# AlexiaChen/mpvss-rs

Hardware: NVIDIA B200
Metric: verified DLEQ shares/sec (MODP n=4096 t=2731, verify_distribution_shares) (higher is better)
Workload: dtype u32 limbs (2048-bit integers)

## Files before the change

mpvss_rs_b200/csrc/ctx.h:

```cpp
#pragma once
#include <cuda_runtime.h>
#include <stdint.h>
#include <mutex>
#include <string.h>
#include <algorithm>
#include <string>
#include <vector>
#include "../../include/mpvss_b200.h"
#include "bigint.h"

struct DevBuf {
  void* p = nullptr;
  size_t cap = 0;
  cudaError_t ensure(size_t bytes) {
    if (bytes <= cap) return cudaSuccess;
    if (p) cudaFree(p);
    p = nullptr;
    cap = 0;
    cudaError_t e = cudaMalloc(&p, bytes);
    if (e == cudaSuccess) cap = bytes;
    return e;
  }
  void release() {
    if (p) cudaFree(p);
    p = nullptr;
    cap = 0;
  }
  template <typename T>
  T* as() const { return static_cast<T*>(p); }
};

struct PinBuf {
  void* p = nullptr;
  size_t cap = 0;
  cudaError_t ensure(size_t bytes) {
    if (bytes <= cap) return cudaSuccess;
    if (p) cudaFreeHost(p);
    p = nullptr;
    cap = 0;
    cudaError_t e = cudaMallocHost(&p, bytes);
    if (e == cudaSuccess) cap = bytes;
    return e;
  }
  void release() {
    if (p) cudaFreeHost(p);
    p = nullptr;
    cap = 0;
  }
  template <typename T>
  T* as() const { return static_cast<T*>(p); }
};

struct mpvss_ctx {
  int group = 0;
  int device = 0;
  int sm_count = 148;
  cudaStream_t stream = nullptr;
  cudaStream_t aux[2] = {nullptr, nullptr};
  cudaEvent_t ev0 = nullptr, ev1 = nullptr, ev_mid = nullptr, ev_h0 = nullptr, ev_h1 = nullptr, ev_fork = nullptr, ev_join[2] = {nullptr, nullptr};
  float phase_ms[4] = {0, 0, 0, 0};
  std::recursive_mutex mu;
  std::string err;
  float last_ms = 0.f;
  int last_launches = 0;
  bool timing_open = false;

  int modp_tpi = 8;
  bool modp_tpi_auto = true;
  int v_tpi = 8;
  int v_wpc = 1;
  std::vector<int64_t> v_plan_pos;
  int v_plan_tpi = 0, v_plan_wpc = 0;
  size_t v_plan_t = 0;
  uint32_t v_plan_kreq = 0, v_k = 1;
  DevBuf v_first, v_steps, v_e, v_h, v_t2;
  int modp_chunks = 0;
  uint64_t v_plan_sqr = 0, v_plan_mul = 0;
  int modp_wpc = 0;
  size_t exp2_filler_ctas = 0;
  int modp_overlap = 3;
  big::Int q, qm1, g;
  DevBuf consts_q, consts_g;
  DevBuf gens;
  DevBuf comb[2];
  int modp_comb = 1;
  int modp_msm = 2;
  int msm_threshold = 512;
  static constexpr size_t msm_batch_threshold = 4096;
  bool device_hash = false;
  bool validate = false;
  bool modp_np1 = false;
  size_t ec_threads = 0;
  DevBuf ec_comb;
  DevBuf ec_consts;
  big::Int ec_order;
  std::vector<uint8_t> ec_gen;
  std::vector<DevBuf> scratch;
  std::vector<PinBuf> pinned;
  size_t v_n = 0, v_t = 0;
  uint32_t v_rwin = 0, v_cwin = 0;
  size_t v_np = 0;
  uint32_t v_nops_max = 1;
  std::vector<uint8_t> v_challenge;
  std::vector<uint32_t> v_hpos;
  size_t ec_chunks = 1;
  const uint32_t* v_comb = nullptr;
  DevBuf v_slot, v_nd, v_ops, v_comm, v_cm, v_pos, v_pk, v_y, v_r, v_c, v_x, v_a1, v_a2;
  DevBuf v_st, v_cst;
  DevBuf v_frames, v_gather, v_ordered;
  PinBuf h_frames;
  size_t v_n_total = 0;
  uint64_t horner_sqr = 0, horner_mul = 0;
  void* comm = nullptr;
  int nranks = 1, rank = 0;
  cudaEvent_t ev_chunk[16] = {};

  mpvss_ctx() : scratch(24), pinned(8) {}
  DevBuf& buf(size_t i) { return scratch.at(i); }
  PinBuf& pin(size_t i) { return pinned.at(i); }
};

int mpvss_fail(mpvss_ctx* ctx, int status, const std::string& msg);
int mpvss_cuda_fail(mpvss_ctx* ctx, cudaError_t e, const char* what);

#define MPVSS_CUDA(ctx, expr)                                        \
  do {                                                               \
    cudaError_t _e = (expr);                                         \
    if (_e != cudaSuccess) return mpvss_cuda_fail(ctx, _e, #expr);   \
  } while (0)
#define MPVSS_TRY(expr)            \
  do {                             \
    int _s = (expr);               \
    if (_s != MPVSS_OK) return _s; \
  } while (0)

void timing_begin(mpvss_ctx* ctx);
void timing_launch(mpvss_ctx* ctx, int n = 1);
int timing_end(mpvss_ctx* ctx);

namespace modp_api {
int init(mpvss_ctx* ctx);
void destroy(mpvss_ctx* ctx);
int batch_exp(mpvss_ctx*, const uint8_t*, size_t, const uint8_t*, size_t, uint8_t*);
int fixed_base_exp(mpvss_ctx*, int, const uint8_t*, size_t, uint8_t*);
int batch_mul(mpvss_ctx*, const uint8_t*, const uint8_t*, size_t, uint8_t*);
int poly_eval_exp(mpvss_ctx*, const uint8_t*, size_t, const int64_t*, size_t, uint8_t*);
int dleq_verify_commit(mpvss_ctx*, const uint8_t*, const uint8_t*, const uint8_t*, const uint8_t*, const uint8_t*,
                       const uint8_t*, size_t, size_t, uint8_t*, uint8_t*);
int dleq_prove_commit(mpvss_ctx*, const uint8_t*, const uint8_t*, const uint8_t*, size_t, uint8_t*, uint8_t*);
int multi_exp(mpvss_ctx*, const uint8_t*, const uint8_t*, size_t, uint8_t*);
int verify_stage(mpvss_ctx*, size_t, size_t, const uint8_t*, const int64_t*, const uint8_t*, const uint8_t*,
                 const uint8_t*, const uint8_t*);
int verify_run(mpvss_ctx*, int*, uint8_t*, uint8_t*, uint8_t*, uint8_t*);
int verify_batch(mpvss_ctx*, size_t, const size_t*, const size_t*, const uint8_t*, const int64_t*, const uint8_t*,
                 const uint8_t*, const uint8_t*, const uint8_t*, int*, uint8_t*);
int scalar_poly_eval(mpvss_ctx*, const uint8_t*, size_t, const int64_t*, size_t, uint8_t*);
int distribute(mpvss_ctx*, size_t, size_t, const uint8_t*, size_t, const uint8_t*, const uint8_t*, const uint8_t*,
               uint8_t*, uint8_t*, uint8_t*, uint8_t*, uint8_t*, uint8_t*);
int extract_shares(mpvss_ctx*, size_t, const uint8_t*, const uint8_t*, const uint8_t*, uint8_t*, uint8_t*, uint8_t*,
                   uint8_t*, int*);
int verify_shares(mpvss_ctx*, size_t, const uint8_t*, const uint8_t*, const uint8_t*, const uint8_t*, const uint8_t*,
                  int*);
int reconstruct(mpvss_ctx*, size_t, const int64_t*, const uint8_t*, const uint8_t*, uint8_t*, uint8_t*);
int reconstruct_batch(mpvss_ctx*, size_t, const size_t*, const int64_t*, const uint8_t*, const uint8_t*, uint8_t*,
                      uint8_t*, int*);
}
namespace secp_api {
int init(mpvss_ctx* ctx);
int batch_exp(mpvss_ctx*, const uint8_t*, size_t, const uint8_t*, size_t, uint8_t*);
int fixed_base_exp(mpvss_ctx*, int, const uint8_t*, size_t, uint8_t*);
int batch_mul(mpvss_ctx*, const uint8_t*, const uint8_t*, size_t, uint8_t*);
int poly_eval_exp(mpvss_ctx*, const uint8_t*, size_t, const int64_t*, size_t, uint8_t*);
int dleq_verify_commit(mpvss_ctx*, const uint8_t*, const uint8_t*, const uint8_t*, const uint8_t*, const uint8_t*,
                       const uint8_t*, size_t, size_t, uint8_t*, uint8_t*);
int dleq_prove_commit(mpvss_ctx*, const uint8_t*, const uint8_t*, const uint8_t*, size_t, uint8_t*, uint8_t*);
int multi_exp(mpvss_ctx*, const uint8_t*, const uint8_t*, size_t, uint8_t*);
int verify_stage(mpvss_ctx*, size_t, size_t, const uint8_t*, const int64_t*, const uint8_t*, const uint8_t*,
                 const uint8_t*, const uint8_t*);
int verify_run(mpvss_ctx*, int*, uint8_t*, uint8_t*, uint8_t*, uint8_t*);
int verify_batch(mpvss_ctx*, size_t, const size_t*, const size_t*, const uint8_t*, const int64_t*, const uint8_t*,
                 const uint8_t*, const uint8_t*, const uint8_t*, int*, uint8_t*);
int scalar_poly_eval(mpvss_ctx*, const uint8_t*, size_t, const int64_t*, size_t, uint8_t*);
int distribute(mpvss_ctx*, size_t, size_t, const uint8_t*, size_t, const uint8_t*, const uint8_t*, const uint8_t*,
               uint8_t*, uint8_t*, uint8_t*, uint8_t*, uint8_t*, uint8_t*);
int extract_shares(mpvss_ctx*, size_t, const uint8_t*, const uint8_t*, const uint8_t*, uint8_t*, uint8_t*, uint8_t*,
                   uint8_t*, int*);
int verify_shares(mpvss_ctx*, size_t, const uint8_t*, const uint8_t*, const uint8_t*, const uint8_t*, const uint8_t*,
                  int*);
int reconstruct(mpvss_ctx*, size_t, const int64_t*, const uint8_t*, const uint8_t*, uint8_t*, uint8_t*);
int reconstruct_batch(mpvss_ctx*, size_t, const size_t*, const int64_t*, const uint8_t*, const uint8_t*, uint8_t*,
                      uint8_t*, int*);
}
namespace rist_api {
int init(mpvss_ctx* ctx);
int batch_exp(mpvss_ctx*, const uint8_t*, size_t, const uint8_t*, size_t, uint8_t*);
int fixed_base_exp(mpvss_ctx*, int, const uint8_t*, size_t, uint8_t*);
int batch_mul(mpvss_ctx*, const uint8_t*, const uint8_t*, size_t, uint8_t*);
int poly_eval_exp(mpvss_ctx*, const uint8_t*, size_t, const int64_t*, size_t, uint8_t*);
int dleq_verify_commit(mpvss_ctx*, const uint8_t*, const uint8_t*, const uint8_t*, const uint8_t*, const uint8_t*,
                       const uint8_t*, size_t, size_t, uint8_t*, uint8_t*);
int dleq_prove_commit(mpvss_ctx*, const uint8_t*, const uint8_t*, const uint8_t*, size_t, uint8_t*, uint8_t*);
int multi_exp(mpvss_ctx*, const uint8_t*, const uint8_t*, size_t, uint8_t*);
int verify_stage(mpvss_ctx*, size_t, size_t, const uint8_t*, const int64_t*, const uint8_t*, const uint8_t*,
                 const uint8_t*, const uint8_t*);
int verify_run(mpvss_ctx*, int*, uint8_t*, uint8_t*, uint8_t*, uint8_t*);
int verify_batch(mpvss_ctx*, size_t, const size_t*, const size_t*, const uint8_t*, const int64_t*, const uint8_t*,
                 const uint8_t*, const uint8_t*, const uint8_t*, int*, uint8_t*);
int scalar_poly_eval(mpvss_ctx*, const uint8_t*, size_t, const int64_t*, size_t, uint8_t*);
int distribute(mpvss_ctx*, size_t, size_t, const uint8_t*, size_t, const uint8_t*, const uint8_t*, const uint8_t*,
               uint8_t*, uint8_t*, uint8_t*, uint8_t*, uint8_t*, uint8_t*);
int extract_shares(mpvss_ctx*, size_t, const uint8_t*, const uint8_t*, const uint8_t*, uint8_t*, uint8_t*, uint8_t*,
                   uint8_t*, int*);
int verify_shares(mpvss_ctx*, size_t, const uint8_t*, const uint8_t*, const uint8_t*, const uint8_t*, const uint8_t*,
                  int*);
int reconstruct(mpvss_ctx*, size_t, const int64_t*, const uint8_t*, const uint8_t*, uint8_t*, uint8_t*);
int reconstruct_batch(mpvss_ctx*, size_t, const size_t*, const int64_t*, const uint8_t*, const uint8_t*, uint8_t*,
                      uint8_t*, int*);
}
```

mpvss_rs_b200/csrc/modp.cu:

```cuda
#include <cuda_runtime.h>
#include "modp_kernels.cuh"
#include "modp_launch.h"

namespace modp {


template <int TPI, bool NP1, bool CHUNKED>
__global__ void __launch_bounds__(HORNER_MAX_WARPS_PER_CTA * 32) horner_kernel(HornerArgs A) {
  extern __shared__ __align__(16) uint32_t smem[];
  uint32_t w = threadIdx.x >> 5;
  horner_body<TPI, NP1, CHUNKED>(A, blockIdx.x * (blockDim.x >> 5) + w, smem + w * horner_smem_words<TPI>,
                                 A.nops ? A.nops[blockIdx.x] : A.nops_all, blockIdx.x);
}

template <int TPI>
__global__ void __launch_bounds__(WARPS_PER_CTA * 32) exp2_kernel(Exp2Args A) {
  extern __shared__ __align__(16) uint32_t smem[];
  uint32_t w = threadIdx.x >> 5;
  exp2_body<TPI>(A, blockIdx.x * WARPS_PER_CTA + w, smem + w * exp2_smem_words<TPI>);
}

template <int TPI>
__global__ void __launch_bounds__(32) exp2_filler_kernel(Exp2Args A, uint32_t nwarps) {
  extern __shared__ __align__(16) uint32_t smem[];
  for (uint32_t w = blockIdx.x; w < nwarps; w += gridDim.x) {
    exp2_body<TPI>(A, w, smem);
    __syncwarp();
  }
}

template <int TPI>
__global__ void __launch_bounds__(32) comb1_kernel(CombArgs A) {
  extern __shared__ __align__(16) uint32_t smem[];
  comb1_body<TPI>(A, blockIdx.x, smem);
}
template <int TPI>
__global__ void __launch_bounds__(32) comb2_kernel(CombArgs A) {
  extern __shared__ __align__(16) uint32_t smem[];
  comb2_body<TPI>(A, blockIdx.x, smem);
}

template <int TPI>
__global__ void __launch_bounds__(WARPS_PER_CTA * 32) mul_kernel(MulArgs A) {
  extern __shared__ __align__(16) uint32_t smem[];
  uint32_t w = threadIdx.x >> 5;
  mul_body<TPI>(A, blockIdx.x * WARPS_PER_CTA + w, smem + w * mul_smem_words<TPI>);
}

__global__ void __launch_bounds__(128) frame_kernel(FrameArgs A) { frame_body(A, blockIdx.x * 128 + threadIdx.x); }
__global__ void __launch_bounds__(64) resp_kernel(RespArgs A) { resp_body(A, blockIdx.x * 64 + threadIdx.x); }
__global__ void __launch_bounds__(64) poly_kernel(PolyArgs A) { poly_body(A, blockIdx.x * 64 + threadIdx.x); }
__global__ void __launch_bounds__(64) lagrange_kernel(LagrangeArgs A) { lagrange_body(A, blockIdx.x * 64 + threadIdx.x); }
__global__ void __launch_bounds__(64) lagrange_boxes_kernel(LagrangeBoxesArgs A) {
  lagrange_boxes_body(A, blockIdx.x * 64 + threadIdx.x);
}

template <int TPI>
__global__ void __launch_bounds__(WARPS_PER_CTA * 32) mul_rows_kernel(MulRowsArgs A) {
  extern __shared__ __align__(16) uint32_t smem[];
  uint32_t w = threadIdx.x >> 5;
  mul_rows_body<TPI>(A, blockIdx.x * WARPS_PER_CTA + w, smem + w * mul_smem_words<TPI>);
}

__global__ void __launch_bounds__(256) msm_sort_kernel(const uint8_t* scalars, uint32_t k, uint32_t* idx, uint32_t* start) {
  __shared__ uint32_t cnt[257], cur[256];
  const uint32_t w = blockIdx.x;
  for (uint32_t d = threadIdx.x; d < 257; d += blockDim.x) cnt[d] = 0;
  __syncthreads();
  for (uint32_t i = threadIdx.x; i < k; i += blockDim.x) atomicAdd(&cnt[scalars[(size_t)i * 256 + w] + 1u], 1u);
  __syncthreads();
  if (threadIdx.x == 0)
    for (int d = 0; d < 256; ++d) cnt[d + 1] += cnt[d];
  __syncthreads();
  for (uint32_t d = threadIdx.x; d < 257; d += blockDim.x) {
    start[w * 257u + d] = cnt[d];
    if (d < 256) cur[d] = cnt[d];
  }
  __syncthreads();
  for (uint32_t i = threadIdx.x; i < k; i += blockDim.x)
    idx[(size_t)w * k + atomicAdd(&cur[scalars[(size_t)i * 256 + w]], 1u)] = i;
}

template <int TPI>
__global__ void __launch_bounds__(WARPS_PER_CTA * 32) msm_bucket_kernel(MsmBucketArgs A) {
  extern __shared__ __align__(16) uint32_t smem[];
  uint32_t w = threadIdx.x >> 5;
  msm_bucket_body<TPI>(A, blockIdx.x * WARPS_PER_CTA + w, smem + w * msm_smem_words<TPI>);
}
template <int TPI>
__global__ void __launch_bounds__(32) msm_window_kernel(MsmWindowArgs A) {
  extern __shared__ __align__(16) uint32_t smem[];
  msm_window_body<TPI>(A, blockIdx.x, smem);
}
template <int TPI>
__global__ void __launch_bounds__(32) msm_fold_kernel(MsmFoldArgs A) {
  extern __shared__ __align__(16) uint32_t smem[];
  msm_fold_body<TPI>(A, smem);
}

template <int TPI>
static uint32_t ctas_for(uint32_t n) {
  uint32_t per_cta = WARPS_PER_CTA * (32 / TPI);
  return (n + per_cta - 1) / per_cta;
}

template <typename K>
static cudaError_t set_smem(K kernel, size_t bytes) {
  cudaError_t e = cudaFuncSetAttribute(kernel, cudaFuncAttributePreferredSharedMemoryCarveout,
                                       (int)cudaSharedmemCarveoutMaxShared);
  if (e != cudaSuccess) return e;
  return cudaFuncSetAttribute(kernel, cudaFuncAttributeMaxDynamicSharedMemorySize, (int)bytes);
}

#define MODP_DISPATCH(tpi, ...)                            \
  switch (tpi) {                                           \
    case 4: { constexpr int T = 4; __VA_ARGS__; break; }   \
    case 8: { constexpr int T = 8; __VA_ARGS__; break; }   \
    case 16: { constexpr int T = 16; __VA_ARGS__; break; } \
    default: return cudaErrorInvalidValue;                 \
  }

template <int TPI, bool NP1, bool CHUNKED>
static cudaError_t horner_go(const HornerArgs& A, uint32_t grid, uint32_t wpc, size_t sm, cudaStream_t s) {
  cudaError_t e = set_smem(horner_kernel<TPI, NP1, CHUNKED>, sm);
  if (e != cudaSuccess) return e;
  horner_kernel<TPI, NP1, CHUNKED><<<grid, wpc * 32, sm, s>>>(A);
  return cudaSuccess;
}
cudaError_t launch_horner(int tpi, const HornerArgs& A, bool np_is_one, cudaStream_t s) {
  if (A.n == 0 || A.t == 0 || A.warps_per_cta > (uint32_t)HORNER_MAX_WARPS_PER_CTA) return cudaErrorInvalidValue;
  MODP_DISPATCH(tpi, {
    const uint32_t wpc = A.warps_per_cta ? A.warps_per_cta : 1u;
    size_t sm = wpc * horner_smem_words<T> * 4;
    uint32_t per_cta = wpc * (32 / T);
    uint32_t grid = (A.n + per_cta - 1) / per_cta;
    const bool chunked = A.cfirst && A.csteps;
    cudaError_t e = np_is_one ? (chunked ? horner_go<T, true, true>(A, grid, wpc, sm, s) : horner_go<T, true, false>(A, grid, wpc, sm, s))
                              : (chunked ? horner_go<T, false, true>(A, grid, wpc, sm, s) : horner_go<T, false, false>(A, grid, wpc, sm, s));
    if (e != cudaSuccess) return e;
  });
  return cudaGetLastError();
}

cudaError_t launch_exp2(int tpi, const Exp2Args& A, cudaStream_t s) {
  if (A.n == 0 || A.e1_windows == 0 || (A.b2 && A.e2_windows == 0)) return cudaErrorInvalidValue;
  MODP_DISPATCH(tpi, {
    size_t sm = WARPS_PER_CTA * exp2_smem_words<T> * 4;
    cudaError_t e = set_smem(exp2_kernel<T>, sm);
    if (e != cudaSuccess) return e;
    exp2_kernel<T><<<ctas_for<T>(A.n), WARPS_PER_CTA * 32, sm, s>>>(A);
  });
  return cudaGetLastError();
}

cudaError_t launch_exp2_filler(int tpi, const Exp2Args& A, size_t ctas, cudaStream_t s) {
  if (A.n == 0 || A.e1_windows == 0 || (A.b2 && A.e2_windows == 0)) return cudaErrorInvalidValue;
  MODP_DISPATCH(tpi, {
    size_t sm = exp2_smem_words<T> * 4;
    cudaError_t e = set_smem(exp2_filler_kernel<T>, sm);
    if (e != cudaSuccess) return e;
    uint32_t per_cta = 32 / T, nwarps = (A.n + per_cta - 1) / per_cta;
    uint32_t grid = (uint32_t)ctas;
    exp2_filler_kernel<T><<<grid < nwarps ? grid : nwarps, 32, sm, s>>>(A, nwarps);
  });
  return cudaGetLastError();
}

cudaError_t launch_frames(const FrameArgs& A, cudaStream_t s) {
  if (A.n == 0) return cudaErrorInvalidValue;
  frame_kernel<<<(A.n * 4 + 127) / 128, 128, 0, s>>>(A);
  return cudaGetLastError();
}

cudaError_t launch_resp(const RespArgs& A, cudaStream_t s) {
  if (A.n == 0) return cudaErrorInvalidValue;
  resp_kernel<<<(A.n + 63) / 64, 64, 0, s>>>(A);
  return cudaGetLastError();
}

cudaError_t launch_poly(const PolyArgs& A, cudaStream_t s) {
  if (A.n == 0 || A.t == 0) return cudaErrorInvalidValue;
  poly_kernel<<<(A.n + 63) / 64, 64, 0, s>>>(A);
  return cudaGetLastError();
}

cudaError_t launch_lagrange(const LagrangeArgs& A, cudaStream_t s) {
  if (A.k == 0) return cudaErrorInvalidValue;
  const uint32_t threads = 2u * (A.parts ? A.parts : 1u) * A.k;
  lagrange_kernel<<<(threads + 63) / 64, 64, 0, s>>>(A);
  return cudaGetLastError();
}

cudaError_t launch_lagrange_boxes(const LagrangeBoxesArgs& A, cudaStream_t s) {
  if (A.n == 0) return cudaErrorInvalidValue;
  const uint32_t threads = 2u * (A.parts ? A.parts : 1u) * A.n;
  lagrange_boxes_kernel<<<(threads + 63) / 64, 64, 0, s>>>(A);
  return cudaGetLastError();
}

cudaError_t launch_comb_build(int tpi, const CombArgs& A, cudaStream_t s) {
  MODP_DISPATCH(tpi, {
    size_t sm = comb_smem_words<T> * 4;
    comb1_kernel<T><<<1, 32, sm, s>>>(A);
    comb2_kernel<T><<<(A.rows + 32 / T - 1) / (32 / T), 32, sm, s>>>(A);
  });
  return cudaGetLastError();
}

cudaError_t launch_msm(const MsmBucketArgs& B, const uint32_t* scalars, uint32_t* idx, uint32_t* start,
                       uint32_t* wprod, uint32_t* out, cudaStream_t s) {
  if (B.windows == 0 || B.windows > 256 || B.k == 0) return cudaErrorInvalidValue;
  constexpr int T = 8;
  msm_sort_kernel<<<B.windows, 256, 0, s>>>(reinterpret_cast<const uint8_t*>(scalars), B.k, idx, start);
  const uint32_t groups = B.windows * 255u, per_cta = WARPS_PER_CTA * (32 / T);
  size_t sm = WARPS_PER_CTA * msm_smem_words<T> * 4;
  msm_bucket_kernel<T><<<(groups + per_cta - 1) / per_cta, WARPS_PER_CTA * 32, sm, s>>>(B);
  MsmWindowArgs W{B.consts, B.buckets, wprod, B.windows};
  msm_window_kernel<T><<<B.windows, 32, msm_window_smem_words<T> * 4, s>>>(W);
  MsmFoldArgs F{B.consts, wprod, out, B.windows};
  msm_fold_kernel<T><<<1, 32, msm_smem_words<T> * 4, s>>>(F);
  return cudaGetLastError();
}

cudaError_t launch_mul(int tpi, const MulArgs& A, cudaStream_t s) {
  if (A.n == 0) return cudaErrorInvalidValue;
  MODP_DISPATCH(tpi, {
    size_t sm = WARPS_PER_CTA * mul_smem_words<T> * 4;
    cudaError_t e = set_smem(mul_kernel<T>, sm);
    if (e != cudaSuccess) return e;
    mul_kernel<T><<<ctas_for<T>(A.n), WARPS_PER_CTA * 32, sm, s>>>(A);
  });
  return cudaGetLastError();
}

cudaError_t launch_mul_rows(int tpi, const MulRowsArgs& A, cudaStream_t s) {
  if (A.n == 0) return cudaErrorInvalidValue;
  MODP_DISPATCH(tpi, {
    size_t sm = WARPS_PER_CTA * mul_smem_words<T> * 4;
    cudaError_t e = set_smem(mul_rows_kernel<T>, sm);
    if (e != cudaSuccess) return e;
    mul_rows_kernel<T><<<ctas_for<T>(A.n), WARPS_PER_CTA * 32, sm, s>>>(A);
  });
  return cudaGetLastError();
}

}
```

mpvss_rs_b200/csrc/modp_api.cu:

```cuda
#include <algorithm>
#include <cstdlib>
#include "ctx.h"
#include "modp_chain.h"
#include "modp_launch.h"
#include "sha2.h"
#include "hash_launch.h"
#include "transcript.h"

namespace {

constexpr size_t EB = 256;
constexpr size_t EW = 64;

const char* RFC3526_2048 =
    "ffffffffffffffffc90fdaa22168c234c4c6628b80dc1cd129024e088a67cc74"
    "020bbea63b139b22514a08798e3404ddef9519b3cd3a431b302b0a6df25f1437"
    "4fe1356d6d51c245e485b576625e7ec6f44c42e9a637ed6b0bff5cb6f406b7ed"
    "ee386bfb5a899fa5ae9f24117c4b1fe649286651ece45b3dc2007cb8a163bf05"
    "98da48361c55d39a69163fa8fd24cf5f83655d23dca3ad961c62f356208552bb"
    "9ed529077096966d670c354e4abc9804f1746c08ca18217c32905e462e36ce3b"
    "e39e772c180e86039b2783a2ec07a28fb5c55df06f4c52c9de2bcbf695581718"
    "3995497cea956ae515d2261898fa051015728e5a8aacaa68ffffffffffffffff";

big::Int from_hex(const char* s) {
  size_t n = strlen(s);
  std::vector<uint8_t> be((n + 1) / 2, 0);
  for (size_t i = 0; i < n; ++i) {
    char c = s[n - 1 - i];
    uint8_t v = c <= '9' ? c - '0' : (c | 32) - 'a' + 10;
    be[be.size() - 1 - i / 2] |= v << (4 * (i % 2));
  }
  return big::from_be(be.data(), be.size());
}

void fill_consts(const big::Int& m, uint32_t* blk) {
  memset(blk, 0, modp::C_WORDS * 4);
  big::Int R(65, 0);
  R[64] = 1;
  big::Int nq = big::sub(R, m), one = big::mod(R, m), r2 = big::mulmod(one, one, m);
  auto put = [&](const big::Int& v, int off) {
    for (size_t i = 0; i < v.size() && i < 64; ++i) blk[off + i] = v[i];
  };
  put(m, modp::C_Q);
  put(nq, modp::C_NQ);
  put(one, modp::C_ONE);
  put(r2, modp::C_R2);
  big::Int one1(1, 1);
  put(big::shr1(big::add(m, one1)), modp::C_QH);
  uint32_t inv = 1, m0 = m[0];
  for (int i = 0; i < 5; ++i) inv *= 2u - m0 * inv;
  blk[modp::C_NP] = 0u - inv;
}

size_t min_be(const uint8_t* le, uint8_t* out) {
  size_t len = EB;
  while (len > 1 && le[len - 1] == 0) --len;
  for (size_t i = 0; i < len; ++i) out[i] = le[len - 1 - i];
  return len;
}
void framed_update(sha2::Sha256& h, const uint8_t* le) {
  uint8_t tmp[EB], len8[8] = {0};
  size_t len = min_be(le, tmp);
  len8[6] = (uint8_t)(len >> 8);
  len8[7] = (uint8_t)len;
  h.update(len8, 8);
  h.update(tmp, len);
}
void challenge_from_digest(const mpvss_ctx* ctx, const uint8_t digest[32], uint8_t out[EB]) {
  uint8_t h2[32];
  sha2::sha256(digest, 32, h2);
  big::Int c = big::mod(big::from_be(h2, 32), ctx->g);
  big::to_le(c, out, EB);
}
uint32_t windows_for(const uint8_t* scalars, size_t stride, size_t n) {
  size_t top = 0;
  for (size_t i = 0; i < n; ++i) {
    const uint8_t* s = scalars + i * stride;
    size_t len = EB;
    while (len > top && s[len - 1] == 0) --len;
    if (len > top) top = len;
    if (top == EB) break;
  }
  uint32_t w = (uint32_t)(top * 2);
  return w ? w : 1;
}

int h2d(mpvss_ctx* ctx, DevBuf& b, const void* src, size_t bytes) {
  MPVSS_CUDA(ctx, b.ensure(bytes));
  MPVSS_CUDA(ctx, cudaMemcpyAsync(b.p, src, bytes, cudaMemcpyHostToDevice, ctx->stream));
  return MPVSS_OK;
}
int d2h(mpvss_ctx* ctx, void* dst, const DevBuf& b, size_t bytes) {
  MPVSS_CUDA(ctx, cudaMemcpyAsync(dst, b.p, bytes, cudaMemcpyDeviceToHost, ctx->stream));
  return MPVSS_OK;
}
int sync(mpvss_ctx* ctx) {
  MPVSS_CUDA(ctx, cudaStreamSynchronize(ctx->stream));
  return MPVSS_OK;
}

int dev_exp2(mpvss_ctx* ctx, const uint32_t* consts, const uint32_t* b1, uint32_t b1s, const uint32_t* e1,
             uint32_t e1s, uint32_t e1w, const uint32_t* b2, uint32_t b2s, const uint32_t* e2, uint32_t e2s,
             uint32_t e2w, size_t n, uint32_t* out, cudaStream_t stream = nullptr, const uint32_t* comb1 = nullptr) {
  modp::Exp2Args A{consts, b1, e1, b2, e2, out, (uint32_t)n, b1s, e1s, e1w, b2s, e2s, e2w, comb1};
  if (ctx->exp2_filler_ctas)
    MPVSS_CUDA(ctx, modp::launch_exp2_filler(ctx->modp_tpi, A, ctx->exp2_filler_ctas, stream ? stream : ctx->stream));
  else
    MPVSS_CUDA(ctx, modp::launch_exp2(ctx->modp_tpi, A, stream ? stream : ctx->stream));
  timing_launch(ctx);
  return MPVSS_OK;
}
int dev_mul(mpvss_ctx* ctx, const uint32_t* consts, const uint32_t* a, uint32_t as, const uint32_t* b, uint32_t bs,
            uint32_t mode, size_t n, uint32_t* out) {
  modp::MulArgs A{consts, a, b, out, (uint32_t)n, mode, as, bs};
  MPVSS_CUDA(ctx, modp::launch_mul(ctx->modp_tpi, A, ctx->stream));
  timing_launch(ctx);
  return MPVSS_OK;
}

int comb_table(mpvss_ctx* ctx, int which, const uint32_t** out) {
  *out = nullptr;
  if (!ctx->modp_comb) return MPVSS_OK;
  DevBuf& t = ctx->comb[which];
  if (!t.p) {
    MPVSS_CUDA(ctx, t.ensure((size_t)256 * 256 * EB));
    modp::CombArgs A{ctx->consts_q.as<uint32_t>(), ctx->gens.as<uint32_t>() + which * 64, t.as<uint32_t>(), 256};
    MPVSS_CUDA(ctx, modp::launch_comb_build(ctx->modp_tpi, A, ctx->stream));
    MPVSS_CUDA(ctx, cudaStreamSynchronize(ctx->stream));
  }
  *out = t.as<uint32_t>();
  return MPVSS_OK;
}

int check_args(mpvss_ctx* ctx, bool ok, const char* what) {
  if (!ok) return mpvss_fail(ctx, MPVSS_ERR_ARG, what);
  return MPVSS_OK;
}

}

namespace modp_api {

int init(mpvss_ctx* ctx) {
  ctx->q = from_hex(RFC3526_2048);
  ctx->qm1 = big::sub(ctx->q, big::from_u64(1));
  ctx->g = big::shr1(ctx->qm1);
  std::vector<uint32_t> blk(modp::C_WORDS);
  fill_consts(ctx->q, blk.data());
  ctx->modp_np1 = blk[modp::C_NP] == 1u;
  MPVSS_TRY(h2d(ctx, ctx->consts_q, blk.data(), blk.size() * 4));
  fill_consts(ctx->g, blk.data());
  MPVSS_TRY(h2d(ctx, ctx->consts_g, blk.data(), blk.size() * 4));
  std::vector<uint32_t> gens(192, 0);
  gens[0] = 2;
  gens[64] = 4;
  gens[128] = 1;
  MPVSS_TRY(h2d(ctx, ctx->gens, gens.data(), gens.size() * 4));
  return sync(ctx);
}

void destroy(mpvss_ctx* ctx) {
  for (DevBuf* b : {&ctx->consts_q, &ctx->consts_g, &ctx->gens, &ctx->comb[0], &ctx->comb[1], &ctx->v_comm, &ctx->v_cm, &ctx->v_pos, &ctx->v_pk,
                    &ctx->v_y, &ctx->v_r, &ctx->v_c, &ctx->v_x, &ctx->v_a1, &ctx->v_a2, &ctx->v_slot, &ctx->v_nd, &ctx->v_ops, &ctx->v_frames, &ctx->v_gather, &ctx->v_ordered, &ctx->v_st, &ctx->v_cst, &ctx->v_first, &ctx->v_steps,
                    &ctx->v_e, &ctx->v_h, &ctx->v_t2})
    b->release();
}

int batch_exp(mpvss_ctx* ctx, const uint8_t* bases, size_t base_stride, const uint8_t* scalars, size_t n,
              uint8_t* out) {
  MPVSS_TRY(check_args(ctx, bases && scalars && out && n > 0 && (base_stride == 0 || base_stride == EB),
                       "batch_exp: bad arguments"));
  DevBuf &db = ctx->buf(0), &de = ctx->buf(1), &dout = ctx->buf(2);
  MPVSS_TRY(h2d(ctx, db, bases, base_stride ? n * EB : EB));
  MPVSS_TRY(h2d(ctx, de, scalars, n * EB));
  MPVSS_CUDA(ctx, dout.ensure(n * EB));
  timing_begin(ctx);
  MPVSS_TRY(dev_exp2(ctx, ctx->consts_q.as<uint32_t>(), db.as<uint32_t>(), base_stride ? EW : 0, de.as<uint32_t>(), EW,
                     windows_for(scalars, EB, n), nullptr, 0, nullptr, 0, 0, n, dout.as<uint32_t>()));
  MPVSS_TRY(timing_end(ctx));
  MPVSS_TRY(d2h(ctx, out, dout, n * EB));
  return sync(ctx);
}

int fixed_base_exp(mpvss_ctx* ctx, int generator, const uint8_t* scalars, size_t n, uint8_t* out) {
  MPVSS_TRY(check_args(ctx, scalars && out && n > 0 && (generator == MPVSS_GEN_MAIN || generator == MPVSS_GEN_SUBGROUP),
                       "fixed_base_exp: bad arguments"));
  DevBuf &de = ctx->buf(1), &dout = ctx->buf(2);
  MPVSS_TRY(h2d(ctx, de, scalars, n * EB));
  MPVSS_CUDA(ctx, dout.ensure(n * EB));
  const uint32_t* comb;
  MPVSS_TRY(comb_table(ctx, generator ? 1 : 0, &comb));
  timing_begin(ctx);
  MPVSS_TRY(dev_exp2(ctx, ctx->consts_q.as<uint32_t>(), ctx->gens.as<uint32_t>() + (generator ? 64 : 0), 0,
                     de.as<uint32_t>(), EW, windows_for(scalars, EB, n), nullptr, 0, nullptr, 0, 0, n,
                     dout.as<uint32_t>(), nullptr, comb));
  MPVSS_TRY(timing_end(ctx));
  MPVSS_TRY(d2h(ctx, out, dout, n * EB));
  return sync(ctx);
}

int batch_mul(mpvss_ctx* ctx, const uint8_t* a, const uint8_t* b, size_t n, uint8_t* out) {
  MPVSS_TRY(check_args(ctx, a && b && out && n > 0, "batch_mul: bad arguments"));
  DevBuf &da = ctx->buf(0), &db = ctx->buf(1), &dout = ctx->buf(2);
  MPVSS_TRY(h2d(ctx, da, a, n * EB));
  MPVSS_TRY(h2d(ctx, db, b, n * EB));
  MPVSS_CUDA(ctx, dout.ensure(n * EB));
  timing_begin(ctx);
  MPVSS_TRY(dev_mul(ctx, ctx->consts_q.as<uint32_t>(), da.as<uint32_t>(), EW, db.as<uint32_t>(), EW, 0, n,
                    dout.as<uint32_t>()));
  MPVSS_TRY(timing_end(ctx));
  MPVSS_TRY(d2h(ctx, out, dout, n * EB));
  return sync(ctx);
}

static int horner_tpi(const mpvss_ctx* ctx, size_t n) {
  if (!ctx->modp_tpi_auto) return ctx->modp_tpi;
  if (n >= 32768) return 4;
  if (n * 8 / 32 < (size_t)4 * (size_t)ctx->sm_count) return 16;
  return ctx->modp_tpi;
}

static int horner_wpc(const mpvss_ctx* ctx, size_t n, int tpi) {
  if (ctx->modp_wpc) return ctx->modp_wpc;
  (void)n;
  (void)tpi;
  return 1;
}

static uint32_t horner_chunks(const mpvss_ctx* ctx, size_t n, size_t t) {
  uint32_t K = 1;
  if (ctx->modp_chunks > 0) {
    K = (uint32_t)ctx->modp_chunks;
  } else {
    const size_t warps = (n + 3) / 4, full = (size_t)8 * (size_t)ctx->sm_count;
    while (K < 8 && warps * (K * 2) <= full) K *= 2;
  }
  if (ctx->modp_chunks <= 0 && t < 1366) K = 1;
  while (K > 1 && t / K < (ctx->modp_chunks > 0 ? 32u : 340u)) K /= 2;
  return K;
}

struct PosPlan {
  int tpi = 8;
  int wpc = 1;
  uint32_t K = 1, B = 0;
  std::vector<uint32_t> first, steps;
  std::vector<uint32_t> slot;
  std::vector<uint16_t> ops;
  std::vector<uint32_t> nops;
  uint64_t sqr = 0, mul = 0;
  uint32_t nops_max = 1;
};
static modp_chain::PowerTree g_tree;
static std::mutex g_tree_mu;

struct PlanBox {
  const int64_t* positions;
  size_t n, t;
  uint32_t cm_off, row_off;
};

static int prep_boxes(mpvss_ctx* ctx, const PlanBox* boxes, size_t nb, bool chunked, PosPlan& plan) {
  static_assert(modp_chain::SLOTS == modp::HC_SLOTS && modp_chain::OPS_MAX == modp::HC_OPS, "kernel / host op format");
  auto position = [&](const PlanBox& bx, size_t i) { return bx.positions ? bx.positions[i] : (int64_t)i + 1; };
  uint32_t maxp = 1;
  size_t n_all = 0;
  for (size_t b = 0; b < nb; ++b) {
    for (size_t i = 0; i < boxes[b].n; ++i) {
      int64_t p = position(boxes[b], i);
      if (p < 1 || p > 0x7fffffff) return mpvss_fail(ctx, MPVSS_ERR_ARG, "position out of range [1, 2^31)");
      maxp = std::max<uint32_t>(maxp, (uint32_t)p);
    }
    n_all += boxes[b].n;
  }
  std::lock_guard<std::mutex> lk(g_tree_mu);
  g_tree.build(std::min<uint32_t>(maxp, modp_chain::TREE_LIMIT));
  std::vector<std::vector<uint16_t>> ops(n_all);
  std::vector<std::vector<std::vector<uint32_t>>> by(nb, std::vector<std::vector<uint32_t>>(modp_chain::OPS_MAX + 1));
  std::vector<uint32_t> sq(n_all), ml(n_all);
  for (size_t b = 0, g = 0; b < nb; ++b)
    for (size_t i = 0; i < boxes[b].n; ++i, ++g) {
      if (!modp_chain::step_ops((uint32_t)position(boxes[b], i), g_tree, ops[g], &sq[g], &ml[g]))
        return mpvss_fail(ctx, MPVSS_ERR_UNSUPPORTED, "no addition chain within the kernel's slot budget");
      by[b][ops[g].size()].push_back((uint32_t)g);
    }
  const size_t t0 = boxes[0].t;
  if (chunked && nb != 1) return mpvss_fail(ctx, MPVSS_ERR_ARG, "a chunked plan covers one box");
  plan.K = chunked ? horner_chunks(ctx, n_all, t0) : 1;
  plan.B = (uint32_t)((t0 + plan.K - 1) / plan.K);
  plan.K = (uint32_t)((t0 + plan.B - 1) / plan.B);
  plan.tpi = plan.K > 1 ? ctx->modp_tpi : horner_tpi(ctx, n_all);
  plan.wpc = horner_wpc(ctx, n_all, plan.tpi);
  const size_t per_cta = (size_t)plan.wpc * (32 / plan.tpi);
  plan.slot.clear(); plan.ops.clear(); plan.nops.clear(); plan.first.clear(); plan.steps.clear();
  plan.nops_max = 1;
  plan.sqr = plan.mul = 0;
  std::vector<uint32_t> base(nb, 0);
  for (size_t b = 1; b < nb; ++b) base[b] = base[b - 1] + (uint32_t)boxes[b - 1].n;
  for (uint32_t k = 0; k < plan.K; ++k) {
    for (uint32_t len = modp_chain::OPS_MAX; len >= 1; --len) {
      for (size_t b = 0; b < nb; ++b) {
        const std::vector<uint32_t>& cls = by[b][len];
        if (cls.empty()) continue;
        const PlanBox& bx = boxes[b];
        const uint32_t lo = plan.K > 1 ? k * plan.B : 0, hi = (uint32_t)std::min<size_t>(bx.t, (size_t)lo + (plan.K > 1 ? plan.B : bx.t));
        plan.nops_max = std::max(plan.nops_max, len);
        auto emit = [&](uint32_t g, uint32_t slot) {
          plan.slot.push_back(slot);
          size_t at = plan.ops.size();
          plan.ops.resize(at + modp_chain::OPS_MAX, (uint16_t)modp_chain::B_ONE);
          std::copy(ops[g].begin(), ops[g].end(), plan.ops.begin() + at);
        };
        for (uint32_t g : cls) {
          emit(g, bx.row_off + k * (uint32_t)bx.n + (g - base[b]));
          plan.sqr += (uint64_t)sq[g] * (hi - lo - 1);
          plan.mul += (uint64_t)ml[g] * (hi - lo - 1);
        }
        while (plan.slot.size() % per_cta) emit(cls.back(), 0xffffffffu);
        const size_t ctas = plan.slot.size() / per_cta;
        plan.nops.resize(ctas, len);
        plan.first.resize(ctas, bx.cm_off + hi - 1);
        plan.steps.resize(ctas, hi - lo - 1);
      }
    }
  }
  return MPVSS_OK;
}
static int prep_positions(mpvss_ctx* ctx, const int64_t* positions, size_t n, size_t t, PosPlan& plan) {
  const PlanBox box{positions, n, t, 0, 0};
  return prep_boxes(ctx, &box, 1, true, plan);
}

static int dev_chunk_exponents(mpvss_ctx* ctx, const int64_t* positions, size_t n, uint32_t E, uint32_t* e_out_dev) {
  std::vector<uint8_t> base(n * EB, 0), bexp(EB, 0), e(n * EB);
  for (size_t i = 0; i < n; ++i) {
    uint32_t p = (uint32_t)(positions ? positions[i] : (int64_t)i + 1);
    memcpy(base.data() + i * EB, &p, 4);
  }
  memcpy(bexp.data(), &E, 4);
  DevBuf &db = ctx->buf(20), &dx = ctx->buf(21);
  MPVSS_TRY(h2d(ctx, db, base.data(), n * EB));
  MPVSS_TRY(h2d(ctx, dx, bexp.data(), EB));
  MPVSS_TRY(dev_exp2(ctx, ctx->consts_g.as<uint32_t>(), db.as<uint32_t>(), EW, dx.as<uint32_t>(), 0,
                     windows_for(bexp.data(), EB, 1), nullptr, 0, nullptr, 0, 0, n, e_out_dev));
  MPVSS_CUDA(ctx, cudaMemcpyAsync(e.data(), e_out_dev, n * EB, cudaMemcpyDeviceToHost, ctx->stream));
  MPVSS_TRY(sync(ctx));
  for (size_t i = 0; i < n; ++i) {
    if ((e[i * EB] & 1u) != (base[i * EB] & 1u)) {
      big::Int v = big::add(big::from_le(e.data() + i * EB, EB), ctx->g);
      big::to_le(v, e.data() + i * EB, EB);
    }
  }
  MPVSS_CUDA(ctx, cudaMemcpyAsync(e_out_dev, e.data(), n * EB, cudaMemcpyHostToDevice, ctx->stream));
  return sync(ctx);
}
static int plan_chunk_exponents(mpvss_ctx* ctx, const int64_t* positions, size_t n, const PosPlan& plan, DevBuf& e) {
  if (plan.K <= 1) return MPVSS_OK;
  MPVSS_CUDA(ctx, e.ensure((size_t)(plan.K - 1) * n * EB));
  for (uint32_t k = 1; k < plan.K; ++k)
    MPVSS_TRY(dev_chunk_exponents(ctx, positions, n, k * plan.B, e.as<uint32_t>() + (size_t)(k - 1) * n * EW));
  return MPVSS_OK;
}

struct PlanDev {
  const uint16_t* ops;
  const uint32_t *slot, *nops, *first, *steps;
  const uint32_t* e;
  size_t n_padded;
  uint32_t K;
  int tpi, wpc;
  bool boxes = false;
};
static int dev_horner(mpvss_ctx* ctx, const PlanDev& P, const uint32_t* comm, DevBuf& cm, size_t t, size_t n, DevBuf& hbuf,
                      DevBuf& tbuf, uint32_t* x) {
  const uint32_t* Kq = ctx->consts_q.as<uint32_t>();
  MPVSS_CUDA(ctx, cm.ensure(t * EB));
  MPVSS_TRY(dev_mul(ctx, Kq, comm, EW, nullptr, 0, 1, t, cm.as<uint32_t>()));
  uint32_t* h = x;
  if (P.K > 1) {
    MPVSS_CUDA(ctx, hbuf.ensure((size_t)P.K * n * EB));
    MPVSS_CUDA(ctx, tbuf.ensure((size_t)(P.K - 1) * n * EB));
    h = hbuf.as<uint32_t>();
  }
  static const bool uniform = getenv("MPVSS_HORNER_UNIFORM") != nullptr;
  const bool arrays = P.K > 1 || P.boxes || !uniform;
  modp::HornerArgs A{Kq, cm.as<uint32_t>(), P.ops, P.slot, P.nops, h, (uint32_t)t, (uint32_t)P.n_padded, 0,
                     (uint32_t)P.wpc, arrays ? P.first : nullptr, arrays ? P.steps : nullptr};
  MPVSS_CUDA(ctx, cudaEventRecord(ctx->ev_h0, ctx->stream));
  MPVSS_CUDA(ctx, modp::launch_horner(P.tpi, A, ctx->modp_np1, ctx->stream));
  MPVSS_CUDA(ctx, cudaEventRecord(ctx->ev_h1, ctx->stream));
  timing_launch(ctx);
  if (P.K > 1) {
    uint32_t* T = tbuf.as<uint32_t>();
    MPVSS_TRY(dev_exp2(ctx, Kq, h + n * EW, EW, P.e, EW, 512, nullptr, 0, nullptr, 0, 0, (size_t)(P.K - 1) * n, T));
    MPVSS_TRY(dev_mul(ctx, Kq, h, EW, T, EW, 0, n, x));
    for (uint32_t k = 2; k < P.K; ++k) MPVSS_TRY(dev_mul(ctx, Kq, x, EW, T + (size_t)(k - 1) * n * EW, EW, 0, n, x));
  }
  return MPVSS_OK;
}

int poly_eval_exp(mpvss_ctx* ctx, const uint8_t* commitments, size_t t, const int64_t* positions, size_t n,
                  uint8_t* out) {
  MPVSS_TRY(check_args(ctx, commitments && out && n > 0 && t > 0, "poly_eval_exp: bad arguments"));
  PosPlan plan;
  MPVSS_TRY(prep_positions(ctx, positions, n, t, plan));
  DevBuf &dc = ctx->buf(0), &dops = ctx->buf(1), &dout = ctx->buf(2), &dcm = ctx->buf(3), &dsl = ctx->buf(4),
         &dno = ctx->buf(5), &dfi = ctx->buf(6), &dstp = ctx->buf(7), &de = ctx->buf(8);
  const size_t np = plan.slot.size();
  MPVSS_TRY(h2d(ctx, dc, commitments, t * EB));
  MPVSS_TRY(h2d(ctx, dops, plan.ops.data(), plan.ops.size() * 2));
  MPVSS_TRY(h2d(ctx, dsl, plan.slot.data(), np * 4));
  MPVSS_TRY(h2d(ctx, dno, plan.nops.data(), plan.nops.size() * 4));
  MPVSS_TRY(h2d(ctx, dfi, plan.first.data(), plan.first.size() * 4));
  MPVSS_TRY(h2d(ctx, dstp, plan.steps.data(), plan.steps.size() * 4));
  MPVSS_CUDA(ctx, dout.ensure(n * EB));
  MPVSS_TRY(plan_chunk_exponents(ctx, positions, n, plan, de));
  PlanDev P{dops.as<uint16_t>(), dsl.as<uint32_t>(), dno.as<uint32_t>(), dfi.as<uint32_t>(), dstp.as<uint32_t>(),
            de.as<uint32_t>(), np, plan.K, plan.tpi, plan.wpc};
  timing_begin(ctx);
  MPVSS_TRY(dev_horner(ctx, P, dc.as<uint32_t>(), dcm, t, n, ctx->buf(9), ctx->buf(10), dout.as<uint32_t>()));
  MPVSS_TRY(timing_end(ctx));
  ctx->horner_sqr = plan.sqr;
  ctx->horner_mul = plan.mul;
  MPVSS_TRY(d2h(ctx, out, dout, n * EB));
  return sync(ctx);
}

int dleq_verify_commit(mpvss_ctx* ctx, const uint8_t* g1, const uint8_t* h1, const uint8_t* g2, const uint8_t* h2,
                       const uint8_t* r, const uint8_t* c, size_t c_stride, size_t n, uint8_t* a1, uint8_t* a2) {
  MPVSS_TRY(check_args(ctx, g1 && h1 && g2 && h2 && r && c && (!a1 == !a2) && n > 0 && (c_stride == 0 || c_stride == EB),
                       "dleq_verify_commit: bad arguments"));
  DevBuf &dg1 = ctx->buf(0), &dh1 = ctx->buf(1), &dg2 = ctx->buf(2), &dh2 = ctx->buf(3), &dr = ctx->buf(4),
         &dc = ctx->buf(5), &da1 = ctx->buf(6), &da2 = ctx->buf(7);
  MPVSS_TRY(h2d(ctx, dg1, g1, EB));
  MPVSS_TRY(h2d(ctx, dh1, h1, n * EB));
  MPVSS_TRY(h2d(ctx, dg2, g2, n * EB));
  MPVSS_TRY(h2d(ctx, dh2, h2, n * EB));
  MPVSS_TRY(h2d(ctx, dr, r, n * EB));
  MPVSS_TRY(h2d(ctx, dc, c, c_stride ? n * EB : EB));
  MPVSS_CUDA(ctx, da1.ensure(n * EB));
  MPVSS_CUDA(ctx, da2.ensure(n * EB));
  uint32_t rw = windows_for(r, EB, n), cw = windows_for(c, EB, c_stride ? n : 1), cs = c_stride ? EW : 0;
  const uint32_t* K = ctx->consts_q.as<uint32_t>();
  const uint32_t* comb = nullptr;
  {
    bool rest_zero = true;
    for (size_t i = 1; i < EB; ++i) rest_zero = rest_zero && g1[i] == 0;
    if (rest_zero && (g1[0] == 2 || g1[0] == 4)) MPVSS_TRY(comb_table(ctx, g1[0] == 4 ? 1 : 0, &comb));
  }
  timing_begin(ctx);
  MPVSS_TRY(dev_exp2(ctx, K, dg1.as<uint32_t>(), 0, dr.as<uint32_t>(), EW, rw, dh1.as<uint32_t>(), EW,
                     dc.as<uint32_t>(), cs, cw, n, da1.as<uint32_t>(), nullptr, comb));
  MPVSS_TRY(dev_exp2(ctx, K, dg2.as<uint32_t>(), EW, dr.as<uint32_t>(), EW, rw, dh2.as<uint32_t>(), EW,
                     dc.as<uint32_t>(), cs, cw, n, da2.as<uint32_t>()));
  MPVSS_TRY(timing_end(ctx));
  if (a1) MPVSS_TRY(d2h(ctx, a1, da1, n * EB));
  if (a2) MPVSS_TRY(d2h(ctx, a2, da2, n * EB));
  return sync(ctx);
}

int dleq_prove_commit(mpvss_ctx* ctx, const uint8_t* g1, const uint8_t* g2, const uint8_t* w, size_t n, uint8_t* a1,
                      uint8_t* a2) {
  MPVSS_TRY(check_args(ctx, g1 && g2 && w && a1 && a2 && n > 0, "dleq_prove_commit: bad arguments"));
  DevBuf &dg1 = ctx->buf(0), &dg2 = ctx->buf(2), &dw = ctx->buf(4), &da1 = ctx->buf(6), &da2 = ctx->buf(7);
  MPVSS_TRY(h2d(ctx, dg1, g1, EB));
  MPVSS_TRY(h2d(ctx, dg2, g2, n * EB));
  MPVSS_TRY(h2d(ctx, dw, w, n * EB));
  MPVSS_CUDA(ctx, da1.ensure(n * EB));
  MPVSS_CUDA(ctx, da2.ensure(n * EB));
  uint32_t ww = windows_for(w, EB, n);
  const uint32_t* K = ctx->consts_q.as<uint32_t>();
  timing_begin(ctx);
  MPVSS_TRY(dev_exp2(ctx, K, dg1.as<uint32_t>(), 0, dw.as<uint32_t>(), EW, ww, nullptr, 0, nullptr, 0, 0, n,
                     da1.as<uint32_t>()));
  MPVSS_TRY(dev_exp2(ctx, K, dg2.as<uint32_t>(), EW, dw.as<uint32_t>(), EW, ww, nullptr, 0, nullptr, 0, 0, n,
                     da2.as<uint32_t>()));
  MPVSS_TRY(timing_end(ctx));
  MPVSS_TRY(d2h(ctx, a1, da1, n * EB));
  MPVSS_TRY(d2h(ctx, a2, da2, n * EB));
  return sync(ctx);
}

static int dev_product_tree(mpvss_ctx* ctx, uint32_t* v, DevBuf& tmp, size_t n) {
  const uint32_t* K = ctx->consts_q.as<uint32_t>();
  MPVSS_CUDA(ctx, tmp.ensure(((n + 1) / 2) * EB));
  while (n > 1) {
    size_t half = n / 2;
    MPVSS_TRY(dev_mul(ctx, K, v, EW, v + half * EW, EW, 0, half, tmp.as<uint32_t>()));
    if (n & 1)
      MPVSS_CUDA(ctx, cudaMemcpyAsync(tmp.as<uint32_t>() + half * EW, v + 2 * half * EW, EB, cudaMemcpyDeviceToDevice,
                                      ctx->stream));
    n = half + (n & 1);
    MPVSS_CUDA(ctx, cudaMemcpyAsync(v, tmp.p, n * EB, cudaMemcpyDeviceToDevice, ctx->stream));
  }
  return MPVSS_OK;
}

static int multi_exp_buckets(mpvss_ctx* ctx, DevBuf& db, DevBuf& de, uint32_t windows, size_t n, DevBuf& dout) {
  DevBuf &dm = ctx->buf(15), &didx = ctx->buf(16), &dst = ctx->buf(17), &dbk = ctx->buf(18), &dwp = ctx->buf(19);
  MPVSS_CUDA(ctx, didx.ensure((size_t)windows * n * 4));
  MPVSS_CUDA(ctx, dst.ensure((size_t)windows * 257 * 4));
  MPVSS_CUDA(ctx, dm.ensure(n * EB));
  MPVSS_CUDA(ctx, dbk.ensure((size_t)windows * 256 * EB));
  MPVSS_CUDA(ctx, dwp.ensure((size_t)windows * EB));
  const uint32_t* K = ctx->consts_q.as<uint32_t>();
  MPVSS_TRY(dev_mul(ctx, K, db.as<uint32_t>(), EW, nullptr, 0, 1, n, dm.as<uint32_t>()));
  modp::MsmBucketArgs B{K, dm.as<uint32_t>(), didx.as<uint32_t>(), dst.as<uint32_t>(), dbk.as<uint32_t>(), windows,
                        (uint32_t)n};
  MPVSS_CUDA(ctx, modp::launch_msm(B, de.as<uint32_t>(), didx.as<uint32_t>(), dst.as<uint32_t>(), dwp.as<uint32_t>(),
                                   dout.as<uint32_t>(), ctx->stream));
  timing_launch(ctx, 4);
  return MPVSS_OK;
}

int multi_exp(mpvss_ctx* ctx, const uint8_t* bases, const uint8_t* scalars, size_t n, uint8_t* out) {
  MPVSS_TRY(check_args(ctx, bases && scalars && out && n > 0, "multi_exp: bad arguments"));
  DevBuf &db = ctx->buf(0), &de = ctx->buf(1), &dout = ctx->buf(2), &tmp = ctx->buf(3);
  MPVSS_TRY(h2d(ctx, db, bases, n * EB));
  MPVSS_CUDA(ctx, dout.ensure(n * EB));
  const bool buckets = ctx->modp_msm == 1 || (ctx->modp_msm == 2 && n >= (size_t)ctx->msm_threshold);
  MPVSS_TRY(h2d(ctx, de, scalars, n * EB));
  timing_begin(ctx);
  if (buckets) {
    MPVSS_TRY(multi_exp_buckets(ctx, db, de, (windows_for(scalars, EB, n) + 1) / 2, n, dout));
  } else {
    MPVSS_TRY(dev_exp2(ctx, ctx->consts_q.as<uint32_t>(), db.as<uint32_t>(), EW, de.as<uint32_t>(), EW,
                       windows_for(scalars, EB, n), nullptr, 0, nullptr, 0, 0, n, dout.as<uint32_t>()));
    MPVSS_TRY(dev_product_tree(ctx, dout.as<uint32_t>(), tmp, n));
  }
  MPVSS_TRY(timing_end(ctx));
  MPVSS_TRY(d2h(ctx, out, dout, EB));
  return sync(ctx);
}

int scalar_poly_eval(mpvss_ctx* ctx, const uint8_t* coeffs, size_t t, const int64_t* positions, size_t n, uint8_t* out) {
  MPVSS_TRY(check_args(ctx, coeffs && out && n > 0 && t > 0, "scalar_poly_eval: bad arguments"));
  std::vector<uint32_t> order(EW, 0), pos(n);
  for (size_t i = 0; i < ctx->qm1.size(); ++i) order[i] = ctx->qm1[i];
  for (size_t i = 0; i < n; ++i) {
    int64_t p = positions ? positions[i] : (int64_t)i + 1;
    if (p < 1 || p > 0x7fffffff) return mpvss_fail(ctx, MPVSS_ERR_ARG, "position out of range [1, 2^31)");
    pos[i] = (uint32_t)p;
  }
  std::vector<uint8_t> co(t * EB);
  for (size_t j = 0; j < t; ++j) big::to_le(big::mod(big::from_le(coeffs + j * EB, EB), ctx->qm1), co.data() + j * EB, EB);
  DevBuf &dco = ctx->buf(0), &dp = ctx->buf(1), &dord = ctx->buf(11), &dpos = ctx->buf(12);
  MPVSS_TRY(h2d(ctx, dco, co.data(), t * EB));
  MPVSS_TRY(h2d(ctx, dord, order.data(), EB));
  MPVSS_TRY(h2d(ctx, dpos, pos.data(), n * 4));
  MPVSS_CUDA(ctx, dp.ensure(n * EB));
  timing_begin(ctx);
  modp::PolyArgs PA{dco.as<uint32_t>(), dord.as<uint32_t>(), dpos.as<uint32_t>(), dp.as<uint32_t>(), (uint32_t)t,
                    (uint32_t)n};
  MPVSS_CUDA(ctx, modp::launch_poly(PA, ctx->stream));
  timing_launch(ctx);
  MPVSS_TRY(timing_end(ctx));
  MPVSS_TRY(d2h(ctx, out, dp, n * EB));
  MPVSS_CUDA(ctx, cudaMemsetAsync(dco.p, 0, dco.cap, ctx->stream));
  return sync(ctx);
}

static int validate_elements(mpvss_ctx* ctx, const uint32_t* dev, size_t count, uint8_t* bad) {
  std::vector<uint8_t> gexp(EB), res(count * EB), in(count * EB);
  big::to_le(ctx->g, gexp.data(), EB);
  DevBuf &de = ctx->buf(20), &dout = ctx->buf(21);
  MPVSS_TRY(h2d(ctx, de, gexp.data(), EB));
  MPVSS_CUDA(ctx, dout.ensure(count * EB));
  MPVSS_TRY(dev_exp2(ctx, ctx->consts_q.as<uint32_t>(), dev, EW, de.as<uint32_t>(), 0, 512, nullptr, 0, nullptr, 0, 0,
                     count, dout.as<uint32_t>()));
  MPVSS_TRY(d2h(ctx, res.data(), dout, count * EB));
  MPVSS_CUDA(ctx, cudaMemcpyAsync(in.data(), dev, count * EB, cudaMemcpyDeviceToHost, ctx->stream));
  MPVSS_TRY(sync(ctx));
  for (size_t i = 0; i < count; ++i) {
    big::Int x = big::from_le(in.data() + i * EB, EB);
    bool one = res[i * EB] == 1;
    for (size_t k = 1; k < EB && one; ++k) one = res[i * EB + k] == 0;
    if (big::is_zero(x) || big::cmp(x, ctx->q) >= 0 || !one) bad[i] = 1;
  }
  return MPVSS_OK;
}

static const transcript::Geom GEOM{EB, true};

static const uint8_t* slice_rows(const mpvss_ctx* ctx, const uint8_t* all, size_t n_total, size_t width,
                                 std::vector<uint8_t>& tmp) {
  if (ctx->nranks <= 1) return all;
  tmp.clear();
  for (size_t i = (size_t)ctx->rank; i < n_total; i += (size_t)ctx->nranks)
    tmp.insert(tmp.end(), all + i * width, all + (i + 1) * width);
  return tmp.data();
}

int verify_stage(mpvss_ctx* ctx, size_t n_total, size_t t, const uint8_t* commitments, const int64_t* positions,
                 const uint8_t* publickeys, const uint8_t* shares, const uint8_t* responses, const uint8_t* challenge) {
  ctx->v_n_total = 0;
  MPVSS_TRY(check_args(ctx, n_total > 0 && t > 0 && commitments && publickeys && shares && responses && challenge,
                       "verify_distribution: bad arguments"));
  const size_t n = transcript::local_count(n_total, ctx->nranks, ctx->rank);
  std::vector<int64_t> pos(n);
  for (size_t j = 0; j < n; ++j) {
    const size_t i = (size_t)ctx->rank + j * (size_t)ctx->nranks;
    pos[j] = positions ? positions[i] : (int64_t)i + 1;
  }
  for (size_t i = 0; i < n_total; ++i)
    if (positions && (positions[i] < 1 || positions[i] > 0x7fffffff))
      return mpvss_fail(ctx, MPVSS_ERR_ENCODING, "verify_distribution: position out of range [1, 2^31)");
  PosPlan plan;
  const uint32_t want_k = n ? horner_chunks(ctx, n, t) : 1;
  const bool replan = n && !(ctx->v_plan_pos == pos && ctx->v_plan_t == t && ctx->v_plan_kreq == want_k &&
                             ctx->v_plan_tpi == (want_k > 1 ? ctx->modp_tpi : horner_tpi(ctx, n)) &&
                             ctx->v_plan_wpc == horner_wpc(ctx, n, ctx->v_plan_tpi));
  if (replan) {
    ctx->v_plan_pos.clear();
    MPVSS_TRY(prep_positions(ctx, pos.data(), n, t, plan));
    ctx->v_np = plan.slot.size();
    ctx->v_nops_max = plan.nops_max;
    ctx->v_tpi = plan.tpi;
    ctx->v_wpc = plan.wpc;
    ctx->v_k = plan.K;
    ctx->v_plan_sqr = plan.sqr;
    ctx->v_plan_mul = plan.mul;
  }
  ctx->horner_sqr = ctx->v_plan_sqr;
  ctx->horner_mul = ctx->v_plan_mul;
  std::vector<uint8_t> tpk, ty, tr;
  const uint8_t* pk = slice_rows(ctx, publickeys, n_total, EB, tpk);
  const uint8_t* y = slice_rows(ctx, shares, n_total, EB, ty);
  const uint8_t* r = slice_rows(ctx, responses, n_total, EB, tr);
  MPVSS_TRY(h2d(ctx, ctx->v_comm, commitments, t * EB));
  MPVSS_TRY(h2d(ctx, ctx->v_c, challenge, EB));
  if (replan) {
    MPVSS_TRY(h2d(ctx, ctx->v_ops, plan.ops.data(), plan.ops.size() * 2));
    MPVSS_TRY(h2d(ctx, ctx->v_slot, plan.slot.data(), ctx->v_np * 4));
    MPVSS_TRY(h2d(ctx, ctx->v_nd, plan.nops.data(), plan.nops.size() * 4));
    MPVSS_TRY(h2d(ctx, ctx->v_first, plan.first.data(), plan.first.size() * 4));
    MPVSS_TRY(h2d(ctx, ctx->v_steps, plan.steps.data(), plan.steps.size() * 4));
    MPVSS_TRY(plan_chunk_exponents(ctx, pos.data(), n, plan, ctx->v_e));
    MPVSS_TRY(sync(ctx));
    ctx->v_plan_pos = pos;
    ctx->v_plan_t = t;
    ctx->v_plan_kreq = want_k;
    ctx->v_plan_tpi = plan.tpi;
    ctx->v_plan_wpc = plan.wpc;
  }
  if (n) {
    MPVSS_TRY(h2d(ctx, ctx->v_pk, pk, n * EB));
    MPVSS_TRY(h2d(ctx, ctx->v_y, y, n * EB));
    MPVSS_TRY(h2d(ctx, ctx->v_r, r, n * EB));
    MPVSS_CUDA(ctx, ctx->v_x.ensure(n * EB));
    MPVSS_CUDA(ctx, ctx->v_a1.ensure(n * EB));
    MPVSS_CUDA(ctx, ctx->v_a2.ensure(n * EB));
  }
  const size_t rpr = transcript::rows_per_rank(n_total, ctx->nranks);
  MPVSS_CUDA(ctx, ctx->v_frames.ensure(rpr * GEOM.row()));
  MPVSS_CUDA(ctx, cudaMemsetAsync(ctx->v_frames.p, 0, rpr * GEOM.row(), ctx->stream));
  if (ctx->nranks > 1) MPVSS_CUDA(ctx, ctx->v_gather.ensure((size_t)ctx->nranks * rpr * GEOM.row()));
  MPVSS_TRY(comb_table(ctx, 1, &ctx->v_comb));
  ctx->v_rwin = n ? windows_for(r, EB, n) : 1;
  ctx->v_cwin = windows_for(challenge, EB, 1);
  ctx->v_challenge.assign(challenge, challenge + EB);
  ctx->v_n = n;
  ctx->v_t = t;
  MPVSS_TRY(sync(ctx));
  ctx->v_n_total = n_total;
  return MPVSS_OK;
}

static int a2_placement(const mpvss_ctx* ctx, size_t n, double horner, size_t np, int tpi, uint32_t rwin, uint32_t cwin) {
  int overlap = ctx->modp_overlap;
  if (overlap == 3) {
    const size_t groups_per_warp = 32 / (size_t)ctx->modp_tpi;
    const size_t nwarps = (n + groups_per_warp - 1) / groups_per_warp;
    const size_t rounds = (nwarps + (size_t)ctx->sm_count - 1) / (size_t)ctx->sm_count;
    const double filler = (double)rounds * (5.0 * (rwin + cwin) + 30.0);
    if (filler > 0.6 * horner) overlap = 0;
    const size_t slots = (size_t)4 * (size_t)ctx->sm_count;
    const size_t hw = np / (32 / (size_t)tpi);
    const size_t holes = (slots - hw % slots) % slots;
    if (holes < (size_t)ctx->sm_count) overlap = 0;
    if (overlap == 0 && hw + nwarps <= (size_t)12 * (size_t)ctx->sm_count) overlap = 2;
  }
  return overlap;
}

static int verify_kernels(mpvss_ctx* ctx) {
  const size_t n = ctx->v_n, t = ctx->v_t;
  const uint32_t* K = ctx->consts_q.as<uint32_t>();
  uint32_t* X = ctx->v_x.as<uint32_t>();
  timing_begin(ctx);
  if (n == 0) {
    MPVSS_TRY(timing_end(ctx));
    ctx->phase_ms[0] = ctx->phase_ms[1] = ctx->phase_ms[2] = 0.f;
    return MPVSS_OK;
  }
  MPVSS_CUDA(ctx, cudaEventRecord(ctx->ev_fork, ctx->stream));
  auto launch_a2 = [&](cudaStream_t s) {
    return dev_exp2(ctx, K, ctx->v_pk.as<uint32_t>(), EW, ctx->v_r.as<uint32_t>(), EW, ctx->v_rwin,
                    ctx->v_y.as<uint32_t>(), EW, ctx->v_c.as<uint32_t>(), 0, ctx->v_cwin, n,
                    ctx->v_a2.as<uint32_t>(), s);
  };
  const int overlap = a2_placement(ctx, n, (double)(t > 1 ? t - 1 : 0) / (double)ctx->v_k * (double)ctx->v_nops_max,
                                   ctx->v_np, ctx->v_tpi, ctx->v_rwin, ctx->v_cwin);
  const bool side = overlap == 2 || overlap == 3;
  if (!side) MPVSS_TRY(launch_a2(ctx->stream));
  PlanDev P{ctx->v_ops.as<uint16_t>(), ctx->v_slot.as<uint32_t>(), ctx->v_nd.as<uint32_t>(), ctx->v_first.as<uint32_t>(),
            ctx->v_steps.as<uint32_t>(), ctx->v_e.as<uint32_t>(), ctx->v_np, ctx->v_k, ctx->v_tpi, ctx->v_wpc};
  MPVSS_TRY(dev_horner(ctx, P, ctx->v_comm.as<uint32_t>(), ctx->v_cm, t, n, ctx->v_h, ctx->v_t2, X));
  if (side) {
    MPVSS_CUDA(ctx, cudaStreamWaitEvent(ctx->aux[0], ctx->ev_fork, 0));
    if (overlap == 3) ctx->exp2_filler_ctas = (size_t)ctx->sm_count;
    int rc = launch_a2(ctx->aux[0]);
    ctx->exp2_filler_ctas = 0;
    MPVSS_TRY(rc);
    MPVSS_CUDA(ctx, cudaEventRecord(ctx->ev_join[0], ctx->aux[0]));
  }
  MPVSS_CUDA(ctx, cudaEventRecord(ctx->ev_mid, ctx->stream));
  MPVSS_TRY(dev_exp2(ctx, K, ctx->gens.as<uint32_t>() + 64, 0, ctx->v_r.as<uint32_t>(), EW, ctx->v_rwin, X, EW,
                     ctx->v_c.as<uint32_t>(), 0, ctx->v_cwin, n, ctx->v_a1.as<uint32_t>(), nullptr, ctx->v_comb));
  if (side) MPVSS_CUDA(ctx, cudaStreamWaitEvent(ctx->stream, ctx->ev_join[0], 0));
  modp::FrameArgs FA{X, ctx->v_y.as<uint32_t>(), ctx->v_a1.as<uint32_t>(), ctx->v_a2.as<uint32_t>(),
                     ctx->v_frames.as<uint8_t>(), (uint32_t)n};
  MPVSS_CUDA(ctx, modp::launch_frames(FA, ctx->stream));
  timing_launch(ctx);
  if (ctx->validate) {
    std::vector<uint8_t> bad(t + 2 * n, 0);
    MPVSS_TRY(validate_elements(ctx, ctx->v_comm.as<uint32_t>(), t, bad.data()));
    MPVSS_TRY(validate_elements(ctx, ctx->v_pk.as<uint32_t>(), n, bad.data() + t));
    MPVSS_TRY(validate_elements(ctx, ctx->v_y.as<uint32_t>(), n, bad.data() + t + n));
    if (std::find(bad.begin(), bad.end(), 1) != bad.end()) {
      const uint8_t mark = 0xff;
      MPVSS_CUDA(ctx, cudaMemcpyAsync(ctx->v_frames.p, &mark, 1, cudaMemcpyHostToDevice, ctx->stream));
    }
  }
  MPVSS_TRY(timing_end(ctx));
  MPVSS_CUDA(ctx, cudaEventElapsedTime(&ctx->phase_ms[0], ctx->ev0, ctx->ev_mid));
  MPVSS_CUDA(ctx, cudaEventElapsedTime(&ctx->phase_ms[1], ctx->ev_mid, ctx->ev1));
  MPVSS_CUDA(ctx, cudaEventElapsedTime(&ctx->phase_ms[2], ctx->ev_h0, ctx->ev_h1));
  return MPVSS_OK;
}

int verify_run(mpvss_ctx* ctx, int* ok, uint8_t* x_out, uint8_t* a1_out, uint8_t* a2_out, uint8_t* digest_out) {
  MPVSS_TRY(check_args(ctx, ok && ctx->v_n_total > 0, "verify_distribution_run: nothing staged"));
  MPVSS_TRY(check_args(ctx, ctx->nranks <= 1 || (!x_out && !a1_out && !a2_out),
                       "verify_distribution: x/a1/a2 outputs are not available with a communicator"));
  const size_t n = ctx->v_n, n_total = ctx->v_n_total;
  MPVSS_TRY(verify_kernels(ctx));
  const uint8_t* rows = ctx->v_frames.as<uint8_t>();
  if (ctx->nranks > 1) {
    MPVSS_TRY(comm_allgather(ctx, ctx->v_frames.p, ctx->v_gather.p,
                             transcript::rows_per_rank(n_total, ctx->nranks) * GEOM.row()));
    MPVSS_CUDA(ctx, ctx->v_ordered.ensure(n_total * GEOM.row()));
    MPVSS_TRY(comm_reorder_rows(ctx, ctx->v_gather.p, ctx->v_ordered.p, n_total, GEOM.row()));
    rows = ctx->v_ordered.as<uint8_t>();
  }
  uint8_t digest[32], c[EB];
  if (ctx->device_hash) {
    MPVSS_TRY(transcript::device_digest(ctx, rows, n_total, ctx->nranks, GEOM, digest));
  } else {
    sha2::Sha256 h;
    MPVSS_TRY(transcript::fetch_and_hash(ctx, rows, n_total, ctx->nranks, GEOM, h, true));
    h.finalize(digest);
  }
  challenge_from_digest(ctx, digest, c);
  *ok = memcmp(c, ctx->v_challenge.data(), EB) == 0;
  for (size_t r = 0; r < std::min<size_t>((size_t)ctx->nranks, n_total); ++r)
    if (ctx->h_frames.as<uint8_t>()[r * GEOM.row()] == 0xff) *ok = 0;
  if (digest_out) memcpy(digest_out, digest, 32);
  if (x_out) MPVSS_TRY(d2h(ctx, x_out, ctx->v_x, n * EB));
  if (a1_out) MPVSS_TRY(d2h(ctx, a1_out, ctx->v_a1, n * EB));
  if (a2_out) MPVSS_TRY(d2h(ctx, a2_out, ctx->v_a2, n * EB));
  return sync(ctx);
}

int verify_batch(mpvss_ctx* ctx, size_t nb, const size_t* nv, const size_t* tv, const uint8_t* commitments,
                 const int64_t* positions, const uint8_t* publickeys, const uint8_t* shares, const uint8_t* responses,
                 const uint8_t* challenges, int* ok_out, uint8_t* digests_out) {
  std::vector<size_t> noff(nb + 1, 0), toff(nb + 1, 0);
  for (size_t b = 0; b < nb; ++b) {
    noff[b + 1] = noff[b] + nv[b];
    toff[b + 1] = toff[b] + tv[b];
  }
  const size_t N = noff[nb], Tt = toff[nb];
  std::vector<uint8_t> live(nb, 1);
  std::vector<PlanBox> boxes;
  for (size_t b = 0; b < nb; ++b) {
    const int64_t* p = positions ? positions + noff[b] : nullptr;
    for (size_t i = 0; p && i < nv[b] && live[b]; ++i) live[b] = p[i] >= 1 && p[i] <= 0x7fffffff;
    if (live[b]) boxes.push_back(PlanBox{p, nv[b], tv[b], (uint32_t)toff[b], (uint32_t)noff[b]});
  }
  std::vector<uint8_t> cexp(N * EB);
  for (size_t b = 0; b < nb; ++b)
    for (size_t i = noff[b]; i < noff[b + 1]; ++i) memcpy(cexp.data() + i * EB, challenges + b * EB, EB);
  const uint32_t rwin = windows_for(responses, EB, N), cwin = windows_for(challenges, EB, nb);
  DevBuf &dcomm = ctx->buf(0), &dcm = ctx->buf(1), &dpk = ctx->buf(2), &dy = ctx->buf(3), &dr = ctx->buf(4),
         &dc = ctx->buf(5), &dx = ctx->buf(6), &da1 = ctx->buf(7), &da2 = ctx->buf(8), &dfr = ctx->buf(9),
         &dops = ctx->buf(10), &dsl = ctx->buf(11), &dno = ctx->buf(12), &dfi = ctx->buf(13), &dstp = ctx->buf(14);
  MPVSS_TRY(h2d(ctx, dcomm, commitments, Tt * EB));
  MPVSS_TRY(h2d(ctx, dpk, publickeys, N * EB));
  MPVSS_TRY(h2d(ctx, dy, shares, N * EB));
  MPVSS_TRY(h2d(ctx, dr, responses, N * EB));
  MPVSS_TRY(h2d(ctx, dc, cexp.data(), N * EB));
  for (DevBuf* b : {&dx, &da1, &da2}) MPVSS_CUDA(ctx, b->ensure(N * EB));
  MPVSS_CUDA(ctx, dfr.ensure(N * GEOM.row()));
  if (boxes.size() < nb) MPVSS_CUDA(ctx, cudaMemsetAsync(dx.p, 0, N * EB, ctx->stream));
  PosPlan plan;
  if (!boxes.empty()) {
    MPVSS_TRY(prep_boxes(ctx, boxes.data(), boxes.size(), false, plan));
    MPVSS_TRY(h2d(ctx, dops, plan.ops.data(), plan.ops.size() * 2));
    MPVSS_TRY(h2d(ctx, dsl, plan.slot.data(), plan.slot.size() * 4));
    MPVSS_TRY(h2d(ctx, dno, plan.nops.data(), plan.nops.size() * 4));
    MPVSS_TRY(h2d(ctx, dfi, plan.first.data(), plan.first.size() * 4));
    MPVSS_TRY(h2d(ctx, dstp, plan.steps.data(), plan.steps.size() * 4));
  }
// ... 197 lines not shown
  big::Int inv;
  if (!big::modinv_odd(big::from_le(root, EB), ctx->g, &inv))
    return mpvss_fail(ctx, MPVSS_ERR_ARG, "batch inversion: an element is 0 modulo the subgroup order");
  big::to_le(inv, root, EB);
  uint32_t *cur = ia.as<uint32_t>(), *nxt = ib.as<uint32_t>();
  MPVSS_CUDA(ctx, cudaMemcpyAsync(cur, root, EB, cudaMemcpyHostToDevice, ctx->stream));
  MPVSS_CUDA(ctx, cudaStreamSynchronize(ctx->stream));
  memset(root, 0, EB);
  std::fill(inv.begin(), inv.end(), 0u);
  for (size_t l = L; l >= 1; --l) {
    const size_t h = N >> l;
    MPVSS_TRY(dev_mul(ctx, Kg, cur, EW, T + (off[l - 1] + h) * EW, EW, 0, h, nxt));
    MPVSS_TRY(dev_mul(ctx, Kg, cur, EW, T + off[l - 1] * EW, EW, 0, h, nxt + h * EW));
    std::swap(cur, nxt);
  }
  MPVSS_CUDA(ctx, cudaMemcpyAsync(out, cur, n * EB, cudaMemcpyDeviceToDevice, ctx->stream));
  return MPVSS_OK;
}

static int share_challenges(mpvss_ctx* ctx, const uint32_t* h1, const uint32_t* h2, const uint32_t* a1, const uint32_t* a2,
                            size_t n, uint32_t* c_out, uint32_t stride) {
  DevBuf& drows = ctx->buf(14);
  MPVSS_CUDA(ctx, drows.ensure(n * 4 * modp::FRAME_BYTES));
  const float ms0 = ctx->last_ms;
  const int l0 = ctx->last_launches;
  timing_begin(ctx);
  modp::FrameArgs FA{h1, h2, a1, a2, drows.as<uint8_t>(), (uint32_t)n};
  MPVSS_CUDA(ctx, modp::launch_frames(FA, ctx->stream));
  shadev::RowHashArgs HA{drows.as<uint8_t>(), 4u * modp::FRAME_BYTES, (uint32_t)modp::FRAME_BYTES, c_out, stride, nullptr,
                         (uint32_t)n, 0u};
  MPVSS_CUDA(ctx, shadev::launch_row_hash(HA, ctx->stream));
  timing_launch(ctx, 2);
  MPVSS_TRY(timing_end(ctx));
  ctx->last_ms += ms0;
  ctx->last_launches += l0;
  return MPVSS_OK;
}

int extract_shares(mpvss_ctx* ctx, size_t n, const uint8_t* private_keys, const uint8_t* witnesses,
                   const uint8_t* enc_shares, uint8_t* publickeys_out, uint8_t* shares_out, uint8_t* challenges_out,
                   uint8_t* responses_out, int* status_out) {
  MPVSS_TRY(check_args(ctx, n > 0 && private_keys && witnesses && enc_shares && publickeys_out && shares_out &&
                                challenges_out && responses_out,
                       "extract_shares: bad arguments"));
  const uint32_t* K = ctx->consts_q.as<uint32_t>();
  const uint32_t* Kg = ctx->consts_g.as<uint32_t>();
  const uint32_t* G = ctx->gens.as<uint32_t>();
  std::vector<uint8_t> skg(n * EB);
  std::vector<int> st(n, MPVSS_OK);
  for (size_t i = 0; i < n; ++i) {
    big::Int sk = big::mod(big::from_le(private_keys + i * EB, EB), ctx->qm1);
    big::Int r = big::mod(sk, ctx->g);
    if (!big::is_odd(sk) || big::is_zero(r)) {
      st[i] = MPVSS_ERR_NOT_INVERTIBLE;
      r = big::from_u64(1);
    }
    big::to_le(r, skg.data() + i * EB, EB);
  }
  DevBuf &dsk = ctx->buf(0), &dskg = ctx->buf(1), &dinv = ctx->buf(3), &dw = ctx->buf(4),
         &dY = ctx->buf(5), &dpk = ctx->buf(6), &dS = ctx->buf(7), &dA1 = ctx->buf(8), &dA2 = ctx->buf(9);
  MPVSS_TRY(h2d(ctx, dsk, private_keys, n * EB));
  MPVSS_TRY(h2d(ctx, dskg, skg.data(), n * EB));
  MPVSS_TRY(h2d(ctx, dw, witnesses, n * EB));
  MPVSS_TRY(h2d(ctx, dY, enc_shares, n * EB));
  for (DevBuf* b : {&dinv, &dpk, &dS, &dA1, &dA2}) MPVSS_CUDA(ctx, b->ensure(n * EB));
  timing_begin(ctx);
  MPVSS_TRY(dev_batch_inverse_g(ctx, dskg.as<uint32_t>(), n, dinv.as<uint32_t>()));
  MPVSS_TRY(timing_end(ctx));
  std::vector<uint8_t> inv(n * EB);
  MPVSS_TRY(d2h(ctx, inv.data(), dinv, n * EB));
  MPVSS_TRY(sync(ctx));
  for (size_t i = 0; i < n; ++i) {
    big::Int x = big::from_le(inv.data() + i * EB, EB);
    if (!big::is_odd(x)) x = big::add(x, ctx->g);
    big::to_le(x, inv.data() + i * EB, EB);
  }
  MPVSS_TRY(h2d(ctx, dinv, inv.data(), n * EB));
  const uint32_t skw = 512, ww = 512;
  const uint32_t* combG;
  MPVSS_TRY(comb_table(ctx, 0, &combG));
  float ms0 = ctx->last_ms;
  int l0 = ctx->last_launches;
  timing_begin(ctx);
  MPVSS_TRY(dev_exp2(ctx, K, G, 0, dsk.as<uint32_t>(), EW, skw, nullptr, 0, nullptr, 0, 0, n, dpk.as<uint32_t>(),
                     nullptr, combG));
  MPVSS_TRY(dev_exp2(ctx, K, dY.as<uint32_t>(), EW, dinv.as<uint32_t>(), EW, 512, nullptr, 0, nullptr, 0, 0, n,
                     dS.as<uint32_t>()));
  MPVSS_TRY(dev_exp2(ctx, K, G, 0, dw.as<uint32_t>(), EW, ww, nullptr, 0, nullptr, 0, 0, n, dA1.as<uint32_t>(),
                     nullptr, combG));
  MPVSS_TRY(dev_exp2(ctx, K, dS.as<uint32_t>(), EW, dw.as<uint32_t>(), EW, ww, nullptr, 0, nullptr, 0, 0, n,
                     dA2.as<uint32_t>()));
  MPVSS_TRY(timing_end(ctx));
  ctx->last_ms += ms0;
  ctx->last_launches += l0;
  {
    std::vector<uint32_t> order(EW, 0);
    for (size_t i = 0; i < ctx->qm1.size(); ++i) order[i] = ctx->qm1[i];
    DevBuf &dord = ctx->buf(11), &dch = ctx->buf(12), &dR = ctx->buf(13);
    MPVSS_TRY(h2d(ctx, dord, order.data(), EB));
    MPVSS_CUDA(ctx, dch.ensure(n * EB));
    MPVSS_CUDA(ctx, dR.ensure(n * EB));
    MPVSS_TRY(share_challenges(ctx, dpk.as<uint32_t>(), dY.as<uint32_t>(), dA1.as<uint32_t>(), dA2.as<uint32_t>(), n,
                               dch.as<uint32_t>(), EW));
    modp::RespArgs RA{dord.as<uint32_t>(), dsk.as<uint32_t>(), dw.as<uint32_t>(), dch.as<uint32_t>(), dR.as<uint32_t>(),
                      (uint32_t)n, EW, EW};
    MPVSS_CUDA(ctx, modp::launch_resp(RA, ctx->stream));
    ctx->last_launches += 1;
    MPVSS_TRY(d2h(ctx, publickeys_out, dpk, n * EB));
    MPVSS_TRY(d2h(ctx, shares_out, dS, n * EB));
    MPVSS_TRY(d2h(ctx, challenges_out, dch, n * EB));
    MPVSS_TRY(d2h(ctx, responses_out, dR, n * EB));
    for (DevBuf* b : {&dsk, &dskg, &dinv, &dw}) MPVSS_CUDA(ctx, cudaMemsetAsync(b->p, 0, b->cap, ctx->stream));
    MPVSS_TRY(sync(ctx));
  }
  if (status_out) memcpy(status_out, st.data(), n * sizeof(int));
  return MPVSS_OK;
}

int verify_shares(mpvss_ctx* ctx, size_t n, const uint8_t* publickeys, const uint8_t* shares,
                  const uint8_t* enc_shares, const uint8_t* challenges, const uint8_t* responses, int* ok_out) {
  MPVSS_TRY(check_args(ctx, n > 0 && publickeys && shares && enc_shares && challenges && responses && ok_out,
                       "verify_shares: bad arguments"));
  std::vector<uint8_t> gen(EB, 0);
  gen[0] = 2;
  MPVSS_TRY(dleq_verify_commit(ctx, gen.data(), publickeys, shares, enc_shares, responses, challenges, EB, n, nullptr,
                               nullptr));
  DevBuf& dch = ctx->buf(12);
  MPVSS_CUDA(ctx, dch.ensure(n * 32));
  MPVSS_TRY(share_challenges(ctx, ctx->buf(1).as<uint32_t>(), ctx->buf(3).as<uint32_t>(), ctx->buf(6).as<uint32_t>(),
                             ctx->buf(7).as<uint32_t>(), n, dch.as<uint32_t>(), 8));
  std::vector<uint8_t> c(n * 32);
  MPVSS_TRY(d2h(ctx, c.data(), dch, n * 32));
  MPVSS_TRY(sync(ctx));
  for (size_t i = 0; i < n; ++i) {
    const uint8_t* given = challenges + i * EB;
    bool same = memcmp(c.data() + i * 32, given, 32) == 0;
    for (size_t k = 32; k < EB && same; ++k) same = given[k] == 0;
    ok_out[i] = same;
  }
  return MPVSS_OK;
}

int reconstruct(mpvss_ctx* ctx, size_t k, const int64_t* positions, const uint8_t* shares, const uint8_t* u,
                uint8_t* secret_out, uint8_t* gs_out) {
  MPVSS_TRY(check_args(ctx, k > 0 && positions && shares && u && secret_out, "reconstruct: bad arguments"));
  for (size_t i = 0; i < k; ++i)
    if (positions[i] < 1 || positions[i] > 0x7fffffff) return mpvss_fail(ctx, MPVSS_ERR_ARG, "position out of range");
  std::vector<uint32_t> pos(k), order(EW, 0);
  for (size_t i = 0; i < k; ++i) pos[i] = (uint32_t)positions[i];
  {
    std::vector<uint32_t> sorted(pos);
    std::sort(sorted.begin(), sorted.end());
    if (std::adjacent_find(sorted.begin(), sorted.end()) != sorted.end())
      return mpvss_fail(ctx, MPVSS_ERR_ARG, "duplicate position");
  }
  for (size_t i = 0; i < ctx->qm1.size(); ++i) order[i] = ctx->qm1[i];
  std::vector<uint8_t> lam(k * EB);
  DevBuf &dpos = ctx->buf(12), &dord = ctx->buf(13), &dnum = ctx->buf(14), &dden = ctx->buf(15), &dneg = ctx->buf(16),
         &dinv = ctx->buf(18), &dlam = ctx->buf(19);
  MPVSS_TRY(h2d(ctx, dpos, pos.data(), k * 4));
  MPVSS_TRY(h2d(ctx, dord, order.data(), EB));
  const size_t parts = k >= 64 ? 8 : 1;
  for (DevBuf* b : {&dnum, &dden}) MPVSS_CUDA(ctx, b->ensure(parts * k * EB));
  for (DevBuf* b : {&dinv, &dlam}) MPVSS_CUDA(ctx, b->ensure(k * EB));
  MPVSS_CUDA(ctx, dneg.ensure(parts * k * 4));
  const uint32_t* Kg = ctx->consts_g.as<uint32_t>();
  modp::LagrangeArgs LA{dord.as<uint32_t>(), dpos.as<uint32_t>(), dnum.as<uint32_t>(), dden.as<uint32_t>(),
                        dneg.as<uint32_t>(), (uint32_t)k, (uint32_t)parts};
  timing_begin(ctx);
  MPVSS_CUDA(ctx, modp::launch_lagrange(LA, ctx->stream));
  timing_launch(ctx);
  for (size_t half = parts / 2; half >= 1; half /= 2)
    for (DevBuf* b : {&dnum, &dden})
      MPVSS_TRY(dev_mul(ctx, Kg, b->as<uint32_t>(), EW, b->as<uint32_t>() + half * k * EW, EW, 0, half * k,
                        b->as<uint32_t>()));
  MPVSS_TRY(dev_batch_inverse_g(ctx, dden.as<uint32_t>(), k, dinv.as<uint32_t>()));
  MPVSS_TRY(dev_mul(ctx, Kg, dnum.as<uint32_t>(), EW, dinv.as<uint32_t>(), EW, 0, k, dlam.as<uint32_t>()));
  MPVSS_TRY(timing_end(ctx));
  const float ms_lambda = ctx->last_ms;
  const int launches_lambda = ctx->last_launches;
  std::vector<uint32_t> negf(parts * k);
  MPVSS_TRY(d2h(ctx, lam.data(), dlam, k * EB));
  MPVSS_TRY(d2h(ctx, negf.data(), dneg, parts * k * 4));
  MPVSS_TRY(sync(ctx));
  for (size_t i = 0; i < k; ++i) {
    for (size_t p = 1; p < parts; ++p) negf[i] ^= negf[p * k + i];
    if (!negf[i]) continue;
    big::Int l = big::from_le(lam.data() + i * EB, EB);
    if (!big::is_zero(l)) big::to_le(big::sub(ctx->qm1, l), lam.data() + i * EB, EB);
  }
  uint8_t gs[EB];
  MPVSS_TRY(multi_exp(ctx, shares, lam.data(), k, gs));
  ctx->last_ms += ms_lambda;
  ctx->last_launches += launches_lambda;
  uint8_t tmp[EB], hs[32];
  size_t len = min_be(gs, tmp);
  sha2::sha256(tmp, len, hs);
  big::Int mask = big::mod(big::from_be(hs, 32), ctx->q);
  big::to_be(big::bxor(mask, big::from_be(u, EB)), secret_out, EB);
  if (gs_out) memcpy(gs_out, gs, EB);
  return MPVSS_OK;
}

int reconstruct_batch(mpvss_ctx* ctx, size_t nb, const size_t* kv, const int64_t* positions, const uint8_t* shares,
                      const uint8_t* u, uint8_t* secrets_out, uint8_t* gs_out, int* status_out) {
  memset(secrets_out, 0, nb * EB);
  if (gs_out) memset(gs_out, 0, nb * EB);
  ctx->last_ms = 0.f;
  ctx->last_launches = 0;
  std::vector<size_t> live, first(nb);
  for (size_t b = 0, off = 0; b < nb; off += kv[b], ++b) {
    first[b] = off;
    status_out[b] = MPVSS_OK;
    std::vector<int64_t> sorted(positions + off, positions + off + kv[b]);
    std::sort(sorted.begin(), sorted.end());
    if (sorted.front() < 1 || sorted.back() > 0x7fffffff || std::adjacent_find(sorted.begin(), sorted.end()) != sorted.end())
      status_out[b] = MPVSS_ERR_ARG;
    else
      live.push_back(b);
  }
  if (live.empty()) return MPVSS_OK;
  const size_t threshold = live.size() == 1 ? (size_t)ctx->msm_threshold : mpvss_ctx::msm_batch_threshold;
  auto buckets = [&](size_t b) { return ctx->modp_msm == 1 || (ctx->modp_msm == 2 && kv[b] >= threshold); };
  std::stable_partition(live.begin(), live.end(), [&](size_t b) { return !buckets(b); });
  const size_t L = live.size();
  size_t n = 0, n_direct = 0, L_direct = 0, kmax = 0;
  std::vector<uint32_t> start(L), cnt(L);
  for (size_t j = 0; j < L; ++j) {
    start[j] = (uint32_t)n;
    cnt[j] = (uint32_t)kv[live[j]];
    n += cnt[j];
    kmax = std::max<size_t>(kmax, cnt[j]);
    if (!buckets(live[j])) n_direct = n, L_direct = j + 1;
  }
  std::vector<uint32_t> idx(3 * n);
  std::vector<uint8_t> host(n * EB);
  for (size_t j = 0; j < L; ++j) {
    const size_t b = live[j];
    for (uint32_t i = 0; i < cnt[j]; ++i) {
      idx[start[j] + i] = (uint32_t)positions[first[b] + i];
      idx[n + start[j] + i] = start[j];
      idx[2 * n + start[j] + i] = cnt[j];
    }
    memcpy(host.data() + (size_t)start[j] * EB, shares + first[b] * EB, cnt[j] * EB);
  }
  DevBuf &dshares = ctx->buf(0), &dexp = ctx->buf(1), &dpow = ctx->buf(2), &dplan = ctx->buf(4), &didx = ctx->buf(10),
         &dord = ctx->buf(11), &dnum = ctx->buf(12), &dden = ctx->buf(13), &dneg = ctx->buf(14), &dinv = ctx->buf(20);
  std::vector<uint32_t> order(EW, 0);
  for (size_t i = 0; i < ctx->qm1.size(); ++i) order[i] = ctx->qm1[i];
  MPVSS_TRY(h2d(ctx, didx, idx.data(), 3 * n * 4));
  MPVSS_TRY(h2d(ctx, dord, order.data(), EB));
  MPVSS_TRY(h2d(ctx, dshares, host.data(), n * EB));
  const size_t parts = kmax >= 64 ? 8 : 1;
  for (DevBuf* b : {&dnum, &dden}) MPVSS_CUDA(ctx, b->ensure(parts * n * EB));
  MPVSS_CUDA(ctx, dinv.ensure(n * EB));
  MPVSS_CUDA(ctx, dneg.ensure(parts * n * 4));
  MPVSS_CUDA(ctx, dpow.ensure(n * EB));
  const uint32_t* K = ctx->consts_q.as<uint32_t>();
  const uint32_t* Kg = ctx->consts_g.as<uint32_t>();
  const uint32_t* di = didx.as<uint32_t>();
  modp::LagrangeBoxesArgs LA{dord.as<uint32_t>(), di, di + n, di + 2 * n, dnum.as<uint32_t>(), dden.as<uint32_t>(),
                             dneg.as<uint32_t>(), (uint32_t)n, (uint32_t)parts};
  timing_begin(ctx);
  MPVSS_CUDA(ctx, modp::launch_lagrange_boxes(LA, ctx->stream));
  timing_launch(ctx);
  for (size_t half = parts / 2; half >= 1; half /= 2)
    for (DevBuf* b : {&dnum, &dden})
      MPVSS_TRY(dev_mul(ctx, Kg, b->as<uint32_t>(), EW, b->as<uint32_t>() + half * n * EW, EW, 0, half * n,
                        b->as<uint32_t>()));
  MPVSS_TRY(dev_batch_inverse_g(ctx, dden.as<uint32_t>(), n, dinv.as<uint32_t>()));
  MPVSS_TRY(dev_mul(ctx, Kg, dnum.as<uint32_t>(), EW, dinv.as<uint32_t>(), EW, 0, n, dnum.as<uint32_t>()));
  MPVSS_TRY(timing_end(ctx));
  const float ms_lambda = ctx->last_ms;
  const int launches_lambda = ctx->last_launches;
  std::vector<uint8_t> lam(n * EB);
  std::vector<uint32_t> negf(parts * n);
  MPVSS_TRY(d2h(ctx, lam.data(), dnum, n * EB));
  MPVSS_TRY(d2h(ctx, negf.data(), dneg, parts * n * 4));
  MPVSS_TRY(sync(ctx));
  for (size_t i = 0; i < n; ++i) {
    for (size_t p = 1; p < parts; ++p) negf[i] ^= negf[p * n + i];
    if (!negf[i]) continue;
    big::Int l = big::from_le(lam.data() + i * EB, EB);
    if (!big::is_zero(l)) big::to_le(big::sub(ctx->qm1, l), lam.data() + i * EB, EB);
  }
  MPVSS_TRY(h2d(ctx, dexp, lam.data(), n * EB));
  std::vector<uint32_t> rows(3 * n_direct), level_end;
  {
    std::vector<uint32_t> c(cnt.begin(), cnt.begin() + L_direct);
    for (size_t m = 0, total = 0; (m = modp::product_tree_level(start.data(), c.data(), (uint32_t)L_direct,
                                                                rows.data() + 3 * total)) > 0;) {
      total += m;
      level_end.push_back((uint32_t)total);
    }
  }
  if (!level_end.empty()) MPVSS_TRY(h2d(ctx, dplan, rows.data(), (size_t)level_end.back() * 3 * 4));
  timing_begin(ctx);
  if (n_direct) {
    MPVSS_TRY(dev_exp2(ctx, K, dshares.as<uint32_t>(), EW, dexp.as<uint32_t>(), EW, windows_for(lam.data(), EB, n_direct),
                       nullptr, 0, nullptr, 0, 0, n_direct, dpow.as<uint32_t>()));
    for (size_t l = 0; l < level_end.size(); ++l) {
      const uint32_t lo = l ? level_end[l - 1] : 0;
      modp::MulRowsArgs MA{K, dpow.as<uint32_t>(), dplan.as<uint32_t>() + 3 * lo, level_end[l] - lo};
      MPVSS_CUDA(ctx, modp::launch_mul_rows(ctx->modp_tpi, MA, ctx->stream));
      timing_launch(ctx);
    }
  }
  for (size_t j = L_direct; j < L; ++j) {
    DevBuf vb, ve, vo;
    vb.p = dshares.as<uint32_t>() + (size_t)start[j] * EW;
    ve.p = dexp.as<uint32_t>() + (size_t)start[j] * EW;
    vo.p = dpow.as<uint32_t>() + (size_t)start[j] * EW;
    const uint32_t windows = (windows_for(lam.data() + (size_t)start[j] * EB, EB, cnt[j]) + 1) / 2;
    MPVSS_TRY(multi_exp_buckets(ctx, vb, ve, windows, cnt[j], vo));
  }
  MPVSS_TRY(timing_end(ctx));
  ctx->last_ms += ms_lambda;
  ctx->last_launches += launches_lambda;
  MPVSS_TRY(d2h(ctx, host.data(), dpow, n * EB));
  MPVSS_TRY(sync(ctx));
  for (size_t j = 0; j < L; ++j) {
    const size_t b = live[j];
    const uint8_t* gs = host.data() + (size_t)start[j] * EB;
    uint8_t tmp[EB], hs[32];
    sha2::sha256(tmp, min_be(gs, tmp), hs);
    big::Int mask = big::mod(big::from_be(hs, 32), ctx->q);
    big::to_be(big::bxor(mask, big::from_be(u + b * EB, EB)), secrets_out + b * EB, EB);
    if (gs_out) memcpy(gs_out + b * EB, gs, EB);
  }
  return MPVSS_OK;
}

}
```

mpvss_rs_b200/csrc/modp_arith.cuh:

```cuda
#pragma once
#include "simt.h"

namespace modp {

template <int TPI>
struct Cfg {
  static_assert(TPI == 4 || TPI == 8 || TPI == 16, "TPI must be 4, 8 or 16");
  static constexpr int L = 64 / TPI;
};

template <int L>
struct Mod {
  uint32_t q[L];
  uint32_t nq[L];
  uint32_t np;
  const uint32_t* qh;
};

struct Lane {
  int k;
  int lane0;
  int shift;
  uint32_t gmask;
};

template <int TPI>
MP_DEV Lane make_lane() {
  Lane ln;
  int wl = (int)simt::lane_id();
  ln.k = wl & (TPI - 1);
  ln.lane0 = wl - ln.k;
  ln.shift = ln.lane0;
  ln.gmask = (TPI == 32) ? 0xffffffffu : ((1u << TPI) - 1u);
  return ln;
}

template <int TPI>
MP_DEV uint32_t resolve(const Lane& ln, bool gen, bool prop, uint32_t* cout) {
  uint32_t G = (simt::ballot(gen) >> ln.shift) & ln.gmask;
  uint32_t P = (simt::ballot(prop) >> ln.shift) & ln.gmask;
  uint32_t C = ((G | P) + G) ^ P;
  *cout = (C >> TPI) & 1u;
  return (C >> ln.k) & 1u;
}

template <int L>
MP_DEV bool all_ones(const uint32_t (&r)[L]) {
  uint32_t x = r[0];
#pragma unroll
  for (int i = 1; i < L; ++i) x &= r[i];
  return x == 0xffffffffu;
}

template <int TPI>
MP_DEV uint32_t add_resolve(uint32_t (&r)[Cfg<TPI>::L], const uint32_t (&x)[Cfg<TPI>::L], uint32_t mask,
                            const Lane& ln) {
  constexpr int L = Cfg<TPI>::L;
  r[0] = simt::add_cc(r[0], x[0] & mask);
#pragma unroll
  for (int i = 1; i < L; ++i) r[i] = simt::addc_cc(r[i], x[i] & mask);
  uint32_t c = simt::addc(0, 0);
  uint32_t cout;
  uint32_t cin = resolve<TPI>(ln, c != 0, all_ones<L>(r), &cout);
  r[0] = simt::add_cc(r[0], cin);
#pragma unroll
  for (int i = 1; i < L; ++i) r[i] = simt::addc_cc(r[i], 0);
  return cout;
}

template <int TPI, bool FIRST>
MP_DEV void mm_digit(uint32_t (&P)[Cfg<TPI>::L + 2], uint32_t (&S)[Cfg<TPI>::L + 2],
                     const uint32_t (&a)[Cfg<TPI>::L], uint32_t b, const Mod<Cfg<TPI>::L>& M, const Lane& ln,
                     uint32_t& in) {
  constexpr int L = Cfg<TPI>::L;
  if (FIRST) {
#pragma unroll
    for (int i = 0; i < L; i += 2) {
      P[i] = simt::mul_lo(a[i], b);
      P[i + 1] = simt::mul_hi(a[i], b);
      S[i] = simt::mul_lo(a[i + 1], b);
      S[i + 1] = simt::mul_hi(a[i + 1], b);
    }
    P[L] = P[L + 1] = 0;
    S[L] = S[L + 1] = 0;
  } else {
    S[L] = simt::add_cc(S[L], in);
    S[L + 1] = simt::addc(S[L + 1], 0);
    P[0] = simt::add_cc(P[0], S[1]);
#pragma unroll
    for (int x = 0; x < L; x += 2) {
      S[x] = simt::madc_lo_cc(a[x + 1], b, S[x + 2]);
      S[x + 1] = simt::madc_hi_cc(a[x + 1], b, S[x + 3]);
    }
    S[L] = simt::addc(0, 0);
    S[L + 1] = 0;
    P[0] = simt::mad_lo_cc(a[0], b, P[0]);
    P[1] = simt::madc_hi_cc(a[0], b, P[1]);
#pragma unroll
    for (int i = 2; i < L; i += 2) {
      P[i] = simt::madc_lo_cc(a[i], b, P[i]);
      P[i + 1] = simt::madc_hi_cc(a[i], b, P[i + 1]);
    }
    P[L] = simt::addc(P[L], 0);
  }
  uint32_t m = simt::shfl(simt::mul_lo(P[0], M.np), ln.lane0);
  S[0] = simt::mad_lo_cc(M.q[1], m, S[0]);
  S[1] = simt::madc_hi_cc(M.q[1], m, S[1]);
#pragma unroll
  for (int i = 3; i < L; i += 2) {
    S[i - 1] = simt::madc_lo_cc(M.q[i], m, S[i - 1]);
    S[i] = simt::madc_hi_cc(M.q[i], m, S[i]);
  }
  S[L] = simt::addc(S[L], 0);
  P[0] = simt::mad_lo_cc(M.q[0], m, P[0]);
  P[1] = simt::madc_hi_cc(M.q[0], m, P[1]);
#pragma unroll
  for (int i = 2; i < L; i += 2) {
    P[i] = simt::madc_lo_cc(M.q[i], m, P[i]);
    P[i + 1] = simt::madc_hi_cc(M.q[i], m, P[i + 1]);
  }
  P[L] = simt::addc(P[L], 0);
  in = simt::shfl(P[0], ((int)simt::lane_id() + 1) & 31);
}

template <int TPI, bool DOUBLE = false>
MP_DEV void mm_finish(uint32_t (&r)[Cfg<TPI>::L], const uint32_t (&A0)[Cfg<TPI>::L + 2],
                      const uint32_t (&A1)[Cfg<TPI>::L + 2], uint32_t in, const Mod<Cfg<TPI>::L>& M, const Lane& ln) {
  constexpr int L = Cfg<TPI>::L;
  r[0] = simt::add_cc(A0[0], A1[1]);
#pragma unroll
  for (int i = 1; i < L; ++i) r[i] = simt::addc_cc(A0[i], A1[i + 1]);
  uint32_t ov = simt::addc(A0[L], A1[L + 1]);
  r[L - 1] = simt::add_cc(r[L - 1], in);
  ov = simt::addc(ov, 0);
  uint32_t ovin = simt::shfl(ov, (int)simt::lane_id() - 1);
  uint32_t ovtop = simt::shfl(ov, ln.lane0 + TPI - 1);
  if (ln.k == 0) ovin = 0;
  r[0] = simt::add_cc(r[0], ovin);
#pragma unroll
  for (int i = 1; i < L; ++i) r[i] = simt::addc_cc(r[i], 0);
  uint32_t c = simt::addc(0, 0);
  uint32_t cout;
  uint32_t cin = resolve<TPI>(ln, c != 0, all_ones<L>(r), &cout);
  r[0] = simt::add_cc(r[0], cin);
#pragma unroll
  for (int i = 1; i < L; ++i) r[i] = simt::addc_cc(r[i], 0);
  uint32_t over = ovtop + cout;
  if (!DOUBLE) {
    (void)add_resolve<TPI>(r, M.nq, 0u - over, ln);
  } else {
    uint32_t top = r[L - 1] >> 31;
    uint32_t bit_in = simt::shfl(top, ((int)simt::lane_id() - 1) & 31);
    uint32_t top_all = simt::shfl(top, ln.lane0 + TPI - 1);
    if (ln.k == 0) bit_in = 0;
#pragma unroll
    for (int i = L - 1; i >= 1; --i) r[i] = (r[i] << 1) | (r[i - 1] >> 31);
    r[0] = (r[0] << 1) | bit_in;
    uint32_t over2 = 2u * over + top_all;
    uint32_t m1 = over2 ? 0xffffffffu : 0u;
    uint32_t c1 = add_resolve<TPI>(r, M.nq, m1, ln);
    over2 = over2 - (m1 & 1u) + c1;
    (void)add_resolve<TPI>(r, M.nq, over2 ? 0xffffffffu : 0u, ln);
  }
}

template <int TPI>
MP_DEV void mont_mul_fused(uint32_t (&r)[Cfg<TPI>::L], const uint32_t (&a)[Cfg<TPI>::L], const uint32_t* bs,
                           const Mod<Cfg<TPI>::L>& M, const Lane& ln) {
  constexpr int L = Cfg<TPI>::L;
  uint32_t A0[L + 2], A1[L + 2];
  uint32_t in = 0;
  constexpr int PER = L + 2, PEEL = 64 % PER;
  static_assert(PEEL >= 2 && PEEL % 2 == 0 && PER % 2 == 0, "digit loop layout");
  const uint2* b2 = reinterpret_cast<const uint2*>(bs);
  {
    uint2 bw = b2[0];
    mm_digit<TPI, true>(A0, A1, a, bw.x, M, ln, in);
    mm_digit<TPI, false>(A1, A0, a, bw.y, M, ln, in);
  }
#pragma unroll
  for (int d = 2; d < PEEL; d += 2) {
    uint2 bw = b2[d / 2];
    mm_digit<TPI, false>(A0, A1, a, bw.x, M, ln, in);
    mm_digit<TPI, false>(A1, A0, a, bw.y, M, ln, in);
  }
#ifndef MPVSS_MODP_UNROLL
#define MPVSS_MODP_UNROLL 2
#endif
  constexpr int UNROLL = MPVSS_MODP_UNROLL;
#pragma unroll UNROLL
  for (int it = 0; it < (64 - PEEL) / PER; ++it) {
    const uint2* p = b2 + (PEEL + it * PER) / 2;
#pragma unroll
    for (int d = 0; d < PER; d += 2) {
      uint2 bw = p[d / 2];
      mm_digit<TPI, false>(A0, A1, a, bw.x, M, ln, in);
      mm_digit<TPI, false>(A1, A0, a, bw.y, M, ln, in);
    }
  }
  mm_finish<TPI>(r, A0, A1, in, M, ln);
}

template <int TPI>
MP_DEV void mm_digit_il(uint32_t (&AP)[Cfg<TPI>::L + 2], uint32_t (&AS)[Cfg<TPI>::L + 2],
                        uint32_t (&QP)[Cfg<TPI>::L + 2], uint32_t (&QS)[Cfg<TPI>::L + 2],
                        const uint32_t (&a)[Cfg<TPI>::L], uint32_t b, const Mod<Cfg<TPI>::L>& M, const Lane& ln,
                        uint32_t& in, uint32_t& cprev) {
  constexpr int L = Cfg<TPI>::L;
  AS[L] = simt::add_cc(AS[L], in);
  AS[L + 1] = simt::addc(AS[L + 1], 0);
  AP[0] = simt::add_cc(AP[0], AS[1]);
#pragma unroll
  for (int x = 0; x < L; x += 2) {
    AS[x] = simt::madc_lo_cc(a[x + 1], b, AS[x + 2]);
    AS[x + 1] = simt::madc_hi_cc(a[x + 1], b, AS[x + 3]);
  }
  AS[L] = simt::addc(0, 0);
  AS[L + 1] = 0;
  AP[0] = simt::mad_lo_cc(a[0], b, AP[0]);
  AP[1] = simt::madc_hi_cc(a[0], b, AP[1]);
#pragma unroll
  for (int i = 2; i < L; i += 2) {
    AP[i] = simt::madc_lo_cc(a[i], b, AP[i]);
    AP[i + 1] = simt::madc_hi_cc(a[i], b, AP[i + 1]);
  }
  AP[L] = simt::addc(AP[L], 0);
  uint32_t m = simt::shfl(simt::mul_lo(AP[0] + QP[0] + QS[1] + cprev, M.np), ln.lane0);
  QP[0] = simt::add_cc(QP[0], QS[1]);
  QS[0] = simt::madc_lo_cc(M.q[1], m, QS[2]);
  QS[1] = simt::madc_hi_cc(M.q[1], m, QS[3]);
#pragma unroll
  for (int i = 3; i < L; i += 2) {
    QS[i - 1] = simt::madc_lo_cc(M.q[i], m, QS[i + 1]);
    QS[i] = simt::madc_hi_cc(M.q[i], m, QS[i + 2]);
  }
  QS[L] = simt::addc(0, 0);
  QS[L + 1] = 0;
  QP[0] = simt::mad_lo_cc(M.q[0], m, QP[0]);
  QP[1] = simt::madc_hi_cc(M.q[0], m, QP[1]);
#pragma unroll
  for (int i = 2; i < L; i += 2) {
    QP[i] = simt::madc_lo_cc(M.q[i], m, QP[i]);
    QP[i + 1] = simt::madc_hi_cc(M.q[i], m, QP[i + 1]);
  }
  QP[L] = simt::addc(QP[L], 0);
  uint32_t e = simt::add_cc(AP[0], QP[0]);
  uint32_t c = simt::addc(0, 0);
  e = simt::add_cc(e, cprev);
  cprev = simt::addc(c, 0);
  in = simt::shfl(e, ((int)simt::lane_id() + 1) & 31);
}

template <int TPI>
MP_DEV void mont_mul_il(uint32_t (&r)[Cfg<TPI>::L], const uint32_t (&a)[Cfg<TPI>::L], const uint32_t* bs,
                        const Mod<Cfg<TPI>::L>& M, const Lane& ln) {
  constexpr int L = Cfg<TPI>::L;
  uint32_t A0[L + 2], A1[L + 2], Q0[L + 2], Q1[L + 2];
#pragma unroll
  for (int i = 0; i < L + 2; ++i) A0[i] = A1[i] = Q0[i] = Q1[i] = 0;
  uint32_t in = 0, cprev = 0;
  constexpr int PER = L + 2, PEEL = 64 % PER;
  const uint2* b2 = reinterpret_cast<const uint2*>(bs);
#pragma unroll
  for (int d = 0; d < PEEL; d += 2) {
    uint2 bw = b2[d / 2];
    mm_digit_il<TPI>(A0, A1, Q0, Q1, a, bw.x, M, ln, in, cprev);
    mm_digit_il<TPI>(A1, A0, Q1, Q0, a, bw.y, M, ln, in, cprev);
  }
#pragma unroll 1
  for (int it = 0; it < (64 - PEEL) / PER; ++it) {
    const uint2* p = b2 + (PEEL + it * PER) / 2;
#pragma unroll
    for (int d = 0; d < PER; d += 2) {
      uint2 bw = p[d / 2];
      mm_digit_il<TPI>(A0, A1, Q0, Q1, a, bw.x, M, ln, in, cprev);
      mm_digit_il<TPI>(A1, A0, Q1, Q0, a, bw.y, M, ln, in, cprev);
    }
  }
  A0[0] = simt::add_cc(A0[0], cprev);
#pragma unroll
  for (int i = 1; i < L + 1; ++i) A0[i] = simt::addc_cc(A0[i], 0);
  A0[L + 1] = simt::addc(A0[L + 1], 0);
  A0[0] = simt::add_cc(A0[0], Q0[0]);
#pragma unroll
  for (int i = 1; i < L + 1; ++i) A0[i] = simt::addc_cc(A0[i], Q0[i]);
  A0[L + 1] = simt::addc(A0[L + 1], Q0[L + 1]);
  A1[1] = simt::add_cc(A1[1], Q1[1]);
#pragma unroll
  for (int i = 2; i < L + 1; ++i) A1[i] = simt::addc_cc(A1[i], Q1[i]);
  A1[L + 1] = simt::addc(A1[L + 1], Q1[L + 1]);
  mm_finish<TPI>(r, A0, A1, in, M, ln);
}

template <int TPI>
MP_DEV void mont_mul(uint32_t (&r)[Cfg<TPI>::L], const uint32_t (&a)[Cfg<TPI>::L], const uint32_t* bs,
                     const Mod<Cfg<TPI>::L>& M, const Lane& ln) {
#ifdef MPVSS_MODP_SPLIT_ACC
  mont_mul_il<TPI>(r, a, bs, M, ln);
#else
  mont_mul_fused<TPI>(r, a, bs, M, ln);
#endif
}

struct SqMasks {
  uint32_t gt, ge, eq, prev;
};

template <int TPI, int RP>
MP_DEV void sq_digit(uint32_t (&P)[Cfg<TPI>::L + 2], uint32_t (&S)[Cfg<TPI>::L + 2],
                     const uint32_t (&a)[Cfg<TPI>::L], const uint32_t (&h)[2 * Cfg<TPI>::L], uint32_t pbn31,
                     uint32_t b, const SqMasks& mk, const Mod<Cfg<TPI>::L>& M, const Lane& ln, uint32_t& in) {
  constexpr int L = Cfg<TPI>::L;
  constexpr int H = L / 2;
  if (RP == 0) {
    P[0] = simt::add_cc(P[0], h[0] & mk.eq);
#pragma unroll
    for (int i = 1; i <= L + 1; ++i) {
      uint32_t v = h[i] & mk.eq;
      if (i == L - 1) v |= pbn31 & mk.prev;
      P[i] = simt::addc_cc(P[i], v);
    }
  } else if (RP == L - 2) {
    P[4] = simt::add_cc(P[4], h[L + 2] & mk.eq);
#pragma unroll
    for (int i = 5; i <= L + 1; ++i) P[i] = simt::addc_cc(P[i], h[L - 2 + i] & mk.eq);
  }
  const uint32_t b_tie = b & (RP < H ? mk.ge : mk.gt);
  const uint32_t b_gt = b & mk.gt;
  S[L] = simt::add_cc(S[L], in);
  S[L + 1] = simt::addc(S[L + 1], 0);
  P[0] = simt::add_cc(P[0], S[1]);
#pragma unroll
  for (int x = 0; x < L; x += 2) {
    const int sl = (x + 1 - RP + L) % L;
    if (sl <= H) {
      const uint32_t d = sl == 0 ? b_gt : (sl == H ? b_tie : b);
      S[x] = simt::madc_lo_cc(a[x + 1], d, S[x + 2]);
      S[x + 1] = simt::madc_hi_cc(a[x + 1], d, S[x + 3]);
    } else {
      S[x] = simt::addc_cc(S[x + 2], 0);
      S[x + 1] = simt::addc_cc(S[x + 3], 0);
    }
  }
  S[L] = simt::addc(0, 0);
  S[L + 1] = 0;
  bool started = false;
#pragma unroll
  for (int i = 0; i < L; i += 2) {
    const int sl = (i - RP + L) % L;
    if (sl <= H) {
      const uint32_t d = sl == 0 ? b_gt : (sl == H ? b_tie : b);
      P[i] = started ? simt::madc_lo_cc(a[i], d, P[i]) : simt::mad_lo_cc(a[i], d, P[i]);
      P[i + 1] = simt::madc_hi_cc(a[i], d, P[i + 1]);
      started = true;
    } else if (started) {
      P[i] = simt::addc_cc(P[i], 0);
      P[i + 1] = simt::addc_cc(P[i + 1], 0);
    }
  }
  P[L] = simt::addc_cc(P[L], 0);
  P[L + 1] = simt::addc(P[L + 1], 0);
  uint32_t m = simt::shfl(simt::mul_lo(P[0], M.np), ln.lane0);
  S[0] = simt::mad_lo_cc(M.q[1], m, S[0]);
  S[1] = simt::madc_hi_cc(M.q[1], m, S[1]);
#pragma unroll
  for (int i = 3; i < L; i += 2) {
    S[i - 1] = simt::madc_lo_cc(M.q[i], m, S[i - 1]);
    S[i] = simt::madc_hi_cc(M.q[i], m, S[i]);
  }
  S[L] = simt::addc(S[L], 0);
  P[0] = simt::mad_lo_cc(M.q[0], m, P[0]);
  P[1] = simt::madc_hi_cc(M.q[0], m, P[1]);
#pragma unroll
  for (int i = 2; i < L; i += 2) {
    P[i] = simt::madc_lo_cc(M.q[i], m, P[i]);
    P[i + 1] = simt::madc_hi_cc(M.q[i], m, P[i + 1]);
  }
  P[L] = simt::addc_cc(P[L], 0);
  P[L + 1] = simt::addc(P[L + 1], 0);
  in = simt::shfl(P[0], ((int)simt::lane_id() + 1) & 31);
}

template <int TPI, int RP, bool END = (RP >= Cfg<TPI>::L)>
struct SqRows {
  static MP_DEV void run(uint32_t (&A0)[Cfg<TPI>::L + 2], uint32_t (&A1)[Cfg<TPI>::L + 2],
                         const uint32_t (&a)[Cfg<TPI>::L], const uint32_t (&h)[2 * Cfg<TPI>::L], uint32_t pbn31,
                         const uint2* bp, const SqMasks& mk, const Mod<Cfg<TPI>::L>& M, const Lane& ln,
                         uint32_t& in) {
    uint2 bw = bp[RP / 2];
    sq_digit<TPI, RP>(A0, A1, a, h, pbn31, bw.x, mk, M, ln, in);
    sq_digit<TPI, RP + 1>(A1, A0, a, h, pbn31, bw.y, mk, M, ln, in);
    SqRows<TPI, RP + 2>::run(A0, A1, a, h, pbn31, bp, mk, M, ln, in);
  }
};
template <int TPI, int RP>
struct SqRows<TPI, RP, true> {
  static MP_DEV void run(uint32_t (&)[Cfg<TPI>::L + 2], uint32_t (&)[Cfg<TPI>::L + 2], const uint32_t (&)[Cfg<TPI>::L],
                         const uint32_t (&)[2 * Cfg<TPI>::L], uint32_t, const uint2*, const SqMasks&,
                         const Mod<Cfg<TPI>::L>&, const Lane&, uint32_t&) {}
};

template <int TPI>
MP_DEV void mont_sqr(uint32_t (&r)[Cfg<TPI>::L], const uint32_t (&a)[Cfg<TPI>::L], const uint32_t* as,
                     const Mod<Cfg<TPI>::L>& M, const Lane& ln) {
  constexpr int L = Cfg<TPI>::L;
  uint32_t h[2 * L];
  {
    uint32_t w[2 * L];
#pragma unroll
    for (int i = 0; i < L; ++i) {
      w[2 * i] = simt::mul_lo(a[i], a[i]);
      w[2 * i + 1] = simt::mul_hi(a[i], a[i]);
    }
#pragma unroll
    for (int i = 0; i < 2 * L - 1; ++i) h[i] = (w[i] >> 1) | (w[i + 1] << 31);
    h[2 * L - 1] = w[2 * L - 1] >> 1;
    h[0] |= 0;
    const uint32_t pb = w[0] & 1u;
    const uint32_t pbn = simt::shfl(pb, ((int)simt::lane_id() + 1) & 31);
    const uint32_t pb0 = simt::shfl(pb, ln.lane0);
    uint32_t A0[L + 2], A1[L + 2];
    const uint32_t m0 = 0u - pb0;
#pragma unroll
    for (int i = 0; i < L; ++i) {
      A0[i] = M.qh[ln.k * L + i] & m0;
      A1[i] = 0;
    }
    A0[L] = A0[L + 1] = A1[L] = A1[L + 1] = 0;
    uint32_t in = 0;
    const uint32_t pbn31 = pbn << 31;
    const uint2* b2 = reinterpret_cast<const uint2*>(as);
#pragma unroll 1
    for (int kp = 0; kp < TPI; ++kp) {
      SqMasks mk;
      mk.gt = ln.k > kp ? 0xffffffffu : 0u;
      mk.ge = ln.k >= kp ? 0xffffffffu : 0u;
      mk.eq = ln.k == kp ? 0xffffffffu : 0u;
      mk.prev = ln.k + 1 == kp ? 0xffffffffu : 0u;
      SqRows<TPI, 0>::run(A0, A1, a, h, pbn31, b2 + kp * (L / 2), mk, M, ln, in);
    }
    mm_finish<TPI, true>(r, A0, A1, in, M, ln);
  }
}

template <int TPI>
MP_DEV void mont_mul2(uint32_t (&r0)[Cfg<TPI>::L], const uint32_t (&a0)[Cfg<TPI>::L], const uint32_t* b0s,
                      uint32_t (&r1)[Cfg<TPI>::L], const uint32_t (&a1)[Cfg<TPI>::L], const uint32_t* b1s,
                      const Mod<Cfg<TPI>::L>& M, const Lane& ln) {
  constexpr int L = Cfg<TPI>::L;
  uint32_t A0[L + 2], A1[L + 2], B0[L + 2], B1[L + 2];
  uint32_t in0 = 0, in1 = 0;
  const uint4* p0 = reinterpret_cast<const uint4*>(b0s);
  const uint4* p1 = reinterpret_cast<const uint4*>(b1s);
  {
    uint4 u = p0[0], v = p1[0];
    mm_digit<TPI, true>(A0, A1, a0, u.x, M, ln, in0);
    mm_digit<TPI, true>(B0, B1, a1, v.x, M, ln, in1);
    mm_digit<TPI, false>(A1, A0, a0, u.y, M, ln, in0);
    mm_digit<TPI, false>(B1, B0, a1, v.y, M, ln, in1);
    mm_digit<TPI, false>(A0, A1, a0, u.z, M, ln, in0);
    mm_digit<TPI, false>(B0, B1, a1, v.z, M, ln, in1);
    mm_digit<TPI, false>(A1, A0, a0, u.w, M, ln, in0);
    mm_digit<TPI, false>(B1, B0, a1, v.w, M, ln, in1);
  }
#pragma unroll 1
  for (int j = 1; j < 16; ++j) {
    uint4 u = p0[j], v = p1[j];
    mm_digit<TPI, false>(A0, A1, a0, u.x, M, ln, in0);
    mm_digit<TPI, false>(B0, B1, a1, v.x, M, ln, in1);
    mm_digit<TPI, false>(A1, A0, a0, u.y, M, ln, in0);
    mm_digit<TPI, false>(B1, B0, a1, v.y, M, ln, in1);
    mm_digit<TPI, false>(A0, A1, a0, u.z, M, ln, in0);
    mm_digit<TPI, false>(B0, B1, a1, v.z, M, ln, in1);
    mm_digit<TPI, false>(A1, A0, a0, u.w, M, ln, in0);
    mm_digit<TPI, false>(B1, B0, a1, v.w, M, ln, in1);
  }
  mm_finish<TPI>(r0, A0, A1, in0, M, ln);
  mm_finish<TPI>(r1, B0, B1, in1, M, ln);
}

template <int TPI>
MP_DEV void canonical(uint32_t (&r)[Cfg<TPI>::L], const Mod<Cfg<TPI>::L>& M, const Lane& ln) {
  constexpr int L = Cfg<TPI>::L;
#pragma unroll 1
  for (int pass = 0; pass < 2; ++pass) {
    uint32_t t[L];
#pragma unroll
    for (int i = 0; i < L; ++i) t[i] = r[i];
    uint32_t ge = add_resolve<TPI>(t, M.nq, 0xffffffffu, ln);
    if (ge) {
#pragma unroll
      for (int i = 0; i < L; ++i) r[i] = t[i];
    }
  }
}

template <int TPI>
MP_DEV void stage(uint32_t* dst64, const uint32_t (&v)[Cfg<TPI>::L], const Lane& ln) {
  constexpr int L = Cfg<TPI>::L;
  uint4* d = reinterpret_cast<uint4*>(dst64 + ln.k * L);
#pragma unroll
  for (int i = 0; i < L; i += 4) d[i / 4] = make_uint4(v[i], v[i + 1], v[i + 2], v[i + 3]);
}

template <int TPI>
MP_DEV void stage_shared(uint32_t* dst64, const uint32_t (&v)[Cfg<TPI>::L], const Lane& ln) {
  simt::syncwarp();
  stage<TPI>(dst64, v, ln);
}

template <int TPI>
MP_DEV void load_slice(uint32_t (&v)[Cfg<TPI>::L], const uint32_t* src64, const Lane& ln) {
  constexpr int L = Cfg<TPI>::L;
  const uint4* s = reinterpret_cast<const uint4*>(src64 + ln.k * L);
#pragma unroll
  for (int i = 0; i < L; i += 4) {
    uint4 w = s[i / 4];
    v[i] = w.x;
    v[i + 1] = w.y;
    v[i + 2] = w.z;
    v[i + 3] = w.w;
  }
}

}
```

mpvss_rs_b200/csrc/modp_kernels.cuh:

```cuda
#pragma once
#include "modp_arith.cuh"
#include "modp_sqr.cuh"

namespace modp {

constexpr int GPAD = 8;
enum { C_Q = 0, C_NQ = 64, C_ONE = 128, C_R2 = 192, C_NP = 256, C_QH = 260, C_WORDS = 324 };

template <int TPI>
MP_DEV void load_mod(Mod<Cfg<TPI>::L>& M, const uint32_t* consts, const Lane& ln) {
  load_slice<TPI>(M.q, consts + C_Q, ln);
  load_slice<TPI>(M.nq, consts + C_NQ, ln);
  M.np = consts[C_NP];
  M.qh = consts + C_QH;
}

MP_DEV void warp_copy64(uint32_t* dst, const uint32_t* src) {
  uint32_t l = simt::lane_id();
  simt::syncwarp();
  dst[2 * l] = src[2 * l];
  dst[2 * l + 1] = src[2 * l + 1];
}

#ifdef MPVSS_MODP_SPLIT_SQR
template <int TPI>
constexpr int sqr_scratch_words = TPI == 8 ? SQS_WORDS : 0;
#else
template <int TPI>
constexpr int sqr_scratch_words = 0;
#endif
struct SqrCtx {
  uint32_t* scratch;
  SqPlan pl;
};
template <int TPI>
MP_DEV SqrCtx make_sqr_ctx(uint32_t* scratch, const Lane& ln) {
  SqrCtx c;
  c.scratch = scratch;
  if (sqr_scratch_words<TPI> != 0) {
    c.pl = make_sq_plan(ln.k);
    scratch[SQS_ZERO + ln.k] = 0;
  }
  return c;
}

template <int TPI>
MP_DEV void sqr_plain(uint32_t (&acc)[Cfg<TPI>::L], uint32_t* sq, const Mod<Cfg<TPI>::L>& M, const Lane& ln) {
  stage_shared<TPI>(sq, acc, ln);
  simt::syncwarp();
  mont_mul<TPI>(acc, acc, sq, M, ln);
}

template <int TPI>
MP_DEV void sqr_inplace(uint32_t (&acc)[Cfg<TPI>::L], uint32_t* sq, const SqrCtx& sc, const Mod<Cfg<TPI>::L>& M,
                        const Lane& ln) {
  stage_shared<TPI>(sq, acc, ln);
  simt::syncwarp();
  if constexpr (sqr_scratch_words<TPI> != 0) {
    mont_sqr_split(acc, acc, sq, sc.scratch, sc.pl, M, ln);
  } else {
#ifdef MPVSS_MODP_DEDICATED_SQR
    mont_sqr<TPI>(acc, acc, sq, M, ln);
#else
    mont_mul<TPI>(acc, acc, sq, M, ln);
#endif
  }
}

template <int TPI>
MP_DEV void finish_store(uint32_t (&acc)[Cfg<TPI>::L], uint32_t* sq, uint32_t* dst64, bool live,
                         const Mod<Cfg<TPI>::L>& M, const Lane& ln) {
  constexpr int L = Cfg<TPI>::L;
  uint32_t one[L];
#pragma unroll
  for (int i = 0; i < L; ++i) one[i] = 0;
  if (ln.k == 0) one[0] = 1;
  stage_shared<TPI>(sq, one, ln);
  simt::syncwarp();
  mont_mul<TPI>(acc, acc, sq, M, ln);
  canonical<TPI>(acc, M, ln);
  if (live) stage<TPI>(dst64, acc, ln);
}

struct HornerArgs {
  const uint32_t* consts;
  const uint32_t* cm;
  const uint16_t* ops;
  const uint32_t* slot;
  const uint32_t* nops;
  uint32_t* out;
  uint32_t t, n, nops_all;
  uint32_t warps_per_cta;
  const uint32_t* cfirst;
  const uint32_t* csteps;
};

constexpr int HC_SLOTS = 6;
constexpr int HC_OPS = 48;
constexpr int HC_GSTRIDE = (HC_SLOTS + 2) * 64 + GPAD;

template <int TPI>
constexpr int horner_smem_words = (32 / TPI) * (HC_GSTRIDE + HC_OPS / 2);

template <int TPI, bool NP1 = false, bool CHUNKED = false>
MP_DEV void horner_body(const HornerArgs& A, uint32_t wg, uint32_t* wsm, uint32_t nops, uint32_t cta = 0) {
  const uint32_t first = CHUNKED ? A.cfirst[cta] : A.t - 1, steps = CHUNKED ? A.csteps[cta] : A.t - 1;
  constexpr int L = Cfg<TPI>::L;
  constexpr int GPW = 32 / TPI;
  Lane ln = make_lane<TPI>();
  const int gi = (int)simt::lane_id() / TPI;
  uint32_t inst = wg * GPW + gi;
  const bool live = inst < A.n;
  if (!live) inst = A.n - 1;
  Mod<L> M;
  load_mod<TPI>(M, A.consts, ln);
  if (NP1) M.np = 1u;
  uint32_t* gbase = wsm + gi * HC_GSTRIDE;
  uint16_t* opsm = reinterpret_cast<uint16_t*>(wsm + GPW * HC_GSTRIDE) + gi * HC_OPS;
  for (int k = ln.k; k < HC_OPS; k += TPI) opsm[k] = A.ops[(size_t)inst * HC_OPS + k];
  uint32_t acc[L];
  load_slice<TPI>(acc, A.consts + C_ONE, ln);
  stage<TPI>(gbase + HC_SLOTS * 64, acc, ln);
  load_slice<TPI>(acc, A.cm + (size_t)first * 64, ln);
  simt::syncwarp();
  const uint32_t* cmb = CHUNKED ? A.cm + (size_t)(first - steps) * 64 : A.cm;
  for (int j = (int)steps - 1; j >= 0; --j) {
    {
      uint32_t cj[L];
      load_slice<TPI>(cj, cmb + (size_t)j * 64, ln);
      stage_shared<TPI>(gbase + (HC_SLOTS + 1) * 64, cj, ln);
    }
    uint32_t op = opsm[0];
#pragma unroll 1
    for (uint32_t k = 0; k < nops; ++k) {
      const uint32_t nxt = opsm[k + 1 < (uint32_t)HC_OPS ? k + 1 : k];
      const uint32_t sv = (op >> 8) & 15u, a = (op >> 4) & 15u, b = op & 15u;
      simt::syncwarp();
      if (sv) stage<TPI>(gbase + (sv - 1) * 64, acc, ln);
      simt::syncwarp();
      if (a) load_slice<TPI>(acc, gbase + (a - 1) * 64, ln);
      mont_mul<TPI>(acc, acc, gbase + b * 64, M, ln);
      op = nxt;
    }
  }
  const uint32_t slot = A.slot ? A.slot[inst] : inst;
  finish_store<TPI>(acc, gbase, A.out + (size_t)(slot == 0xffffffffu ? 0 : slot) * 64, live && slot != 0xffffffffu, M,
                    ln);
}

struct Exp2Args {
  const uint32_t* consts;
  const uint32_t* b1;
  const uint32_t* e1;
  const uint32_t* b2;
  const uint32_t* e2;
  uint32_t* out;
  uint32_t n;
  uint32_t b1_stride, e1_stride, e1_windows;
  uint32_t b2_stride, e2_stride, e2_windows;
  const uint32_t* comb1;
};

template <int TPI>
constexpr int exp2_smem_words = 64 + (32 / TPI) * (16 * 64 + 64 + GPAD + sqr_scratch_words<TPI>);

template <int TPI>
MP_DEV void exp_window4(uint32_t (&acc)[Cfg<TPI>::L], const uint32_t* base64, const uint32_t* e, uint32_t windows,
                        uint32_t* tbl, uint32_t* sq, const SqrCtx& sc, const uint32_t* r2, const uint32_t* consts,
                        const Mod<Cfg<TPI>::L>& M, const Lane& ln) {
  constexpr int L = Cfg<TPI>::L;
  uint32_t x[L];
  load_slice<TPI>(x, consts + C_ONE, ln);
  stage_shared<TPI>(tbl, x, ln);
  load_slice<TPI>(x, base64, ln);
  mont_mul<TPI>(x, x, r2, M, ln);
  stage_shared<TPI>(tbl + 64, x, ln);
  simt::syncwarp();
  for (int i = 2; i < 16; ++i) {
    mont_mul<TPI>(x, x, tbl + 64, M, ln);
    stage_shared<TPI>(tbl + i * 64, x, ln);
    simt::syncwarp();
  }
  uint32_t wi = windows - 1;
  uint32_t d = (e[wi >> 3] >> ((wi & 7u) * 4)) & 15u;
  load_slice<TPI>(acc, tbl + d * 64, ln);
  while (wi-- > 0) {
#pragma unroll 1
    for (int rep = 0; rep < 4; ++rep) sqr_inplace<TPI>(acc, sq, sc, M, ln);
    d = (e[wi >> 3] >> ((wi & 7u) * 4)) & 15u;
    mont_mul<TPI>(acc, acc, tbl + d * 64, M, ln);
  }
}

template <int TPI>
MP_DEV void exp_comb8(uint32_t (&acc)[Cfg<TPI>::L], const uint32_t* tbl, const uint32_t* e, uint32_t nbytes,
                      uint32_t* sq, const Mod<Cfg<TPI>::L>& M, const Lane& ln) {
  constexpr int L = Cfg<TPI>::L;
  uint32_t d = e[0] & 0xffu;
  load_slice<TPI>(acc, tbl + (size_t)d * 64, ln);
  for (uint32_t w = 1; w < nbytes; ++w) {
    d = (e[w >> 2] >> ((w & 3u) * 8)) & 0xffu;
    uint32_t x[L];
    load_slice<TPI>(x, tbl + ((size_t)w * 256 + d) * 64, ln);
    stage_shared<TPI>(sq, x, ln);
    simt::syncwarp();
    mont_mul<TPI>(acc, acc, sq, M, ln);
  }
}

struct CombArgs {
  const uint32_t* consts;
  const uint32_t* base;
  uint32_t* tbl;
  uint32_t rows;
};
template <int TPI>
constexpr int comb_smem_words = 64 + (32 / TPI) * (128 + GPAD);

template <int TPI>
MP_DEV void comb1_body(const CombArgs& A, uint32_t wg, uint32_t* wsm) {
  constexpr int L = Cfg<TPI>::L;
  Lane ln = make_lane<TPI>();
  const int gi = (int)simt::lane_id() / TPI;
  Mod<L> M;
  load_mod<TPI>(M, A.consts, ln);
  uint32_t* r2 = wsm;
  uint32_t* sq = wsm + 64 + gi * (128 + GPAD);
  warp_copy64(r2, A.consts + C_R2);
  simt::syncwarp();
  uint32_t b[L];
  load_slice<TPI>(b, A.base, ln);
  mont_mul<TPI>(b, b, r2, M, ln);
  for (uint32_t w = 0; w < A.rows; ++w) {
    if (wg == 0 && gi == 0) stage<TPI>(A.tbl + ((size_t)w * 256 + 1) * 64, b, ln);
    for (int k = 0; k < 8; ++k) sqr_plain<TPI>(b, sq, M, ln);
  }
}
template <int TPI>
MP_DEV void comb2_body(const CombArgs& A, uint32_t wg, uint32_t* wsm) {
  constexpr int L = Cfg<TPI>::L;
  constexpr int GPW = 32 / TPI;
  Lane ln = make_lane<TPI>();
  const int gi = (int)simt::lane_id() / TPI;
  uint32_t w = wg * GPW + gi;
  const bool live = w < A.rows;
  if (!live) w = A.rows - 1;
  Mod<L> M;
  load_mod<TPI>(M, A.consts, ln);
  uint32_t* b1 = wsm + 64 + gi * (128 + GPAD);
  uint32_t* row = A.tbl + (size_t)w * 256 * 64;
  uint32_t x[L];
  load_slice<TPI>(x, A.consts + C_ONE, ln);
  if (live) stage<TPI>(row, x, ln);
  load_slice<TPI>(x, row + 64, ln);
  stage_shared<TPI>(b1, x, ln);
  simt::syncwarp();
  for (uint32_t d = 2; d < 256; ++d) {
    mont_mul<TPI>(x, x, b1, M, ln);
    if (live) stage<TPI>(row + (size_t)d * 64, x, ln);
  }
}

template <int TPI>
MP_DEV void exp2_body(const Exp2Args& A, uint32_t wg, uint32_t* wsm) {
  constexpr int L = Cfg<TPI>::L;
  constexpr int GPW = 32 / TPI;
  Lane ln = make_lane<TPI>();
  const int gi = (int)simt::lane_id() / TPI;
  uint32_t inst = wg * GPW + gi;
  const bool live = inst < A.n;
  if (!live) inst = A.n - 1;
  Mod<L> M;
  load_mod<TPI>(M, A.consts, ln);
  uint32_t* r2 = wsm;
  uint32_t* tbl = wsm + 64 + gi * (16 * 64 + 64 + GPAD + sqr_scratch_words<TPI>);
  uint32_t* sq = tbl + 16 * 64;
  const SqrCtx sc = make_sqr_ctx<TPI>(sq + 64, ln);
  warp_copy64(r2, A.consts + C_R2);
  simt::syncwarp();
  uint32_t acc[L];
  if (A.comb1)
    exp_comb8<TPI>(acc, A.comb1, A.e1 + (size_t)inst * A.e1_stride, (A.e1_windows + 1) / 2, sq, M, ln);
  else
    exp_window4<TPI>(acc, A.b1 + (size_t)inst * A.b1_stride, A.e1 + (size_t)inst * A.e1_stride, A.e1_windows, tbl,
                     sq, sc, r2, A.consts, M, ln);
  if (A.b2 != nullptr) {
    uint32_t acc2[L];
    exp_window4<TPI>(acc2, A.b2 + (size_t)inst * A.b2_stride, A.e2 + (size_t)inst * A.e2_stride, A.e2_windows, tbl,
                     sq, sc, r2, A.consts, M, ln);
    stage_shared<TPI>(sq, acc2, ln);
    simt::syncwarp();
    mont_mul<TPI>(acc, acc, sq, M, ln);
  }
  finish_store<TPI>(acc, sq, A.out + (size_t)inst * 64, live, M, ln);
}

struct FrameArgs {
  const uint32_t *x, *y, *a1, *a2;
  uint8_t* out;
  uint32_t n;
};
constexpr int FRAME_BYTES = 8 + 256;

MP_DEV void frame_body(const FrameArgs& A, uint32_t tid) {
  const uint32_t j = tid >> 2, e = tid & 3u;
  if (j >= A.n) return;
  const uint32_t* src = (e == 0 ? A.x : e == 1 ? A.y : e == 2 ? A.a1 : A.a2) + (size_t)j * 64;
  uint8_t* dst = A.out + ((size_t)j * 4 + e) * FRAME_BYTES;
  int top = 63;
  while (top > 0 && src[top] == 0) --top;
  const uint32_t w = src[top];
  const uint32_t len = (uint32_t)top * 4 + ((w >> 24) ? 4u : (w >> 16) ? 3u : (w >> 8) ? 2u : 1u);
  uint32_t* d32 = reinterpret_cast<uint32_t*>(dst);
  d32[0] = 0;
  d32[1] = ((len & 0xffu) << 24) | ((len >> 8) << 16);
  if (len == 256) {
#pragma unroll 8
    for (int k = 0; k < 64; ++k) {
      const uint32_t v = src[63 - k];
      d32[2 + k] = (v >> 24) | ((v >> 8) & 0xff00u) | ((v << 8) & 0xff0000u) | (v << 24);
    }
  } else {
    for (uint32_t k = 0; k < 256; ++k) {
      const uint32_t b = len - 1 - k;
      dst[8 + k] = k < len ? (uint8_t)(src[b >> 2] >> ((b & 3u) * 8)) : (uint8_t)0;
    }
  }
}

struct PolyArgs {
  const uint32_t* coeffs;
  const uint32_t* order;
  const uint32_t* pos;
  uint32_t* out;
  uint32_t t, n;
};
MP_DEV void poly_body(const PolyArgs& A, uint32_t tid) {
  if (tid >= A.n) return;
  const uint64_t x = A.pos[tid];
  uint32_t acc[64], delta[64];
  {
    uint64_t br = 0;
#pragma unroll
    for (int i = 0; i < 64; ++i) {
      uint64_t d = (uint64_t)0 - A.order[i] - br;
      delta[i] = (uint32_t)d;
      br = (d >> 32) & 1u;
      acc[i] = 0;
    }
  }
#pragma unroll 1
  for (int j = (int)A.t - 1; j >= 0; --j) {
    const uint32_t* a = A.coeffs + (size_t)j * 64;
    uint64_t c = 0;
#pragma unroll
    for (int i = 0; i < 64; ++i) {
      c += (uint64_t)acc[i] * x + a[i];
      acc[i] = (uint32_t)c;
      c >>= 32;
    }
    uint64_t top = c, cc = 0;
#pragma unroll
    for (int i = 0; i < 64; ++i) {
      cc += top * delta[i] + acc[i];
      acc[i] = (uint32_t)cc;
      cc >>= 32;
    }
    uint32_t m = 0u - (uint32_t)cc;
    uint64_t c2 = 0;
#pragma unroll
    for (int i = 0; i < 64; ++i) {
      c2 += (uint64_t)acc[i] + (delta[i] & m);
      acc[i] = (uint32_t)c2;
      c2 >>= 32;
    }
  }
  uint32_t r[64];
  uint64_t br = 0;
#pragma unroll
  for (int i = 0; i < 64; ++i) {
    uint64_t d = (uint64_t)acc[i] - A.order[i] - br;
    r[i] = (uint32_t)d;
    br = (d >> 32) & 1u;
  }
#pragma unroll
  for (int i = 0; i < 64; ++i) A.out[(size_t)tid * 64 + i] = br ? acc[i] : r[i];
}

struct RespArgs {
  const uint32_t* order;
  const uint32_t* alpha;
  const uint32_t* w;
  const uint32_t* c;
  uint32_t* out;
  uint32_t n, alpha_stride, c_stride;
};
MP_DEV void resp_body(const RespArgs& A, uint32_t tid) {
  if (tid >= A.n) return;
  const uint32_t* al = A.alpha + (size_t)tid * A.alpha_stride;
  const uint32_t* cc = A.c + (size_t)tid * A.c_stride;
  uint32_t prod[72], delta[62];
  {
    uint64_t br = 0;
    for (int i = 0; i < 62; ++i) {
      uint64_t d = (uint64_t)0 - A.order[i] - br;
      delta[i] = (uint32_t)d;
      br = (d >> 32) & 1u;
    }
  }
  for (int i = 0; i < 72; ++i) prod[i] = 0;
  for (int j = 0; j < 8; ++j) {
    const uint64_t cj = cc[j];
    uint64_t carry = 0;
    for (int i = 0; i < 64; ++i) {
      carry += (uint64_t)al[i] * cj + prod[i + j];
      prod[i + j] = (uint32_t)carry;
      carry >>= 32;
    }
    prod[64 + j] = (uint32_t)carry;
  }
  for (int pass = 0; pass < 9; ++pass) {
    uint32_t hi[8], any = 0;
    for (int j = 0; j < 8; ++j) {
      hi[j] = prod[64 + j];
      any |= hi[j];
      prod[64 + j] = 0;
    }
    if (!any) break;
    for (int j = 0; j < 8; ++j) {
      const uint64_t hj = hi[j];
      uint64_t carry = 0;
      for (int i = 0; i < 62; ++i) {
        carry += (uint64_t)delta[i] * hj + prod[i + j];
        prod[i + j] = (uint32_t)carry;
        carry >>= 32;
      }
      for (int i = 62 + j; carry && i < 72; ++i) {
        carry += prod[i];
        prod[i] = (uint32_t)carry;
        carry >>= 32;
      }
    }
  }
  uint32_t r[64];
  auto sub_order = [&](uint32_t* v) {
    uint32_t t[64];
    uint64_t br = 0;
    for (int i = 0; i < 64; ++i) {
      uint64_t d = (uint64_t)v[i] - A.order[i] - br;
      t[i] = (uint32_t)d;
      br = (d >> 32) & 1u;
    }
    if (!br)
      for (int i = 0; i < 64; ++i) v[i] = t[i];
  };
  sub_order(prod);
  const uint32_t* w = A.w + (size_t)tid * 64;
  uint64_t br = 0;
  for (int i = 0; i < 64; ++i) {
    uint64_t d = (uint64_t)w[i] - prod[i] - br;
    r[i] = (uint32_t)d;
    br = (d >> 32) & 1u;
  }
  if (br) {
    uint64_t c2 = 0;
    for (int i = 0; i < 64; ++i) {
      c2 += (uint64_t)r[i] + A.order[i];
      r[i] = (uint32_t)c2;
      c2 >>= 32;
    }
  } else {
    sub_order(r);
    sub_order(r);
  }
  for (int i = 0; i < 64; ++i) A.out[(size_t)tid * 64 + i] = r[i];
}

struct LagrangeArgs {
  const uint32_t* order;
  const uint32_t* pos;
  uint32_t* num;
  uint32_t* den;
  uint32_t* negative;
  uint32_t k, parts;
};
MP_DEV void lagrange_product(uint32_t* out64, const LagrangeArgs& A, uint32_t tid, bool denominator, uint32_t* neg,
                             uint32_t j0, uint32_t j1) {
  const uint32_t xi = A.pos[tid];
  uint32_t acc[64], delta[64];
  {
    uint64_t br = 0;
#pragma unroll
    for (int i = 0; i < 64; ++i) {
      uint64_t d = (uint64_t)0 - A.order[i] - br;
      delta[i] = (uint32_t)d;
      br = (d >> 32) & 1u;
      acc[i] = 0;
    }
    acc[0] = 1;
  }
  uint32_t sign = 0;
#pragma unroll 1
  for (uint32_t j = j0; j < j1; ++j) {
    if (j == tid) continue;
    const uint32_t xj = A.pos[j];
    uint64_t f = xj;
    if (denominator) {
      if (xj < xi) {
        sign ^= 1u;
        f = xi - xj;
      } else {
        f = xj - xi;
      }
    }
    uint64_t c = 0;
#pragma unroll
    for (int i = 0; i < 64; ++i) {
      c += (uint64_t)acc[i] * f;
      acc[i] = (uint32_t)c;
      c >>= 32;
    }
    uint64_t top = c, cc = 0;
#pragma unroll
    for (int i = 0; i < 64; ++i) {
      cc += top * delta[i] + acc[i];
      acc[i] = (uint32_t)cc;
      cc >>= 32;
    }
    uint32_t m = 0u - (uint32_t)cc;
    uint64_t c2 = 0;
#pragma unroll
    for (int i = 0; i < 64; ++i) {
      c2 += (uint64_t)acc[i] + (delta[i] & m);
      acc[i] = (uint32_t)c2;
      c2 >>= 32;
    }
  }
  uint64_t br = 0;
  uint32_t r[64];
#pragma unroll
  for (int i = 0; i < 64; ++i) {
    uint64_t d = (uint64_t)acc[i] - A.order[i] - br;
    r[i] = (uint32_t)d;
    br = (d >> 32) & 1u;
  }
#pragma unroll
  for (int i = 0; i < 64; ++i) out64[i] = br ? acc[i] : r[i];
  if (neg) *neg = sign;
}
MP_DEV void lagrange_body(const LagrangeArgs& A, uint32_t tid) {
  const uint32_t P = A.parts ? A.parts : 1u;
  if (tid >= 2u * P * A.k) return;
  const bool denominator = tid >= P * A.k;
  const uint32_t row = denominator ? tid - P * A.k : tid, part = row / A.k, i = row % A.k;
  const uint32_t per = (A.k + P - 1) / P, j0 = part * per, j1 = j0 + per < A.k ? j0 + per : A.k;
  lagrange_product((denominator ? A.den : A.num) + (size_t)row * 64, A, i, denominator,
                   denominator ? A.negative + row : nullptr, j0 < A.k ? j0 : A.k, j1);
}

struct LagrangeBoxesArgs {
  const uint32_t* order;
  const uint32_t* pos;
  const uint32_t* boff;
  const uint32_t* bk;
  uint32_t* num;
  uint32_t* den;
  uint32_t* negative;
  uint32_t n, parts;
};
MP_DEV void lagrange_boxes_body(const LagrangeBoxesArgs& A, uint32_t tid) {
  const uint32_t P = A.parts ? A.parts : 1u;
  if (tid >= 2u * P * A.n) return;
  const bool denominator = tid >= P * A.n;
  const uint32_t row = denominator ? tid - P * A.n : tid, part = row / A.n, i = row % A.n;
  const uint32_t off = A.boff[i], k = A.bk[i];
  const uint32_t per = (k + P - 1) / P, j0 = part * per, j1 = j0 + per < k ? j0 + per : k;
  const LagrangeArgs box{A.order, A.pos + off, nullptr, nullptr, nullptr, k, P};
  lagrange_product((denominator ? A.den : A.num) + (size_t)row * 64, box, i - off, denominator,
                   denominator ? A.negative + row : nullptr, j0 < k ? j0 : k, j1);
}

struct MsmBucketArgs {
  const uint32_t* consts;
  const uint32_t* bases;
  const uint32_t* idx;
  const uint32_t* start;
  uint32_t* buckets;
  uint32_t windows, k;
};
template <int TPI>
constexpr int msm_smem_words = (32 / TPI) * (2 * 64 + GPAD);

template <int TPI>
MP_DEV void msm_bucket_body(const MsmBucketArgs& A, uint32_t wg, uint32_t* wsm) {
  constexpr int L = Cfg<TPI>::L;
  constexpr int GPW = 32 / TPI;
  Lane ln = make_lane<TPI>();
  const int gi = (int)simt::lane_id() / TPI;
  const uint32_t total = A.windows * 255u;
  uint32_t id = wg * GPW + gi;
  const bool live = id < total;
  if (!live) id = total - 1;
  const uint32_t w = id / 255u, d = id % 255u + 1u;
  Mod<L> M;
  load_mod<TPI>(M, A.consts, ln);
  uint32_t* stage_buf = wsm + gi * (2 * 64 + GPAD);
  uint32_t* one = stage_buf + 64;
  uint32_t acc[L], x[L];
  load_slice<TPI>(acc, A.consts + C_ONE, ln);
  stage_shared<TPI>(one, acc, ln);
  const uint32_t lo = A.start[w * 257u + d], hi = A.start[w * 257u + d + 1];
  uint32_t cnt = live ? hi - lo : 0u, mx = cnt;
  for (int off = 16; off >= 1; off >>= 1) {
    uint32_t o = simt::shfl(mx, (int)simt::lane_id() ^ off);
    mx = o > mx ? o : mx;
  }
  simt::syncwarp();
  for (uint32_t j = 0; j < mx; ++j) {
    const bool have = j < cnt;
    if (have) load_slice<TPI>(x, A.bases + (size_t)A.idx[(size_t)w * A.k + lo + j] * 64, ln);
    simt::syncwarp();
    if (have) stage<TPI>(stage_buf, x, ln);
    simt::syncwarp();
    mont_mul<TPI>(acc, acc, have ? stage_buf : one, M, ln);
  }
  if (live) stage<TPI>(A.buckets + ((size_t)w * 256 + d) * 64, acc, ln);
}

struct MsmWindowArgs {
  const uint32_t* consts;
  const uint32_t* buckets;
  uint32_t* wprod;
  uint32_t windows;
};
template <int TPI>
constexpr int msm_window_smem_words = (32 / TPI) * (4 * 64 + GPAD);

template <int TPI>
MP_DEV void msm_window_body(const MsmWindowArgs& A, uint32_t wg, uint32_t* wsm) {
  constexpr int L = Cfg<TPI>::L;
  constexpr int GPW = 32 / TPI;
  constexpr uint32_t SEG = 256 / GPW;
  Lane ln = make_lane<TPI>();
  const uint32_t gi = simt::lane_id() / TPI;
  const uint32_t w = wg < A.windows ? wg : A.windows - 1;
  Mod<L> M;
  load_mod<TPI>(M, A.consts, ln);
  uint32_t* buf = wsm + gi * (4 * 64 + GPAD);
  uint32_t run[L], acc[L], x[L];
  load_slice<TPI>(run, A.consts + C_ONE, ln);
  load_slice<TPI>(acc, A.consts + C_ONE, ln);
  simt::syncwarp();
  for (uint32_t d = SEG; d >= 1; --d) {
    const uint32_t b = gi * SEG + d;
    load_slice<TPI>(x, b < 256u ? A.buckets + ((size_t)w * 256 + b) * 64 : A.consts + C_ONE, ln);
    stage_shared<TPI>(buf, x, ln);
    simt::syncwarp();
    mont_mul<TPI>(run, run, buf, M, ln);
    stage_shared<TPI>(buf + 64, run, ln);
    simt::syncwarp();
    mont_mul<TPI>(acc, acc, buf + 64, M, ln);
  }
  uint32_t y[L];
#pragma unroll
  for (int i = 0; i < L; ++i) y[i] = run[i];
  for (uint32_t q = SEG; q > 1; q >>= 1) sqr_plain<TPI>(y, buf, M, ln);
  stage_shared<TPI>(buf + 128, y, ln);
  load_slice<TPI>(x, A.consts + C_ONE, ln);
  stage_shared<TPI>(buf + 64, x, ln);
  simt::syncwarp();
  for (uint32_t e = 0; e < (uint32_t)GPW - 1; ++e)
    mont_mul<TPI>(acc, acc, e < gi ? buf + 128 : buf + 64, M, ln);
  stage_shared<TPI>(buf + 192, acc, ln);
  simt::syncwarp();
  load_slice<TPI>(acc, wsm + 192, ln);
  for (uint32_t s = 1; s < (uint32_t)GPW; ++s) mont_mul<TPI>(acc, acc, wsm + s * (4 * 64 + GPAD) + 192, M, ln);
  if (wg < A.windows && gi == 0) stage<TPI>(A.wprod + (size_t)w * 64, acc, ln);
}

struct MsmFoldArgs {
  const uint32_t* consts;
  const uint32_t* wprod;
  uint32_t* out;
  uint32_t windows;
};
template <int TPI>
MP_DEV void msm_fold_body(const MsmFoldArgs& A, uint32_t* wsm) {
  constexpr int L = Cfg<TPI>::L;
  Lane ln = make_lane<TPI>();
  const uint32_t gi = simt::lane_id() / TPI;
  Mod<L> M;
  load_mod<TPI>(M, A.consts, ln);
  uint32_t* buf = wsm + gi * (2 * 64 + GPAD);
  uint32_t acc[L], x[L];
  load_slice<TPI>(acc, A.wprod + (size_t)(A.windows - 1) * 64, ln);
  simt::syncwarp();
  for (int w = (int)A.windows - 2; w >= 0; --w) {
#pragma unroll 1
    for (int r = 0; r < 8; ++r) sqr_plain<TPI>(acc, buf, M, ln);
    load_slice<TPI>(x, A.wprod + (size_t)w * 64, ln);
    stage_shared<TPI>(buf, x, ln);
    simt::syncwarp();
    mont_mul<TPI>(acc, acc, buf, M, ln);
  }
  finish_store<TPI>(acc, buf, A.out, gi == 0, M, ln);
}

struct MulArgs {
  const uint32_t* consts;
  const uint32_t* a;
  const uint32_t* b;
  uint32_t* out;
  uint32_t n;
  uint32_t mode;
  uint32_t a_stride, b_stride;
};

template <int TPI>
constexpr int mul_smem_words = 64 + (32 / TPI) * (64 + GPAD);

template <int TPI>
MP_DEV void mul_body(const MulArgs& A, uint32_t wg, uint32_t* wsm) {
  constexpr int L = Cfg<TPI>::L;
  constexpr int GPW = 32 / TPI;
  Lane ln = make_lane<TPI>();
  const int gi = (int)simt::lane_id() / TPI;
  uint32_t inst = wg * GPW + gi;
  const bool live = inst < A.n;
  if (!live) inst = A.n - 1;
  Mod<L> M;
  load_mod<TPI>(M, A.consts, ln);
  uint32_t* r2 = wsm;
  uint32_t* sq = wsm + 64 + gi * (64 + GPAD);
  warp_copy64(r2, A.consts + C_R2);
  simt::syncwarp();
  uint32_t acc[L];
  load_slice<TPI>(acc, A.a + (size_t)inst * A.a_stride, ln);
  if (A.mode == 2) {
    stage_shared<TPI>(sq, acc, ln);
    simt::syncwarp();
    mont_sqr<TPI>(acc, acc, sq, M, ln);
  } else {
    mont_mul<TPI>(acc, acc, r2, M, ln);
  }
  if (A.mode == 0 || A.mode == 3) {
    uint32_t y[L];
    load_slice<TPI>(y, A.b + (size_t)inst * A.b_stride, ln);
    stage_shared<TPI>(sq, y, ln);
    simt::syncwarp();
    if (A.mode == 3)
      mont_mul_il<TPI>(acc, acc, sq, M, ln);
    else
      mont_mul<TPI>(acc, acc, sq, M, ln);
  }
  canonical<TPI>(acc, M, ln);
  if (live) stage<TPI>(A.out + (size_t)inst * 64, acc, ln);
}

struct MulRowsArgs {
  const uint32_t* consts;
  uint32_t* v;
  const uint32_t* rows;
  uint32_t n;
};

template <int TPI>
MP_DEV void mul_rows_body(const MulRowsArgs& A, uint32_t wg, uint32_t* wsm) {
  constexpr int L = Cfg<TPI>::L;
  constexpr int GPW = 32 / TPI;
  Lane ln = make_lane<TPI>();
  const int gi = (int)simt::lane_id() / TPI;
  uint32_t inst = wg * GPW + gi;
  const bool live = inst < A.n;
  if (!live) inst = A.n - 1;
  const uint32_t* t = A.rows + (size_t)inst * 3;
  Mod<L> M;
  load_mod<TPI>(M, A.consts, ln);
  uint32_t* r2 = wsm;
  uint32_t* sq = wsm + 64 + gi * (64 + GPAD);
  warp_copy64(r2, A.consts + C_R2);
  simt::syncwarp();
  uint32_t acc[L], y[L];
  load_slice<TPI>(acc, A.v + (size_t)t[0] * 64, ln);
  load_slice<TPI>(y, A.v + (size_t)t[1] * 64, ln);
  mont_mul<TPI>(acc, acc, r2, M, ln);
  stage_shared<TPI>(sq, y, ln);
  simt::syncwarp();
  mont_mul<TPI>(acc, acc, sq, M, ln);
  canonical<TPI>(acc, M, ln);
  if (live) stage<TPI>(A.v + (size_t)t[2] * 64, acc, ln);
}

inline uint32_t product_tree_level(const uint32_t* start, uint32_t* cnt, uint32_t segments, uint32_t* rows) {
  uint32_t m = 0;
  for (uint32_t s = 0; s < segments; ++s) {
    const uint32_t c = cnt[s], h = (c + 1) / 2;
    for (uint32_t i = 0; i < c / 2; ++i) {
      rows[3 * m] = start[s] + i;
      rows[3 * m + 1] = start[s] + i + h;
      rows[3 * m + 2] = start[s] + i;
      ++m;
    }
    cnt[s] = h;
  }
  return m;
}

constexpr int sqrtest_smem_words = 64 + 4 * (64 + SQS_WORDS);
MP_DEV void sqr_split_test_body(const MulArgs& A, uint32_t wg, uint32_t* wsm) {
  constexpr int TPI = 8, L = 8, GPW = 4;
  Lane ln = make_lane<TPI>();
  const int gi = (int)simt::lane_id() / TPI;
  uint32_t inst = wg * GPW + gi;
  const bool live = inst < A.n;
  if (!live) inst = A.n - 1;
  Mod<L> M;
  load_mod<TPI>(M, A.consts, ln);
  uint32_t* sq = wsm + 64 + gi * (64 + SQS_WORDS);
  uint32_t* scratch = sq + 64;
  scratch[SQS_ZERO + ln.k] = 0;
  const SqPlan pl = make_sq_plan(ln.k);
  uint32_t acc[L];
  load_slice<TPI>(acc, A.a + (size_t)inst * A.a_stride, ln);
  for (uint32_t rep = 0; rep < (A.mode ? A.mode : 1u); ++rep) {
    stage_shared<TPI>(sq, acc, ln);
    simt::syncwarp();
    mont_sqr_split(acc, acc, sq, scratch, pl, M, ln);
  }
  canonical<TPI>(acc, M, ln);
  if (live) stage<TPI>(A.out + (size_t)inst * 64, acc, ln);
}

}
```

mpvss_rs_b200/csrc/modp_launch.h:

```cpp
#pragma once
#include <cuda_runtime.h>
#include "modp_kernels.cuh"

namespace modp {
constexpr int WARPS_PER_CTA = 4;
constexpr int HORNER_MAX_WARPS_PER_CTA = 4;
cudaError_t launch_horner(int tpi, const HornerArgs& A, bool np_is_one, cudaStream_t s);
cudaError_t launch_exp2(int tpi, const Exp2Args& A, cudaStream_t s);
cudaError_t launch_exp2_filler(int tpi, const Exp2Args& A, size_t ctas, cudaStream_t s);
cudaError_t launch_frames(const FrameArgs& A, cudaStream_t s);
cudaError_t launch_resp(const RespArgs& A, cudaStream_t s);
cudaError_t launch_comb_build(int tpi, const CombArgs& A, cudaStream_t s);
cudaError_t launch_poly(const PolyArgs& A, cudaStream_t s);
cudaError_t launch_lagrange(const LagrangeArgs& A, cudaStream_t s);
cudaError_t launch_lagrange_boxes(const LagrangeBoxesArgs& A, cudaStream_t s);
cudaError_t launch_mul(int tpi, const MulArgs& A, cudaStream_t s);
cudaError_t launch_mul_rows(int tpi, const MulRowsArgs& A, cudaStream_t s);
cudaError_t launch_msm(const MsmBucketArgs& B, const uint32_t* scalars, uint32_t* idx, uint32_t* start, uint32_t* wprod,
                       uint32_t* out, cudaStream_t s);
}
```

Before: 18280.

## Specialize Montgomery reduction for moduli with low 64 bits all ones

```diff
diff --git a/mpvss_rs_b200/csrc/ctx.h b/mpvss_rs_b200/csrc/ctx.h
--- a/mpvss_rs_b200/csrc/ctx.h
+++ b/mpvss_rs_b200/csrc/ctx.h
@@ -89,7 +89,7 @@
   static constexpr size_t msm_batch_threshold = 4096;
   bool device_hash = false;
   bool validate = false;
-  bool modp_np1 = false;
+  bool modp_q64 = false;
   size_t ec_threads = 0;
   DevBuf ec_comb;
   DevBuf ec_consts;
diff --git a/mpvss_rs_b200/csrc/modp.cu b/mpvss_rs_b200/csrc/modp.cu
--- a/mpvss_rs_b200/csrc/modp.cu
+++ b/mpvss_rs_b200/csrc/modp.cu
@@ -5,46 +5,46 @@
 namespace modp {
 
 
-template <int TPI, bool NP1, bool CHUNKED>
+template <int TPI, bool Q64, bool CHUNKED>
 __global__ void __launch_bounds__(HORNER_MAX_WARPS_PER_CTA * 32) horner_kernel(HornerArgs A) {
   extern __shared__ __align__(16) uint32_t smem[];
   uint32_t w = threadIdx.x >> 5;
-  horner_body<TPI, NP1, CHUNKED>(A, blockIdx.x * (blockDim.x >> 5) + w, smem + w * horner_smem_words<TPI>,
+  horner_body<TPI, Q64, CHUNKED>(A, blockIdx.x * (blockDim.x >> 5) + w, smem + w * horner_smem_words<TPI>,
                                  A.nops ? A.nops[blockIdx.x] : A.nops_all, blockIdx.x);
 }
 
-template <int TPI>
+template <int TPI, bool Q64>
 __global__ void __launch_bounds__(WARPS_PER_CTA * 32) exp2_kernel(Exp2Args A) {
   extern __shared__ __align__(16) uint32_t smem[];
   uint32_t w = threadIdx.x >> 5;
-  exp2_body<TPI>(A, blockIdx.x * WARPS_PER_CTA + w, smem + w * exp2_smem_words<TPI>);
-}
-
-template <int TPI>
+  exp2_body<TPI, Q64>(A, blockIdx.x * WARPS_PER_CTA + w, smem + w * exp2_smem_words<TPI>);
+}
+
+template <int TPI, bool Q64>
 __global__ void __launch_bounds__(32) exp2_filler_kernel(Exp2Args A, uint32_t nwarps) {
   extern __shared__ __align__(16) uint32_t smem[];
   for (uint32_t w = blockIdx.x; w < nwarps; w += gridDim.x) {
-    exp2_body<TPI>(A, w, smem);
+    exp2_body<TPI, Q64>(A, w, smem);
     __syncwarp();
   }
 }
 
-template <int TPI>
+template <int TPI, bool Q64>
 __global__ void __launch_bounds__(32) comb1_kernel(CombArgs A) {
   extern __shared__ __align__(16) uint32_t smem[];
-  comb1_body<TPI>(A, blockIdx.x, smem);
-}
-template <int TPI>
+  comb1_body<TPI, Q64>(A, blockIdx.x, smem);
+}
+template <int TPI, bool Q64>
 __global__ void __launch_bounds__(32) comb2_kernel(CombArgs A) {
   extern __shared__ __align__(16) uint32_t smem[];
-  comb2_body<TPI>(A, blockIdx.x, smem);
-}
-
-template <int TPI>
+  comb2_body<TPI, Q64>(A, blockIdx.x, smem);
+}
+
+template <int TPI, bool Q64>
 __global__ void __launch_bounds__(WARPS_PER_CTA * 32) mul_kernel(MulArgs A) {
   extern __shared__ __align__(16) uint32_t smem[];
   uint32_t w = threadIdx.x >> 5;
-  mul_body<TPI>(A, blockIdx.x * WARPS_PER_CTA + w, smem + w * mul_smem_words<TPI>);
+  mul_body<TPI, Q64>(A, blockIdx.x * WARPS_PER_CTA + w, smem + w * mul_smem_words<TPI>);
 }
 
 __global__ void __launch_bounds__(128) frame_kernel(FrameArgs A) { frame_body(A, blockIdx.x * 128 + threadIdx.x); }
@@ -55,11 +55,11 @@
   lagrange_boxes_body(A, blockIdx.x * 64 + threadIdx.x);
 }
 
-template <int TPI>
+template <int TPI, bool Q64>
 __global__ void __launch_bounds__(WARPS_PER_CTA * 32) mul_rows_kernel(MulRowsArgs A) {
   extern __shared__ __align__(16) uint32_t smem[];
   uint32_t w = threadIdx.x >> 5;
-  mul_rows_body<TPI>(A, blockIdx.x * WARPS_PER_CTA + w, smem + w * mul_smem_words<TPI>);
+  mul_rows_body<TPI, Q64>(A, blockIdx.x * WARPS_PER_CTA + w, smem + w * mul_smem_words<TPI>);
 }
 
 __global__ void __launch_bounds__(256) msm_sort_kernel(const uint8_t* scalars, uint32_t k, uint32_t* idx, uint32_t* start) {
@@ -81,21 +81,21 @@
     idx[(size_t)w * k + atomicAdd(&cur[scalars[(size_t)i * 256 + w]], 1u)] = i;
 }
 
-template <int TPI>
+template <int TPI, bool Q64>
 __global__ void __launch_bounds__(WARPS_PER_CTA * 32) msm_bucket_kernel(MsmBucketArgs A) {
   extern __shared__ __align__(16) uint32_t smem[];
   uint32_t w = threadIdx.x >> 5;
-  msm_bucket_body<TPI>(A, blockIdx.x * WARPS_PER_CTA + w, smem + w * msm_smem_words<TPI>);
-}
-template <int TPI>
+  msm_bucket_body<TPI, Q64>(A, blockIdx.x * WARPS_PER_CTA + w, smem + w * msm_smem_words<TPI>);
+}
+template <int TPI, bool Q64>
 __global__ void __launch_bounds__(32) msm_window_kernel(MsmWindowArgs A) {
   extern __shared__ __align__(16) uint32_t smem[];
-  msm_window_body<TPI>(A, blockIdx.x, smem);
-}
-template <int TPI>
+  msm_window_body<TPI, Q64>(A, blockIdx.x, smem);
+}
+template <int TPI, bool Q64>
 __global__ void __launch_bounds__(32) msm_fold_kernel(MsmFoldArgs A) {
   extern __shared__ __align__(16) uint32_t smem[];
-  msm_fold_body<TPI>(A, smem);
+  msm_fold_body<TPI, Q64>(A, smem);
 }
 
 template <int TPI>
@@ -119,15 +119,19 @@
     case 16: { constexpr int T = 16; __VA_ARGS__; break; } \
     default: return cudaErrorInvalidValue;                 \
   }
-
-template <int TPI, bool NP1, bool CHUNKED>
+#define MODP_DISPATCH_Q(tpi, q64, ...)                                               \
+  MODP_DISPATCH(tpi, {                                                               \
+    if (q64) { constexpr bool Q = true; __VA_ARGS__; } else { constexpr bool Q = false; __VA_ARGS__; } \
+  })
+
+template <int TPI, bool Q64, bool CHUNKED>
 static cudaError_t horner_go(const HornerArgs& A, uint32_t grid, uint32_t wpc, size_t sm, cudaStream_t s) {
-  cudaError_t e = set_smem(horner_kernel<TPI, NP1, CHUNKED>, sm);
+  cudaError_t e = set_smem(horner_kernel<TPI, Q64, CHUNKED>, sm);
   if (e != cudaSuccess) return e;
-  horner_kernel<TPI, NP1, CHUNKED><<<grid, wpc * 32, sm, s>>>(A);
+  horner_kernel<TPI, Q64, CHUNKED><<<grid, wpc * 32, sm, s>>>(A);
   return cudaSuccess;
 }
-cudaError_t launch_horner(int tpi, const HornerArgs& A, bool np_is_one, cudaStream_t s) {
+cudaError_t launch_horner(int tpi, const HornerArgs& A, bool q64, cudaStream_t s) {
   if (A.n == 0 || A.t == 0 || A.warps_per_cta > (uint32_t)HORNER_MAX_WARPS_PER_CTA) return cudaErrorInvalidValue;
   MODP_DISPATCH(tpi, {
     const uint32_t wpc = A.warps_per_cta ? A.warps_per_cta : 1u;
@@ -135,33 +139,33 @@
     uint32_t per_cta = wpc * (32 / T);
     uint32_t grid = (A.n + per_cta - 1) / per_cta;
     const bool chunked = A.cfirst && A.csteps;
-    cudaError_t e = np_is_one ? (chunked ? horner_go<T, true, true>(A, grid, wpc, sm, s) : horner_go<T, true, false>(A, grid, wpc, sm, s))
-                              : (chunked ? horner_go<T, false, true>(A, grid, wpc, sm, s) : horner_go<T, false, false>(A, grid, wpc, sm, s));
-    if (e != cudaSuccess) return e;
-  });
-  return cudaGetLastError();
-}
-
-cudaError_t launch_exp2(int tpi, const Exp2Args& A, cudaStream_t s) {
+    cudaError_t e = q64 ? (chunked ? horner_go<T, true, true>(A, grid, wpc, sm, s) : horner_go<T, true, false>(A, grid, wpc, sm, s))
+                        : (chunked ? horner_go<T, false, true>(A, grid, wpc, sm, s) : horner_go<T, false, false>(A, grid, wpc, sm, s));
+    if (e != cudaSuccess) return e;
+  });
+  return cudaGetLastError();
+}
+
+cudaError_t launch_exp2(int tpi, const Exp2Args& A, bool q64, cudaStream_t s) {
   if (A.n == 0 || A.e1_windows == 0 || (A.b2 && A.e2_windows == 0)) return cudaErrorInvalidValue;
-  MODP_DISPATCH(tpi, {
+  MODP_DISPATCH_Q(tpi, q64, {
     size_t sm = WARPS_PER_CTA * exp2_smem_words<T> * 4;
-    cudaError_t e = set_smem(exp2_kernel<T>, sm);
-    if (e != cudaSuccess) return e;
-    exp2_kernel<T><<<ctas_for<T>(A.n), WARPS_PER_CTA * 32, sm, s>>>(A);
-  });
-  return cudaGetLastError();
-}
-
-cudaError_t launch_exp2_filler(int tpi, const Exp2Args& A, size_t ctas, cudaStream_t s) {
+    cudaError_t e = set_smem(exp2_kernel<T, Q>, sm);
+    if (e != cudaSuccess) return e;
+    exp2_kernel<T, Q><<<ctas_for<T>(A.n), WARPS_PER_CTA * 32, sm, s>>>(A);
+  });
+  return cudaGetLastError();
+}
+
+cudaError_t launch_exp2_filler(int tpi, const Exp2Args& A, bool q64, size_t ctas, cudaStream_t s) {
   if (A.n == 0 || A.e1_windows == 0 || (A.b2 && A.e2_windows == 0)) return cudaErrorInvalidValue;
-  MODP_DISPATCH(tpi, {
+  MODP_DISPATCH_Q(tpi, q64, {
     size_t sm = exp2_smem_words<T> * 4;
-    cudaError_t e = set_smem(exp2_filler_kernel<T>, sm);
+    cudaError_t e = set_smem(exp2_filler_kernel<T, Q>, sm);
     if (e != cudaSuccess) return e;
     uint32_t per_cta = 32 / T, nwarps = (A.n + per_cta - 1) / per_cta;
     uint32_t grid = (uint32_t)ctas;
-    exp2_filler_kernel<T><<<grid < nwarps ? grid : nwarps, 32, sm, s>>>(A, nwarps);
+    exp2_filler_kernel<T, Q><<<grid < nwarps ? grid : nwarps, 32, sm, s>>>(A, nwarps);
   });
   return cudaGetLastError();
 }
@@ -198,50 +202,56 @@
   return cudaGetLastError();
 }
 
-cudaError_t launch_comb_build(int tpi, const CombArgs& A, cudaStream_t s) {
-  MODP_DISPATCH(tpi, {
+cudaError_t launch_comb_build(int tpi, const CombArgs& A, bool q64, cudaStream_t s) {
+  MODP_DISPATCH_Q(tpi, q64, {
     size_t sm = comb_smem_words<T> * 4;
-    comb1_kernel<T><<<1, 32, sm, s>>>(A);
-    comb2_kernel<T><<<(A.rows + 32 / T - 1) / (32 / T), 32, sm, s>>>(A);
-  });
-  return cudaGetLastError();
-}
-
-cudaError_t launch_msm(const MsmBucketArgs& B, const uint32_t* scalars, uint32_t* idx, uint32_t* start,
-                       uint32_t* wprod, uint32_t* out, cudaStream_t s) {
-  if (B.windows == 0 || B.windows > 256 || B.k == 0) return cudaErrorInvalidValue;
+    comb1_kernel<T, Q><<<1, 32, sm, s>>>(A);
+    comb2_kernel<T, Q><<<(A.rows + 32 / T - 1) / (32 / T), 32, sm, s>>>(A);
+  });
+  return cudaGetLastError();
+}
+
+template <bool Q64>
+static cudaError_t msm_go(const MsmBucketArgs& B, const uint32_t* scalars, uint32_t* idx, uint32_t* start,
+                          uint32_t* wprod, uint32_t* out, cudaStream_t s) {
   constexpr int T = 8;
   msm_sort_kernel<<<B.windows, 256, 0, s>>>(reinterpret_cast<const uint8_t*>(scalars), B.k, idx, start);
   const uint32_t groups = B.windows * 255u, per_cta = WARPS_PER_CTA * (32 / T);
   size_t sm = WARPS_PER_CTA * msm_smem_words<T> * 4;
-  msm_bucket_kernel<T><<<(groups + per_cta - 1) / per_cta, WARPS_PER_CTA * 32, sm, s>>>(B);
+  msm_bucket_kernel<T, Q64><<<(groups + per_cta - 1) / per_cta, WARPS_PER_CTA * 32, sm, s>>>(B);
   MsmWindowArgs W{B.consts, B.buckets, wprod, B.windows};
-  msm_window_kernel<T><<<B.windows, 32, msm_window_smem_words<T> * 4, s>>>(W);
+  msm_window_kernel<T, Q64><<<B.windows, 32, msm_window_smem_words<T> * 4, s>>>(W);
   MsmFoldArgs F{B.consts, wprod, out, B.windows};
-  msm_fold_kernel<T><<<1, 32, msm_smem_words<T> * 4, s>>>(F);
-  return cudaGetLastError();
-}
-
-cudaError_t launch_mul(int tpi, const MulArgs& A, cudaStream_t s) {
-  if (A.n == 0) return cudaErrorInvalidValue;
-  MODP_DISPATCH(tpi, {
+  msm_fold_kernel<T, Q64><<<1, 32, msm_smem_words<T> * 4, s>>>(F);
+  return cudaGetLastError();
+}
+
+cudaError_t launch_msm(const MsmBucketArgs& B, const uint32_t* scalars, uint32_t* idx, uint32_t* start,
+                       uint32_t* wprod, uint32_t* out, bool q64, cudaStream_t s) {
+  if (B.windows == 0 || B.windows > 256 || B.k == 0) return cudaErrorInvalidValue;
+  return q64 ? msm_go<true>(B, scalars, idx, start, wprod, out, s) : msm_go<false>(B, scalars, idx, start, wprod, out, s);
+}
+
+cudaError_t launch_mul(int tpi, const MulArgs& A, bool q64, cudaStream_t s) {
+  if (A.n == 0) return cudaErrorInvalidValue;
+  MODP_DISPATCH_Q(tpi, q64, {
     size_t sm = WARPS_PER_CTA * mul_smem_words<T> * 4;
-    cudaError_t e = set_smem(mul_kernel<T>, sm);
-    if (e != cudaSuccess) return e;
-    mul_kernel<T><<<ctas_for<T>(A.n), WARPS_PER_CTA * 32, sm, s>>>(A);
-  });
-  return cudaGetLastError();
-}
-
-cudaError_t launch_mul_rows(int tpi, const MulRowsArgs& A, cudaStream_t s) {
-  if (A.n == 0) return cudaErrorInvalidValue;
-  MODP_DISPATCH(tpi, {
+    cudaError_t e = set_smem(mul_kernel<T, Q>, sm);
+    if (e != cudaSuccess) return e;
+    mul_kernel<T, Q><<<ctas_for<T>(A.n), WARPS_PER_CTA * 32, sm, s>>>(A);
+  });
+  return cudaGetLastError();
+}
+
+cudaError_t launch_mul_rows(int tpi, const MulRowsArgs& A, bool q64, cudaStream_t s) {
+  if (A.n == 0) return cudaErrorInvalidValue;
+  MODP_DISPATCH_Q(tpi, q64, {
     size_t sm = WARPS_PER_CTA * mul_smem_words<T> * 4;
-    cudaError_t e = set_smem(mul_rows_kernel<T>, sm);
-    if (e != cudaSuccess) return e;
-    mul_rows_kernel<T><<<ctas_for<T>(A.n), WARPS_PER_CTA * 32, sm, s>>>(A);
-  });
-  return cudaGetLastError();
-}
-
-}
+    cudaError_t e = set_smem(mul_rows_kernel<T, Q>, sm);
+    if (e != cudaSuccess) return e;
+    mul_rows_kernel<T, Q><<<ctas_for<T>(A.n), WARPS_PER_CTA * 32, sm, s>>>(A);
+  });
+  return cudaGetLastError();
+}
+
+}
diff --git a/mpvss_rs_b200/csrc/modp_api.cu b/mpvss_rs_b200/csrc/modp_api.cu
--- a/mpvss_rs_b200/csrc/modp_api.cu
+++ b/mpvss_rs_b200/csrc/modp_api.cu
@@ -99,21 +99,25 @@
   return MPVSS_OK;
 }
 
+bool q64(const mpvss_ctx* ctx, const uint32_t* consts) {
+  return ctx->modp_q64 && consts == ctx->consts_q.as<uint32_t>();
+}
+
 int dev_exp2(mpvss_ctx* ctx, const uint32_t* consts, const uint32_t* b1, uint32_t b1s, const uint32_t* e1,
              uint32_t e1s, uint32_t e1w, const uint32_t* b2, uint32_t b2s, const uint32_t* e2, uint32_t e2s,
              uint32_t e2w, size_t n, uint32_t* out, cudaStream_t stream = nullptr, const uint32_t* comb1 = nullptr) {
   modp::Exp2Args A{consts, b1, e1, b2, e2, out, (uint32_t)n, b1s, e1s, e1w, b2s, e2s, e2w, comb1};
   if (ctx->exp2_filler_ctas)
-    MPVSS_CUDA(ctx, modp::launch_exp2_filler(ctx->modp_tpi, A, ctx->exp2_filler_ctas, stream ? stream : ctx->stream));
+    MPVSS_CUDA(ctx, modp::launch_exp2_filler(ctx->modp_tpi, A, q64(ctx, consts), ctx->exp2_filler_ctas, stream ? stream : ctx->stream));
   else
-    MPVSS_CUDA(ctx, modp::launch_exp2(ctx->modp_tpi, A, stream ? stream : ctx->stream));
+    MPVSS_CUDA(ctx, modp::launch_exp2(ctx->modp_tpi, A, q64(ctx, consts), stream ? stream : ctx->stream));
   timing_launch(ctx);
   return MPVSS_OK;
 }
 int dev_mul(mpvss_ctx* ctx, const uint32_t* consts, const uint32_t* a, uint32_t as, const uint32_t* b, uint32_t bs,
             uint32_t mode, size_t n, uint32_t* out) {
   modp::MulArgs A{consts, a, b, out, (uint32_t)n, mode, as, bs};
-  MPVSS_CUDA(ctx, modp::launch_mul(ctx->modp_tpi, A, ctx->stream));
+  MPVSS_CUDA(ctx, modp::launch_mul(ctx->modp_tpi, A, q64(ctx, consts), ctx->stream));
   timing_launch(ctx);
   return MPVSS_OK;
 }
@@ -125,7 +129,7 @@
   if (!t.p) {
     MPVSS_CUDA(ctx, t.ensure((size_t)256 * 256 * EB));
     modp::CombArgs A{ctx->consts_q.as<uint32_t>(), ctx->gens.as<uint32_t>() + which * 64, t.as<uint32_t>(), 256};
-    MPVSS_CUDA(ctx, modp::launch_comb_build(ctx->modp_tpi, A, ctx->stream));
+    MPVSS_CUDA(ctx, modp::launch_comb_build(ctx->modp_tpi, A, q64(ctx, A.consts), ctx->stream));
     MPVSS_CUDA(ctx, cudaStreamSynchronize(ctx->stream));
   }
   *out = t.as<uint32_t>();
@@ -147,7 +151,7 @@
   ctx->g = big::shr1(ctx->qm1);
   std::vector<uint32_t> blk(modp::C_WORDS);
   fill_consts(ctx->q, blk.data());
-  ctx->modp_np1 = blk[modp::C_NP] == 1u;
+  ctx->modp_q64 = blk[modp::C_Q] == 0xffffffffu && blk[modp::C_Q + 1] == 0xffffffffu;
   MPVSS_TRY(h2d(ctx, ctx->consts_q, blk.data(), blk.size() * 4));
   fill_consts(ctx->g, blk.data());
   MPVSS_TRY(h2d(ctx, ctx->consts_g, blk.data(), blk.size() * 4));
@@ -387,7 +391,7 @@
   modp::HornerArgs A{Kq, cm.as<uint32_t>(), P.ops, P.slot, P.nops, h, (uint32_t)t, (uint32_t)P.n_padded, 0,
                      (uint32_t)P.wpc, arrays ? P.first : nullptr, arrays ? P.steps : nullptr};
   MPVSS_CUDA(ctx, cudaEventRecord(ctx->ev_h0, ctx->stream));
-  MPVSS_CUDA(ctx, modp::launch_horner(P.tpi, A, ctx->modp_np1, ctx->stream));
+  MPVSS_CUDA(ctx, modp::launch_horner(P.tpi, A, ctx->modp_q64, ctx->stream));
   MPVSS_CUDA(ctx, cudaEventRecord(ctx->ev_h1, ctx->stream));
   timing_launch(ctx);
   if (P.K > 1) {
@@ -508,7 +512,7 @@
   modp::MsmBucketArgs B{K, dm.as<uint32_t>(), didx.as<uint32_t>(), dst.as<uint32_t>(), dbk.as<uint32_t>(), windows,
                         (uint32_t)n};
   MPVSS_CUDA(ctx, modp::launch_msm(B, de.as<uint32_t>(), didx.as<uint32_t>(), dst.as<uint32_t>(), dwp.as<uint32_t>(),
-                                   dout.as<uint32_t>(), ctx->stream));
+                                   dout.as<uint32_t>(), q64(ctx, B.consts), ctx->stream));
   timing_launch(ctx, 4);
   return MPVSS_OK;
 }
@@ -1312,7 +1316,7 @@
     for (size_t l = 0; l < level_end.size(); ++l) {
       const uint32_t lo = l ? level_end[l - 1] : 0;
       modp::MulRowsArgs MA{K, dpow.as<uint32_t>(), dplan.as<uint32_t>() + 3 * lo, level_end[l] - lo};
-      MPVSS_CUDA(ctx, modp::launch_mul_rows(ctx->modp_tpi, MA, ctx->stream));
+      MPVSS_CUDA(ctx, modp::launch_mul_rows(ctx->modp_tpi, MA, q64(ctx, MA.consts), ctx->stream));
       timing_launch(ctx);
     }
   }
diff --git a/mpvss_rs_b200/csrc/modp_arith.cuh b/mpvss_rs_b200/csrc/modp_arith.cuh
--- a/mpvss_rs_b200/csrc/modp_arith.cuh
+++ b/mpvss_rs_b200/csrc/modp_arith.cuh
@@ -124,6 +124,9 @@
 }
 
 template <int TPI, bool DOUBLE = false>
+MP_DEV void mm_resolve(uint32_t (&r)[Cfg<TPI>::L], uint32_t ov, const Mod<Cfg<TPI>::L>& M, const Lane& ln);
+
+template <int TPI, bool DOUBLE = false>
 MP_DEV void mm_finish(uint32_t (&r)[Cfg<TPI>::L], const uint32_t (&A0)[Cfg<TPI>::L + 2],
                       const uint32_t (&A1)[Cfg<TPI>::L + 2], uint32_t in, const Mod<Cfg<TPI>::L>& M, const Lane& ln) {
   constexpr int L = Cfg<TPI>::L;
@@ -133,6 +136,12 @@
   uint32_t ov = simt::addc(A0[L], A1[L + 1]);
   r[L - 1] = simt::add_cc(r[L - 1], in);
   ov = simt::addc(ov, 0);
+  mm_resolve<TPI, DOUBLE>(r, ov, M, ln);
+}
+
+template <int TPI, bool DOUBLE>
+MP_DEV void mm_resolve(uint32_t (&r)[Cfg<TPI>::L], uint32_t ov, const Mod<Cfg<TPI>::L>& M, const Lane& ln) {
+  constexpr int L = Cfg<TPI>::L;
   uint32_t ovin = simt::shfl(ov, (int)simt::lane_id() - 1);
   uint32_t ovtop = simt::shfl(ov, ln.lane0 + TPI - 1);
   if (ln.k == 0) ovin = 0;
@@ -202,6 +211,121 @@
 }
 
 template <int TPI>
+MP_DEV void mm_step64(uint32_t (&E)[Cfg<TPI>::L + 3], uint32_t (&O)[Cfg<TPI>::L + 2], const uint32_t (&a)[Cfg<TPI>::L],
+                      uint32_t b0, uint32_t b1, const Mod<Cfg<TPI>::L>& M, const Lane& ln) {
+  constexpr int L = Cfg<TPI>::L;
+  const uint32_t x0 = E[0];
+  const uint32_t x1 = simt::add_cc(E[1], O[0]);
+  E[2] = simt::addc_cc(E[2], O[1]);
+#pragma unroll
+  for (int x = 0; x < L; x += 2) {
+    O[x] = simt::madc_lo_cc(a[x + 1], b0, O[x + 2]);
+    O[x + 1] = simt::madc_hi_cc(a[x + 1], b0, O[x + 3]);
+  }
+  O[L] = simt::addc(0, 0);
+  O[0] = simt::mad_lo_cc(a[0], b1, O[0]);
+  O[1] = simt::madc_hi_cc(a[0], b1, O[1]);
+#pragma unroll
+  for (int x = 2; x < L; x += 2) {
+    O[x] = simt::madc_lo_cc(a[x], b1, O[x]);
+    O[x + 1] = simt::madc_hi_cc(a[x], b1, O[x + 1]);
+  }
+  O[L] = simt::addc(O[L], 0);
+  E[0] = simt::mad_lo_cc(a[0], b0, E[2]);
+  E[1] = simt::madc_hi_cc(a[0], b0, E[3]);
+#pragma unroll
+  for (int i = 2; i < L; i += 2) {
+    E[i] = simt::madc_lo_cc(a[i], b0, E[i + 2]);
+    E[i + 1] = simt::madc_hi_cc(a[i], b0, E[i + 3]);
+  }
+  E[L] = simt::addc(E[L + 2], 0);
+  E[L + 1] = E[L + 2] = 0;
+  const int up = ((int)simt::lane_id() + 1) & 31;
+  const uint32_t in0 = simt::shfl(x0, up), in1 = simt::shfl(x1, up);
+  E[L - 2] = simt::add_cc(E[L - 2], in0);
+  E[L - 1] = simt::addc_cc(E[L - 1], in1);
+  E[L] = simt::addc(E[L], 0);
+  const uint32_t Q0 = simt::shfl(E[0], ln.lane0), Q1 = simt::shfl(E[1] + O[0], ln.lane0);
+  E[0] = simt::mad_lo_cc(M.q[0], Q0, E[0]);
+  E[1] = simt::madc_hi_cc(M.q[0], Q0, E[1]);
+#pragma unroll
+  for (int i = 2; i < L; i += 2) {
+    E[i] = simt::madc_lo_cc(M.q[i], Q0, E[i]);
+    E[i + 1] = simt::madc_hi_cc(M.q[i], Q0, E[i + 1]);
+  }
+  E[L] = simt::addc(E[L], 0);
+  E[2] = simt::mad_lo_cc(a[1], b1, E[2]);
+  E[3] = simt::madc_hi_cc(a[1], b1, E[3]);
+#pragma unroll
+  for (int i = 3; i < L; i += 2) {
+    E[i + 1] = simt::madc_lo_cc(a[i], b1, E[i + 1]);
+    E[i + 2] = simt::madc_hi_cc(a[i], b1, E[i + 2]);
+  }
+  E[L + 2] = simt::addc(0, 0);
+  E[2] = simt::mad_lo_cc(M.q[1], Q1, E[2]);
+  E[3] = simt::madc_hi_cc(M.q[1], Q1, E[3]);
+#pragma unroll
+  for (int i = 3; i < L; i += 2) {
+    E[i + 1] = simt::madc_lo_cc(M.q[i], Q1, E[i + 1]);
+    E[i + 2] = simt::madc_hi_cc(M.q[i], Q1, E[i + 2]);
+  }
+  E[L + 2] = simt::addc(E[L + 2], 0);
+  O[0] = simt::mad_lo_cc(M.q[1], Q0, O[0]);
+  O[1] = simt::madc_hi_cc(M.q[1], Q0, O[1]);
+#pragma unroll
+  for (int i = 3; i < L; i += 2) {
+    O[i - 1] = simt::madc_lo_cc(M.q[i], Q0, O[i - 1]);
+    O[i] = simt::madc_hi_cc(M.q[i], Q0, O[i]);
+  }
+  O[L] = simt::addc(O[L], 0);
+  O[0] = simt::mad_lo_cc(M.q[0], Q1, O[0]);
+  O[1] = simt::madc_hi_cc(M.q[0], Q1, O[1]);
+#pragma unroll
+  for (int i = 2; i < L; i += 2) {
+    O[i] = simt::madc_lo_cc(M.q[i], Q1, O[i]);
+    O[i + 1] = simt::madc_hi_cc(M.q[i], Q1, O[i + 1]);
+  }
+  O[L] = simt::addc(O[L], 0);
+}
+
+template <int TPI>
+MP_DEV void mont_mul_q64(uint32_t (&r)[Cfg<TPI>::L], const uint32_t (&a)[Cfg<TPI>::L], const uint32_t* bs,
+                         const Mod<Cfg<TPI>::L>& M, const Lane& ln) {
+  constexpr int L = Cfg<TPI>::L;
+  uint32_t E[L + 3], O[L + 2];
+#pragma unroll
+  for (int i = 0; i < L + 2; ++i) E[i] = O[i] = 0;
+  E[L + 2] = 0;
+  constexpr int PER = 16, PEEL = 32 % PER;
+  const uint2* b2 = reinterpret_cast<const uint2*>(bs);
+#pragma unroll
+  for (int s = 0; s < PEEL; ++s) {
+    const uint2 bw = b2[s];
+    mm_step64<TPI>(E, O, a, bw.x, bw.y, M, ln);
+  }
+#pragma unroll 1
+  for (int it = 0; it < (32 - PEEL) / PER; ++it) {
+    const uint2* p = b2 + PEEL + it * PER;
+#pragma unroll
+    for (int s = 0; s < PER; ++s) {
+      const uint2 bw = p[s];
+      mm_step64<TPI>(E, O, a, bw.x, bw.y, M, ln);
+    }
+  }
+  const uint32_t x0 = E[0];
+  const uint32_t x1 = simt::add_cc(E[1], O[0]);
+#pragma unroll
+  for (int c = 0; c < L; ++c) r[c] = simt::addc_cc(E[c + 2], O[c + 1]);
+  uint32_t ov = simt::addc(E[L + 2], 0);
+  const int up = ((int)simt::lane_id() + 1) & 31;
+  const uint32_t in0 = simt::shfl(x0, up), in1 = simt::shfl(x1, up);
+  r[L - 2] = simt::add_cc(r[L - 2], in0);
+  r[L - 1] = simt::addc_cc(r[L - 1], in1);
+  ov = simt::addc(ov, 0);
+  mm_resolve<TPI>(r, ov, M, ln);
+}
+
+template <int TPI>
 MP_DEV void mm_digit_il(uint32_t (&AP)[Cfg<TPI>::L + 2], uint32_t (&AS)[Cfg<TPI>::L + 2],
                         uint32_t (&QP)[Cfg<TPI>::L + 2], uint32_t (&QS)[Cfg<TPI>::L + 2],
                         const uint32_t (&a)[Cfg<TPI>::L], uint32_t b, const Mod<Cfg<TPI>::L>& M, const Lane& ln,
@@ -292,9 +416,13 @@
   mm_finish<TPI>(r, A0, A1, in, M, ln);
 }
 
-template <int TPI>
+template <int TPI, bool Q64 = false>
 MP_DEV void mont_mul(uint32_t (&r)[Cfg<TPI>::L], const uint32_t (&a)[Cfg<TPI>::L], const uint32_t* bs,
                      const Mod<Cfg<TPI>::L>& M, const Lane& ln) {
+  if constexpr (Q64) {
+    mont_mul_q64<TPI>(r, a, bs, M, ln);
+    return;
+  }
 #ifdef MPVSS_MODP_SPLIT_ACC
   mont_mul_il<TPI>(r, a, bs, M, ln);
 #else
diff --git a/mpvss_rs_b200/csrc/modp_kernels.cuh b/mpvss_rs_b200/csrc/modp_kernels.cuh
--- a/mpvss_rs_b200/csrc/modp_kernels.cuh
+++ b/mpvss_rs_b200/csrc/modp_kernels.cuh
@@ -44,14 +44,14 @@
   return c;
 }
 
-template <int TPI>
+template <int TPI, bool Q64 = false>
 MP_DEV void sqr_plain(uint32_t (&acc)[Cfg<TPI>::L], uint32_t* sq, const Mod<Cfg<TPI>::L>& M, const Lane& ln) {
   stage_shared<TPI>(sq, acc, ln);
   simt::syncwarp();
-  mont_mul<TPI>(acc, acc, sq, M, ln);
-}
-
-template <int TPI>
+  mont_mul<TPI, Q64>(acc, acc, sq, M, ln);
+}
+
+template <int TPI, bool Q64 = false>
 MP_DEV void sqr_inplace(uint32_t (&acc)[Cfg<TPI>::L], uint32_t* sq, const SqrCtx& sc, const Mod<Cfg<TPI>::L>& M,
                         const Lane& ln) {
   stage_shared<TPI>(sq, acc, ln);
@@ -62,12 +62,12 @@
 #ifdef MPVSS_MODP_DEDICATED_SQR
     mont_sqr<TPI>(acc, acc, sq, M, ln);
 #else
-    mont_mul<TPI>(acc, acc, sq, M, ln);
+    mont_mul<TPI, Q64>(acc, acc, sq, M, ln);
 #endif
   }
 }
 
-template <int TPI>
+template <int TPI, bool Q64 = false>
 MP_DEV void finish_store(uint32_t (&acc)[Cfg<TPI>::L], uint32_t* sq, uint32_t* dst64, bool live,
                          const Mod<Cfg<TPI>::L>& M, const Lane& ln) {
   constexpr int L = Cfg<TPI>::L;
@@ -77,7 +77,7 @@
   if (ln.k == 0) one[0] = 1;
   stage_shared<TPI>(sq, one, ln);
   simt::syncwarp();
-  mont_mul<TPI>(acc, acc, sq, M, ln);
+  mont_mul<TPI, Q64>(acc, acc, sq, M, ln);
   canonical<TPI>(acc, M, ln);
   if (live) stage<TPI>(dst64, acc, ln);
 }
@@ -102,7 +102,7 @@
 template <int TPI>
 constexpr int horner_smem_words = (32 / TPI) * (HC_GSTRIDE + HC_OPS / 2);
 
-template <int TPI, bool NP1 = false, bool CHUNKED = false>
+template <int TPI, bool Q64 = false, bool CHUNKED = false>
 MP_DEV void horner_body(const HornerArgs& A, uint32_t wg, uint32_t* wsm, uint32_t nops, uint32_t cta = 0) {
   const uint32_t first = CHUNKED ? A.cfirst[cta] : A.t - 1, steps = CHUNKED ? A.csteps[cta] : A.t - 1;
   constexpr int L = Cfg<TPI>::L;
@@ -114,7 +114,6 @@
   if (!live) inst = A.n - 1;
   Mod<L> M;
   load_mod<TPI>(M, A.consts, ln);
-  if (NP1) M.np = 1u;
   uint32_t* gbase = wsm + gi * HC_GSTRIDE;
   uint16_t* opsm = reinterpret_cast<uint16_t*>(wsm + GPW * HC_GSTRIDE) + gi * HC_OPS;
   for (int k = ln.k; k < HC_OPS; k += TPI) opsm[k] = A.ops[(size_t)inst * HC_OPS + k];
@@ -139,12 +138,12 @@
       if (sv) stage<TPI>(gbase + (sv - 1) * 64, acc, ln);
       simt::syncwarp();
       if (a) load_slice<TPI>(acc, gbase + (a - 1) * 64, ln);
-      mont_mul<TPI>(acc, acc, gbase + b * 64, M, ln);
+      mont_mul<TPI, Q64>(acc, acc, gbase + b * 64, M, ln);
       op = nxt;
     }
   }
   const uint32_t slot = A.slot ? A.slot[inst] : inst;
-  finish_store<TPI>(acc, gbase, A.out + (size_t)(slot == 0xffffffffu ? 0 : slot) * 64, live && slot != 0xffffffffu, M,
+  finish_store<TPI, Q64>(acc, gbase, A.out + (size_t)(slot == 0xffffffffu ? 0 : slot) * 64, live && slot != 0xffffffffu, M,
                     ln);
 }
 
@@ -164,7 +163,7 @@
 template <int TPI>
 constexpr int exp2_smem_words = 64 + (32 / TPI) * (16 * 64 + 64 + GPAD + sqr_scratch_words<TPI>);
 
-template <int TPI>
+template <int TPI, bool Q64 = false>
 MP_DEV void exp_window4(uint32_t (&acc)[Cfg<TPI>::L], const uint32_t* base64, const uint32_t* e, uint32_t windows,
                         uint32_t* tbl, uint32_t* sq, const SqrCtx& sc, const uint32_t* r2, const uint32_t* consts,
                         const Mod<Cfg<TPI>::L>& M, const Lane& ln) {
@@ -173,11 +172,11 @@
   load_slice<TPI>(x, consts + C_ONE, ln);
   stage_shared<TPI>(tbl, x, ln);
   load_slice<TPI>(x, base64, ln);
-  mont_mul<TPI>(x, x, r2, M, ln);
+  mont_mul<TPI, Q64>(x, x, r2, M, ln);
   stage_shared<TPI>(tbl + 64, x, ln);
   simt::syncwarp();
   for (int i = 2; i < 16; ++i) {
-    mont_mul<TPI>(x, x, tbl + 64, M, ln);
+    mont_mul<TPI, Q64>(x, x, tbl + 64, M, ln);
     stage_shared<TPI>(tbl + i * 64, x, ln);
     simt::syncwarp();
   }
@@ -186,13 +185,13 @@
   load_slice<TPI>(acc, tbl + d * 64, ln);
   while (wi-- > 0) {
 #pragma unroll 1
-    for (int rep = 0; rep < 4; ++rep) sqr_inplace<TPI>(acc, sq, sc, M, ln);
+    for (int rep = 0; rep < 4; ++rep) sqr_inplace<TPI, Q64>(acc, sq, sc, M, ln);
     d = (e[wi >> 3] >> ((wi & 7u) * 4)) & 15u;
-    mont_mul<TPI>(acc, acc, tbl + d * 64, M, ln);
-  }
-}
-
-template <int TPI>
+    mont_mul<TPI, Q64>(acc, acc, tbl + d * 64, M, ln);
+  }
+}
+
+template <int TPI, bool Q64 = false>
 MP_DEV void exp_comb8(uint32_t (&acc)[Cfg<TPI>::L], const uint32_t* tbl, const uint32_t* e, uint32_t nbytes,
                       uint32_t* sq, const Mod<Cfg<TPI>::L>& M, const Lane& ln) {
   constexpr int L = Cfg<TPI>::L;
@@ -204,7 +203,7 @@
     load_slice<TPI>(x, tbl + ((size_t)w * 256 + d) * 64, ln);
     stage_shared<TPI>(sq, x, ln);
     simt::syncwarp();
-    mont_mul<TPI>(acc, acc, sq, M, ln);
+    mont_mul<TPI, Q64>(acc, acc, sq, M, ln);
   }
 }
 
@@ -217,7 +216,7 @@
 template <int TPI>
 constexpr int comb_smem_words = 64 + (32 / TPI) * (128 + GPAD);
 
-template <int TPI>
+template <int TPI, bool Q64 = false>
 MP_DEV void comb1_body(const CombArgs& A, uint32_t wg, uint32_t* wsm) {
   constexpr int L = Cfg<TPI>::L;
   Lane ln = make_lane<TPI>();
@@ -230,13 +229,13 @@
   simt::syncwarp();
   uint32_t b[L];
   load_slice<TPI>(b, A.base, ln);
-  mont_mul<TPI>(b, b, r2, M, ln);
+  mont_mul<TPI, Q64>(b, b, r2, M, ln);
   for (uint32_t w = 0; w < A.rows; ++w) {
     if (wg == 0 && gi == 0) stage<TPI>(A.tbl + ((size_t)w * 256 + 1) * 64, b, ln);
-    for (int k = 0; k < 8; ++k) sqr_plain<TPI>(b, sq, M, ln);
-  }
-}
-template <int TPI>
+    for (int k = 0; k < 8; ++k) sqr_plain<TPI, Q64>(b, sq, M, ln);
+  }
+}
+template <int TPI, bool Q64 = false>
 MP_DEV void comb2_body(const CombArgs& A, uint32_t wg, uint32_t* wsm) {
   constexpr int L = Cfg<TPI>::L;
   constexpr int GPW = 32 / TPI;
@@ -256,12 +255,12 @@
   stage_shared<TPI>(b1, x, ln);
   simt::syncwarp();
   for (uint32_t d = 2; d < 256; ++d) {
-    mont_mul<TPI>(x, x, b1, M, ln);
+    mont_mul<TPI, Q64>(x, x, b1, M, ln);
     if (live) stage<TPI>(row + (size_t)d * 64, x, ln);
   }
 }
 
-template <int TPI>
+template <int TPI, bool Q64 = false>
 MP_DEV void exp2_body(const Exp2Args& A, uint32_t wg, uint32_t* wsm) {
   constexpr int L = Cfg<TPI>::L;
   constexpr int GPW = 32 / TPI;
@@ -280,19 +279,19 @@
   simt::syncwarp();
   uint32_t acc[L];
   if (A.comb1)
-    exp_comb8<TPI>(acc, A.comb1, A.e1 + (size_t)inst * A.e1_stride, (A.e1_windows + 1) / 2, sq, M, ln);
+    exp_comb8<TPI, Q64>(acc, A.comb1, A.e1 + (size_t)inst * A.e1_stride, (A.e1_windows + 1) / 2, sq, M, ln);
   else
-    exp_window4<TPI>(acc, A.b1 + (size_t)inst * A.b1_stride, A.e1 + (size_t)inst * A.e1_stride, A.e1_windows, tbl,
+    exp_window4<TPI, Q64>(acc, A.b1 + (size_t)inst * A.b1_stride, A.e1 + (size_t)inst * A.e1_stride, A.e1_windows, tbl,
                      sq, sc, r2, A.consts, M, ln);
   if (A.b2 != nullptr) {
     uint32_t acc2[L];
-    exp_window4<TPI>(acc2, A.b2 + (size_t)inst * A.b2_stride, A.e2 + (size_t)inst * A.e2_stride, A.e2_windows, tbl,
+    exp_window4<TPI, Q64>(acc2, A.b2 + (size_t)inst * A.b2_stride, A.e2 + (size_t)inst * A.e2_stride, A.e2_windows, tbl,
                      sq, sc, r2, A.consts, M, ln);
     stage_shared<TPI>(sq, acc2, ln);
     simt::syncwarp();
-    mont_mul<TPI>(acc, acc, sq, M, ln);
-  }
-  finish_store<TPI>(acc, sq, A.out + (size_t)inst * 64, live, M, ln);
+    mont_mul<TPI, Q64>(acc, acc, sq, M, ln);
+  }
+  finish_store<TPI, Q64>(acc, sq, A.out + (size_t)inst * 64, live, M, ln);
 }
 
 struct FrameArgs {
@@ -591,7 +590,7 @@
 template <int TPI>
 constexpr int msm_smem_words = (32 / TPI) * (2 * 64 + GPAD);
 
-template <int TPI>
+template <int TPI, bool Q64 = false>
 MP_DEV void msm_bucket_body(const MsmBucketArgs& A, uint32_t wg, uint32_t* wsm) {
   constexpr int L = Cfg<TPI>::L;
   constexpr int GPW = 32 / TPI;
@@ -622,7 +621,7 @@
     simt::syncwarp();
     if (have) stage<TPI>(stage_buf, x, ln);
     simt::syncwarp();
-    mont_mul<TPI>(acc, acc, have ? stage_buf : one, M, ln);
+    mont_mul<TPI, Q64>(acc, acc, have ? stage_buf : one, M, ln);
   }
   if (live) stage<TPI>(A.buckets + ((size_t)w * 256 + d) * 64, acc, ln);
 }
@@ -636,7 +635,7 @@
 template <int TPI>
 constexpr int msm_window_smem_words = (32 / TPI) * (4 * 64 + GPAD);
 
-template <int TPI>
+template <int TPI, bool Q64 = false>
 MP_DEV void msm_window_body(const MsmWindowArgs& A, uint32_t wg, uint32_t* wsm) {
   constexpr int L = Cfg<TPI>::L;
   constexpr int GPW = 32 / TPI;
@@ -656,25 +655,25 @@
     load_slice<TPI>(x, b < 256u ? A.buckets + ((size_t)w * 256 + b) * 64 : A.consts + C_ONE, ln);
     stage_shared<TPI>(buf, x, ln);
     simt::syncwarp();
-    mont_mul<TPI>(run, run, buf, M, ln);
+    mont_mul<TPI, Q64>(run, run, buf, M, ln);
     stage_shared<TPI>(buf + 64, run, ln);
     simt::syncwarp();
-    mont_mul<TPI>(acc, acc, buf + 64, M, ln);
+    mont_mul<TPI, Q64>(acc, acc, buf + 64, M, ln);
   }
   uint32_t y[L];
 #pragma unroll
   for (int i = 0; i < L; ++i) y[i] = run[i];
-  for (uint32_t q = SEG; q > 1; q >>= 1) sqr_plain<TPI>(y, buf, M, ln);
+  for (uint32_t q = SEG; q > 1; q >>= 1) sqr_plain<TPI, Q64>(y, buf, M, ln);
   stage_shared<TPI>(buf + 128, y, ln);
   load_slice<TPI>(x, A.consts + C_ONE, ln);
   stage_shared<TPI>(buf + 64, x, ln);
   simt::syncwarp();
   for (uint32_t e = 0; e < (uint32_t)GPW - 1; ++e)
-    mont_mul<TPI>(acc, acc, e < gi ? buf + 128 : buf + 64, M, ln);
+    mont_mul<TPI, Q64>(acc, acc, e < gi ? buf + 128 : buf + 64, M, ln);
   stage_shared<TPI>(buf + 192, acc, ln);
   simt::syncwarp();
   load_slice<TPI>(acc, wsm + 192, ln);
-  for (uint32_t s = 1; s < (uint32_t)GPW; ++s) mont_mul<TPI>(acc, acc, wsm + s * (4 * 64 + GPAD) + 192, M, ln);
+  for (uint32_t s = 1; s < (uint32_t)GPW; ++s) mont_mul<TPI, Q64>(acc, acc, wsm + s * (4 * 64 + GPAD) + 192, M, ln);
   if (wg < A.windows && gi == 0) stage<TPI>(A.wprod + (size_t)w * 64, acc, ln);
 }
 
@@ -684,7 +683,7 @@
   uint32_t* out;
   uint32_t windows;
 };
-template <int TPI>
+template <int TPI, bool Q64 = false>
 MP_DEV void msm_fold_body(const MsmFoldArgs& A, uint32_t* wsm) {
   constexpr int L = Cfg<TPI>::L;
   Lane ln = make_lane<TPI>();
@@ -697,13 +696,13 @@
   simt::syncwarp();
   for (int w = (int)A.windows - 2; w >= 0; --w) {
 #pragma unroll 1
-    for (int r = 0; r < 8; ++r) sqr_plain<TPI>(acc, buf, M, ln);
+    for (int r = 0; r < 8; ++r) sqr_plain<TPI, Q64>(acc, buf, M, ln);
     load_slice<TPI>(x, A.wprod + (size_t)w * 64, ln);
     stage_shared<TPI>(buf, x, ln);
     simt::syncwarp();
-    mont_mul<TPI>(acc, acc, buf, M, ln);
-  }
-  finish_store<TPI>(acc, buf, A.out, gi == 0, M, ln);
+    mont_mul<TPI, Q64>(acc, acc, buf, M, ln);
+  }
+  finish_store<TPI, Q64>(acc, buf, A.out, gi == 0, M, ln);
 }
 
 struct MulArgs {
@@ -719,7 +718,7 @@
 template <int TPI>
 constexpr int mul_smem_words = 64 + (32 / TPI) * (64 + GPAD);
 
-template <int TPI>
+template <int TPI, bool Q64 = false>
 MP_DEV void mul_body(const MulArgs& A, uint32_t wg, uint32_t* wsm) {
   constexpr int L = Cfg<TPI>::L;
   constexpr int GPW = 32 / TPI;
@@ -741,7 +740,7 @@
     simt::syncwarp();
     mont_sqr<TPI>(acc, acc, sq, M, ln);
   } else {
-    mont_mul<TPI>(acc, acc, r2, M, ln);
+    mont_mul<TPI, Q64>(acc, acc, r2, M, ln);
   }
   if (A.mode == 0 || A.mode == 3) {
     uint32_t y[L];
@@ -751,7 +750,7 @@
     if (A.mode == 3)
       mont_mul_il<TPI>(acc, acc, sq, M, ln);
     else
-      mont_mul<TPI>(acc, acc, sq, M, ln);
+      mont_mul<TPI, Q64>(acc, acc, sq, M, ln);
   }
   canonical<TPI>(acc, M, ln);
   if (live) stage<TPI>(A.out + (size_t)inst * 64, acc, ln);
@@ -764,7 +763,7 @@
   uint32_t n;
 };
 
-template <int TPI>
+template <int TPI, bool Q64 = false>
 MP_DEV void mul_rows_body(const MulRowsArgs& A, uint32_t wg, uint32_t* wsm) {
   constexpr int L = Cfg<TPI>::L;
   constexpr int GPW = 32 / TPI;
@@ -783,10 +782,10 @@
   uint32_t acc[L], y[L];
   load_slice<TPI>(acc, A.v + (size_t)t[0] * 64, ln);
   load_slice<TPI>(y, A.v + (size_t)t[1] * 64, ln);
-  mont_mul<TPI>(acc, acc, r2, M, ln);
+  mont_mul<TPI, Q64>(acc, acc, r2, M, ln);
   stage_shared<TPI>(sq, y, ln);
   simt::syncwarp();
-  mont_mul<TPI>(acc, acc, sq, M, ln);
+  mont_mul<TPI, Q64>(acc, acc, sq, M, ln);
   canonical<TPI>(acc, M, ln);
   if (live) stage<TPI>(A.v + (size_t)t[2] * 64, acc, ln);
 }
diff --git a/mpvss_rs_b200/csrc/modp_launch.h b/mpvss_rs_b200/csrc/modp_launch.h
--- a/mpvss_rs_b200/csrc/modp_launch.h
+++ b/mpvss_rs_b200/csrc/modp_launch.h
@@ -5,17 +5,17 @@
 namespace modp {
 constexpr int WARPS_PER_CTA = 4;
 constexpr int HORNER_MAX_WARPS_PER_CTA = 4;
-cudaError_t launch_horner(int tpi, const HornerArgs& A, bool np_is_one, cudaStream_t s);
-cudaError_t launch_exp2(int tpi, const Exp2Args& A, cudaStream_t s);
-cudaError_t launch_exp2_filler(int tpi, const Exp2Args& A, size_t ctas, cudaStream_t s);
+cudaError_t launch_horner(int tpi, const HornerArgs& A, bool q64, cudaStream_t s);
+cudaError_t launch_exp2(int tpi, const Exp2Args& A, bool q64, cudaStream_t s);
+cudaError_t launch_exp2_filler(int tpi, const Exp2Args& A, bool q64, size_t ctas, cudaStream_t s);
 cudaError_t launch_frames(const FrameArgs& A, cudaStream_t s);
 cudaError_t launch_resp(const RespArgs& A, cudaStream_t s);
-cudaError_t launch_comb_build(int tpi, const CombArgs& A, cudaStream_t s);
+cudaError_t launch_comb_build(int tpi, const CombArgs& A, bool q64, cudaStream_t s);
 cudaError_t launch_poly(const PolyArgs& A, cudaStream_t s);
 cudaError_t launch_lagrange(const LagrangeArgs& A, cudaStream_t s);
 cudaError_t launch_lagrange_boxes(const LagrangeBoxesArgs& A, cudaStream_t s);
-cudaError_t launch_mul(int tpi, const MulArgs& A, cudaStream_t s);
-cudaError_t launch_mul_rows(int tpi, const MulRowsArgs& A, cudaStream_t s);
+cudaError_t launch_mul(int tpi, const MulArgs& A, bool q64, cudaStream_t s);
+cudaError_t launch_mul_rows(int tpi, const MulRowsArgs& A, bool q64, cudaStream_t s);
 cudaError_t launch_msm(const MsmBucketArgs& B, const uint32_t* scalars, uint32_t* idx, uint32_t* start, uint32_t* wprod,
-                       uint32_t* out, cudaStream_t s);
+                       uint32_t* out, bool q64, cudaStream_t s);
 }
```

Result: slower. 17940, median of 6 (-1.8%).
